# c-zhou/oatk

Hardware: AMD Instinct MI355X
Metric: HiFi Gbases/s through syncasm (syncmer+syncerr) at k=1001 s=31 (higher is better)
Workload: dtype u64

## Files before the change

### include/oatk_hip_ec.h

```cpp
#ifndef OATK_HIP_EC_H
#define OATK_HIP_EC_H

#include "oatk_hip.h"

#ifdef __cplusplus
extern "C" {
#endif

typedef struct {
    uint64_t n_vtx, n_arc;
    const uint64_t *idx_p;
    const uint64_t *idx_n;
    const uint64_t *arc_v;
    const uint64_t *arc_w;
    const uint64_t *arc_ls;
    const uint32_t *arc_cov;
    const uint8_t *arc_del;
} oatk_ec_graph_t;

int oatk_hip_ec(oatk_hip_ctx *ctx, const oatk_ec_graph_t *g, double max_edist, uint32_t err_mer_c, uint32_t max_err_c,
                uint32_t err_arc_c, double max_arc_f);

int oatk_hip_ec_stats(oatk_hip_ctx *ctx, uint64_t *stats12);

int oatk_hip_debug_ec_tiers(oatk_hip_ctx *ctx, int cap_t0, int cap_t1);

int oatk_hip_debug_wf_ed(oatk_hip_ctx *ctx, uint64_t n_jobs, const uint8_t *t_codes, const uint64_t *t_off, const uint8_t *q_codes, const uint64_t *q_off,
                         const int32_t *bw, const int32_t *step_ql, const uint64_t *step_off, int32_t *out3);
int oatk_hip_debug_wf_ed_wg(oatk_hip_ctx *ctx, int R, uint64_t n_jobs, const uint8_t *t_codes, const uint64_t *t_off, const uint8_t *q_codes, const uint64_t *q_off,
                            const int32_t *bw, const int32_t *step_ql, const uint64_t *step_off, int32_t *out3);
int oatk_hip_debug_tables(oatk_hip_ctx *ctx, uint64_t n_jobs, const uint8_t *t_codes, const uint64_t *t_off, const uint8_t *s_codes, const uint64_t *s_off, int32_t *out, const uint64_t *out_off);

enum {
    OATK_BUF_EC_N_SCM = 100, OATK_BUF_EC_SCM_OFF, OATK_BUF_EC_KMER, OATK_BUF_EC_MPOS, OATK_BUF_EC_SMER,
    OATK_BUF_EC_SCM_COV, OATK_BUF_EC_SCM_DEL, OATK_BUF_EC_SCM_OCC_OFF, OATK_BUF_EC_SCM_OCC, OATK_BUF_EC_ERR_DEL,
    OATK_BUF_EC_SCM_FWD,
    OATK_BUF_EC_VTX_SRC,
    OATK_BUF_EC_BLOCK_WORK, OATK_BUF_EC_BLOCK_OUT,
    OATK_BUF_EC_CSEQ_LEN,
    OATK_BUF_EC_CSEQ_OFF,
    OATK_BUF_EC_CSEQ,
    OATK_BUF_EC_BLOCK_QEND
};

int oatk_hip_ec_keep_seq(oatk_hip_ctx *ctx, int on);
int oatk_hip_ec_corrected_reads(oatk_hip_ctx *ctx, uint64_t *n_bases);

int oatk_hip_ec_mark(oatk_hip_ctx *ctx, uint32_t err_mer_c, uint32_t max_err_c, uint32_t err_arc_c, double max_arc_f);
int oatk_hip_ec_correct(oatk_hip_ctx *ctx, double max_edist);

int oatk_hip_ec_graph(oatk_hip_ctx *ctx);
int oatk_hip_ec_graph_light(oatk_hip_ctx *ctx, uint32_t err_mer_c);

int oatk_hip_ec_set_global(oatk_hip_ctx *ctx, uint64_t n_global, const uint32_t *d_l2g, const uint32_t *d_cov, const uint64_t *d_s);
int oatk_hip_ec_pairs(oatk_hip_ctx *ctx, const void **d_keys, const void **d_dist, uint64_t *n_pairs);
int oatk_hip_ec_graph_from_pairs(oatk_hip_ctx *ctx, const uint64_t *d_keys, const uint32_t *d_dist, uint64_t n_pairs);
int oatk_hip_ec_graph_from_segments(oatk_hip_ctx *ctx, const uint64_t *d_keys, const uint64_t *d_val, uint64_t n_seg);
int oatk_hip_ec_export_kmers(oatk_hip_ctx *ctx, const uint32_t *d_ids, uint64_t n, uint8_t *d_out, uint32_t stride, uint8_t *d_rev);
int oatk_hip_ec_import_kmers(oatk_hip_ctx *ctx, const uint32_t *d_ids, const uint8_t *d_rev, const uint8_t *d_kmers, uint64_t n, uint32_t stride);
int oatk_hip_ec_reserve_import(oatk_hip_ctx *ctx, uint64_t bytes);

enum {
    OATK_BUF_EG_IDX_P = 120, OATK_BUF_EG_IDX_N, OATK_BUF_EG_ARC_V, OATK_BUF_EG_ARC_W, OATK_BUF_EG_ARC_LS, OATK_BUF_EG_ARC_COV,
    OATK_BUF_EG_ARC_COMP
};

#ifdef __cplusplus
}
#endif
#endif
```

### oatk_amd/_lib.py

```python
import ctypes as C
import os

HERE = os.path.dirname(os.path.abspath(__file__))
LIB_PATH = os.environ.get("OATK_HIP_LIB") or os.path.join(HERE, "lib", "liboatk_hip.so")
HOST_LIB_PATH = os.path.join(HERE, "lib", "liboatk_host.so")

OK, E_NODEV, E_ARG, E_STATE, E_SMER, E_SPLIT, E_NOMEM = range(7)
READ_ALIGN = 64
BUF = {name: i for i, name in enumerate([
    "HOCO_L", "N_SCM", "N_NN", "N_LRL", "HO_RL", "HOCO_S", "NN_KEY", "LRL_KEY", "LRL_VAL",
    "SCM_OFF", "POS_MPOS", "POS_SMER", "POS_HASH", "POS_KID",
    "SCM_H", "SCM_S", "SCM_COV", "SCM_OCC_OFF", "SCM_OCC"])}
BUF.update({name: 100 + i for i, name in enumerate([
    "EC_N_SCM", "EC_SCM_OFF", "EC_KMER", "EC_MPOS", "EC_SMER", "EC_SCM_COV", "EC_SCM_DEL", "EC_SCM_OCC_OFF", "EC_SCM_OCC", "EC_ERR_DEL",
    "EC_SCM_FWD", "EC_VTX_SRC", "EC_BLOCK_WORK", "EC_BLOCK_OUT", "EC_CSEQ_LEN", "EC_CSEQ_OFF", "EC_CSEQ", "EC_BLOCK_QEND"])})
BUF.update({name: 160 + i for i, name in enumerate(["INGEST_SEQ", "INGEST_OFF", "INGEST_LEN", "INGEST_HDR"])})
FMT_AUTO, FMT_FASTA, FMT_FASTQ = 0, 1, 2
BUF.update({name: 140 + i for i, name in enumerate(["CONS_SEL", "CONS_SLOT", "CONS_RL", "CONS_MSEQ", "CONS_FIRST", "CONS_TOT"])})
BUF.update({name: 200 + i for i, name in enumerate(["RA_ALN_SID", "RA_ALN_OFF", "RA_ALN_S", "RA_FRG_UID", "RA_FRG_UBEG", "RA_FRG_UEND", "RA_FRG_SBEG", "RA_FRG_SEND", "RA_SKIPPED"])})
BUF.update({name: 150 + i for i, name in enumerate(["OVL_KEY", "OVL_OFF", "OVL_DIST", "OVL_CNT", "OVL_TAIL"])})
BUF.update({name: 120 + i for i, name in enumerate([
    "EG_IDX_P", "EG_IDX_N", "EG_ARC_V", "EG_ARC_W", "EG_ARC_LS", "EG_ARC_COV", "EG_ARC_COMP"])})
BUF.update({name: 180 + i for i, name in enumerate([
    "AG_SCM_DEL", "AG_VTX_SCM", "AG_VTX_COV", "AG_IDX_P", "AG_IDX_N", "AG_ARC_V", "AG_ARC_W", "AG_ARC_COV", "AG_ARC_COMP", "AG_ARC_LINK"])})
BUF.update({name: 220 + i for i, name in enumerate(["MG_H", "MG_S", "MG_COV", "MG_L2G", "MG_EC_COV", "MG_EC_DEL", "MG_LCOV"])})
BUF.update({name: 230 + i for i, name in enumerate(["MG_G_H", "MG_G_S", "MG_G_COV", "MG_G_DEL", "MG_G_OCC_OFF", "MG_G_OCC", "MG_POS_GKID"])})
TIMERS = ["hpc", "syncmer", "syncmer_n", "scan_post", "count_place", "count_sort", "count_group", "kmer_hash", "ec_graph", "ec_mark", "ec_solve", "ec_refresh"]

EXPORTS = [
    "oatk_hip_abi_version", "oatk_hip_device_count", "oatk_hip_create", "oatk_hip_destroy", "oatk_hip_last_error",
    "oatk_hip_stream", "oatk_hip_sync", "oatk_hip_max_k", "oatk_hip_scan", "oatk_hip_scan_host", "oatk_hip_count",
    "oatk_comm_unique_id", "oatk_comm_create", "oatk_comm_group_create", "oatk_comm_group_rank", "oatk_comm_group_destroy", "oatk_comm_destroy",
    "oatk_comm_rank", "oatk_comm_size", "oatk_comm_backend", "oatk_comm_traffic", "oatk_hip_merge_counts", "oatk_hip_multi_range", "oatk_hip_ec_sharded",
    "oatk_hip_gather_table", "oatk_hip_asm_graph_sharded", "oatk_hip_consensus_sharded", "oatk_hip_overlap_hist_sharded", "oatk_hip_stat_sharded",
    "oatk_hip_scan_begin", "oatk_hip_scan_reserve", "oatk_hip_scan_append", "oatk_hip_device", "oatk_hip_d2d", "oatk_hip_mem_pool",
    "oatk_hip_info", "oatk_hip_buffer", "oatk_hip_d2h", "oatk_hip_d2h_async", "oatk_hip_h2d_async", "oatk_hip_staging", "oatk_hip_ingest_text_buffer", "oatk_hip_set_timing", "oatk_hip_get_timing",
    "oatk_hip_debug_hash_mask", "oatk_hip_debug_force_general", "oatk_hip_debug_list_cap",
    "oatk_hip_ec_graph", "oatk_hip_ec_graph_light", "oatk_hip_ec", "oatk_hip_ec_stats", "oatk_hip_debug_ec_tiers", "oatk_hip_debug_wf_ed", "oatk_hip_debug_wf_ed_wg", "oatk_hip_ec_mark", "oatk_hip_ec_correct",
    "oatk_hip_ec_set_global", "oatk_hip_ec_pairs", "oatk_hip_ec_graph_from_pairs", "oatk_hip_ec_graph_from_segments", "oatk_hip_ec_export_kmers", "oatk_hip_ec_import_kmers",
    "oatk_hip_ec_reserve_import", "oatk_hip_consensus", "oatk_hip_consensus_ids", "oatk_hip_ingest", "oatk_hip_ingest_host", "oatk_hip_scan_ingested", "oatk_hip_stat", "oatk_hip_stat_keys", "oatk_hip_stat_from_keys",
    "oatk_hip_asm_graph", "oatk_hip_asm_pairs", "oatk_hip_asm_graph_from_pairs", "oatk_hip_overlap_hist", "oatk_hip_overlap_pairs", "oatk_hip_overlap_hist_from_pairs", "oatk_hip_read_alignment", "oatk_hip_debug_align_two_pass",
    "oatk_hip_ra_utg_coverage", "oatk_hip_ra_arc_coverage", "oatk_hip_debug_racov_cap", "oatk_hip_ra_utg_coverage_sharded", "oatk_hip_ra_arc_coverage_sharded",
    "oatk_hip_ra_triplet_scores", "oatk_hip_ra_triplet_scores_sharded",
    "oatk_hip_ec_keep_seq", "oatk_hip_ec_corrected_reads",
]

HOST_EXPORTS = ["oatk_multi_scg_ra_utg_coverage", "oatk_multi_scg_ra_arc_coverage", "oatk_scg_multiplex_plan", "oatk_multi_scg_multiplex_plan",
                "oatk_triplet_table_free", "oatk_multi_read_error_correction_fo"]


def load_host():
    H = C.CDLL(HOST_LIB_PATH)
    vp = C.c_void_p
    H.oatk_sr_db_new.restype = vp
    H.oatk_sr_db_new.argtypes = [C.c_int, C.c_int]
    H.oatk_multi_create.restype = vp
    H.oatk_multi_create.argtypes = [C.POINTER(C.c_int), C.c_int]
    H.oatk_multi_destroy.argtypes = [vp]
    H.oatk_multi_ctx.restype = vp
    H.oatk_multi_ctx.argtypes = [vp, C.c_int]
    H.oatk_multi_last_error.restype = C.c_char_p
    H.oatk_multi_last_error.argtypes = [vp]
    H.oatk_multi_range.argtypes = [vp, C.c_int, C.POINTER(C.c_uint64), C.POINTER(C.c_uint64)]
    H.oatk_multi_sr_read_files.argtypes = [vp, vp, C.POINTER(C.c_char_p), C.c_int]
    H.oatk_multi_collect_syncmer_from_reads.restype = vp
    H.oatk_multi_collect_syncmer_from_reads.argtypes = [vp, vp, C.POINTER(C.c_int)]
    H.oatk_multi_read_error_correction.argtypes = [vp, vp, vp, C.c_double, C.c_uint32, C.c_uint32, C.c_uint32, C.c_double, vp]
    H.oatk_multi_read_error_correction_fo.argtypes = [vp, vp, vp, C.c_double, C.c_uint32, C.c_uint32, C.c_uint32, C.c_double, vp, vp]
    H.oatk_multi_make_syncmer_asmg.restype = vp
    H.oatk_multi_make_syncmer_asmg.argtypes = [vp, vp, C.c_uint32, C.c_double, C.POINTER(C.c_int)]
    H.oatk_multi_scg_read_alignment.argtypes = [vp, vp, vp, vp, C.c_int, C.POINTER(C.c_uint64)]
    H.oatk_multi_scg_ra_utg_coverage.argtypes = [vp, vp, vp, vp, C.c_int]
    H.oatk_multi_scg_ra_arc_coverage.argtypes = [vp, vp, vp, vp, C.c_int]
    H.oatk_scg_multiplex_plan.argtypes = [vp, vp, vp, C.c_uint, C.c_uint32, C.c_double, C.c_double, vp, C.POINTER(C.c_int), C.POINTER(TripletTable)]
    H.oatk_multi_scg_multiplex_plan.argtypes = [vp, vp, vp, C.c_uint32, C.c_double, C.c_double, vp, C.POINTER(C.c_int), C.POINTER(TripletTable)]
    H.oatk_triplet_table_free.restype = None
    H.oatk_triplet_table_free.argtypes = [C.POINTER(TripletTable)]
    H.oatk_host_debug_window.argtypes = [C.c_uint64]
    return H


class TripletTable(C.Structure):
    _fields_ = [("n", C.c_uint64), ("m", C.c_uint64), ("l_in", C.POINTER(C.c_uint64)), ("l_out", C.POINTER(C.c_uint64)), ("val", C.POINTER(C.c_double))]


class EcGraph(C.Structure):
    _fields_ = [("n_vtx", C.c_uint64), ("n_arc", C.c_uint64), ("idx_p", C.c_void_p), ("idx_n", C.c_void_p), ("arc_v", C.c_void_p),
                ("arc_w", C.c_void_p), ("arc_ls", C.c_void_p), ("arc_cov", C.c_void_p), ("arc_del", C.c_void_p)]


class RaGraph(C.Structure):
    _fields_ = [("n_scm", C.c_uint64), ("n_utg", C.c_uint64), ("n_arc", C.c_uint64), ("su_off", C.c_void_p), ("su_uid", C.c_void_p), ("su_pos", C.c_void_p),
                ("utg_n", C.c_void_p), ("idx_p", C.c_void_p), ("idx_n", C.c_void_p), ("arc_w", C.c_void_p), ("arc_ln", C.c_void_p), ("arc_del", C.c_void_p)]


class RacovGraph(C.Structure):
    _fields_ = [("n_scm", C.c_uint64), ("n_utg", C.c_uint64), ("n_arc", C.c_uint64), ("su_off", C.c_void_p), ("su_uid", C.c_void_p), ("su_pos", C.c_void_p),
                ("scm_cov", C.c_void_p), ("utg_off", C.c_void_p), ("utg_a", C.c_void_p), ("idx_p", C.c_void_p), ("idx_n", C.c_void_p), ("arc_v", C.c_void_p),
                ("arc_w", C.c_void_p), ("arc_link", C.c_void_p), ("arc_comp", C.c_void_p), ("arc_del", C.c_void_p), ("vtx_del", C.c_void_p)]


class RacovAln(C.Structure):
    _fields_ = [("n_aln", C.c_uint64), ("n_frg", C.c_uint64), ("sid", C.c_void_p), ("off", C.c_void_p), ("s", C.c_void_p), ("uid", C.c_void_p),
                ("u_beg", C.c_void_p), ("u_end", C.c_void_p), ("s_beg", C.c_void_p), ("s_end", C.c_void_p)]


class RacovReads(C.Structure):
    _fields_ = [("n_reads", C.c_uint64), ("off", C.c_void_p), ("k_mer", C.c_void_p)]


class StatRaw(C.Structure):
    _fields_ = [("n_reads", C.c_uint64), ("n_syncmers", C.c_uint64), ("sum_dist", C.c_int64), ("n_dist", C.c_uint64),
                ("smer_unique", C.c_uint64), ("kmer_unique", C.c_uint64), ("smer_cnt", C.c_int64 * 1001), ("kmer_cnt", C.c_int64 * 1001),
                ("smer_no_singleton", C.c_int64), ("kmer_no_singleton", C.c_int64)]


class Info(C.Structure):
    _fields_ = [("n_reads", C.c_uint64), ("seq_bytes", C.c_uint64), ("sid0", C.c_uint64),
                ("k", C.c_int32), ("s", C.c_int32),
                ("n_occ", C.c_uint64), ("n_nn", C.c_uint64), ("n_lrl", C.c_uint64), ("n_scm", C.c_uint64),
                ("scan_retries", C.c_uint32), ("collisions", C.c_uint32)]


class OatkHipError(RuntimeError):
    pass


_lib = None


def load():
    global _lib
    if _lib is not None:
        return _lib
    if not os.path.exists(LIB_PATH):
        raise OatkHipError("%s is missing: build it with __graft_entry__.build()" % LIB_PATH)
    L = C.CDLL(LIB_PATH)
    vp = C.c_void_p
    L.oatk_hip_abi_version.restype = C.c_int
    L.oatk_hip_device_count.restype = C.c_int
    L.oatk_hip_create.restype = vp
    L.oatk_hip_create.argtypes = [C.c_int]
    L.oatk_hip_destroy.argtypes = [vp]
    L.oatk_hip_last_error.restype = C.c_char_p
    L.oatk_hip_last_error.argtypes = [vp]
    L.oatk_hip_stream.restype = vp
    L.oatk_hip_stream.argtypes = [vp]
    L.oatk_hip_sync.argtypes = [vp]
    L.oatk_hip_max_k.restype = C.c_int
    L.oatk_hip_scan.argtypes = [vp, vp, vp, vp, C.c_uint64, C.c_uint64, C.c_uint64, C.c_int, C.c_int]
    L.oatk_hip_scan_host.argtypes = [vp, vp, vp, vp, C.c_uint64, C.c_uint64, C.c_uint64, C.c_int, C.c_int]
    L.oatk_hip_count.argtypes = [vp]
    L.oatk_comm_unique_id.argtypes = [vp]
    L.oatk_comm_create.restype = vp
    L.oatk_comm_create.argtypes = [vp, C.c_int, C.c_int, C.c_int]
    L.oatk_comm_group_create.restype = vp
    L.oatk_comm_group_create.argtypes = [C.c_int]
    L.oatk_comm_group_rank.restype = vp
    L.oatk_comm_group_rank.argtypes = [vp, C.c_int]
    L.oatk_comm_group_destroy.argtypes = [vp]
    L.oatk_comm_destroy.argtypes = [vp]
    L.oatk_comm_rank.argtypes = [vp]
    L.oatk_comm_size.argtypes = [vp]
    L.oatk_comm_backend.restype = C.c_char_p
    L.oatk_comm_backend.argtypes = [vp]
    L.oatk_comm_traffic.restype = None
    L.oatk_comm_traffic.argtypes = [vp, C.POINTER(C.c_uint64), C.c_int]
    L.oatk_hip_merge_counts.argtypes = [vp, vp, C.POINTER(C.c_uint64)]
    L.oatk_hip_multi_range.argtypes = [vp, C.POINTER(C.c_uint64), C.POINTER(C.c_uint64), C.POINTER(C.c_uint64)]
    L.oatk_hip_ec_sharded.argtypes = [vp, vp, C.c_double, C.c_uint32, C.c_uint32, C.c_uint32, C.c_double, vp, C.POINTER(C.c_uint64)]
    L.oatk_hip_gather_table.argtypes = [vp, vp, C.c_int]
    L.oatk_hip_asm_graph_sharded.argtypes = [vp, vp, C.c_uint32, C.c_double, C.POINTER(C.c_uint64), C.POINTER(C.c_uint64)]
    L.oatk_hip_consensus_sharded.argtypes = [vp, vp, C.c_uint32]
    L.oatk_hip_overlap_hist_sharded.argtypes = [vp, vp, C.c_uint32, C.POINTER(C.c_uint64), C.POINTER(C.c_uint64)]
    L.oatk_hip_stat_sharded.argtypes = [vp, vp, C.POINTER(StatRaw)]
    L.oatk_hip_scan_begin.argtypes = [vp, C.c_uint64, C.c_int, C.c_int]
    L.oatk_hip_scan_reserve.argtypes = [vp, C.c_uint64, C.c_uint64, C.c_uint64]
    L.oatk_hip_scan_append.argtypes = [vp, vp]
    L.oatk_hip_device.argtypes = [vp]
    L.oatk_hip_mem_pool.argtypes = [vp, C.c_uint64]
    L.oatk_hip_d2d.argtypes = [vp, vp, vp, C.c_uint64]
    L.oatk_hip_info.argtypes = [vp, C.POINTER(Info)]
    L.oatk_hip_buffer.argtypes = [vp, C.c_int, C.POINTER(vp), C.POINTER(C.c_uint64)]
    L.oatk_hip_d2h.argtypes = [vp, vp, vp, C.c_uint64]
    L.oatk_hip_staging.restype = vp
    L.oatk_hip_staging.argtypes = [vp, C.c_uint64]
    L.oatk_hip_set_timing.argtypes = [vp, C.c_int]
    L.oatk_hip_get_timing.argtypes = [vp, C.POINTER(C.c_float), C.c_int]
    L.oatk_hip_debug_hash_mask.argtypes = [vp, C.c_uint64]
    L.oatk_hip_debug_force_general.argtypes = [vp, C.c_int]
    L.oatk_hip_debug_list_cap.argtypes = [vp, C.c_int]
    L.oatk_hip_ec_graph.argtypes = [vp]
    L.oatk_hip_ec_graph_light.argtypes = [vp, C.c_uint32]
    L.oatk_hip_ec.argtypes = [vp, C.POINTER(EcGraph), C.c_double, C.c_uint32, C.c_uint32, C.c_uint32, C.c_double]
    L.oatk_hip_ec_stats.argtypes = [vp, vp]
    L.oatk_hip_debug_ec_tiers.argtypes = [vp, C.c_int, C.c_int]
    L.oatk_hip_debug_wf_ed.argtypes = [vp, C.c_uint64, vp, vp, vp, vp, vp, vp, vp, vp]
    if hasattr(L, "oatk_hip_debug_wf_ed_wg"):
        L.oatk_hip_debug_wf_ed_wg.argtypes = [vp, C.c_int, C.c_uint64, vp, vp, vp, vp, vp, vp, vp, vp]
    if hasattr(L, "oatk_hip_debug_ed_ab"):
        L.oatk_hip_debug_ed_ab.argtypes = [vp, C.c_int, C.c_uint64, vp, vp, vp, vp, vp, vp, C.POINTER(C.c_float)]
    L.oatk_hip_ec_mark.argtypes = [vp, C.c_uint32, C.c_uint32, C.c_uint32, C.c_double]
    L.oatk_hip_ec_correct.argtypes = [vp, C.c_double]
    L.oatk_hip_ec_keep_seq.argtypes = [vp, C.c_int]
    L.oatk_hip_ec_corrected_reads.argtypes = [vp, C.POINTER(C.c_uint64)]
    L.oatk_hip_ec_set_global.argtypes = [vp, C.c_uint64, vp, vp, vp]
    L.oatk_hip_ec_pairs.argtypes = [vp, C.POINTER(vp), C.POINTER(vp), C.POINTER(C.c_uint64)]
    L.oatk_hip_ec_graph_from_pairs.argtypes = [vp, vp, vp, C.c_uint64]
    L.oatk_hip_ec_graph_from_segments.argtypes = [vp, vp, vp, C.c_uint64]
    L.oatk_hip_ec_export_kmers.argtypes = [vp, vp, C.c_uint64, vp, C.c_uint32, vp]
    L.oatk_hip_ec_import_kmers.argtypes = [vp, vp, vp, vp, C.c_uint64, C.c_uint32]
    L.oatk_hip_ec_reserve_import.argtypes = [vp, C.c_uint64]
    L.oatk_hip_consensus.argtypes = [vp, C.c_uint32]
    L.oatk_hip_consensus_ids.argtypes = [vp, vp, C.c_uint64]
    L.oatk_hip_ingest.argtypes = [vp, vp, C.c_uint64, C.c_int, C.c_int, C.POINTER(C.c_uint64), C.POINTER(C.c_uint64)]
    L.oatk_hip_ingest_host.argtypes = [vp, vp, C.c_uint64, C.c_int, C.c_int, C.POINTER(C.c_uint64), C.POINTER(C.c_uint64)]
    L.oatk_hip_scan_ingested.argtypes = [vp, C.c_uint64, C.c_int, C.c_int]
    L.oatk_hip_stat.argtypes = [vp, C.POINTER(StatRaw)]
    L.oatk_hip_stat_keys.argtypes = [vp, C.POINTER(vp), C.POINTER(vp), C.POINTER(C.c_uint64), vp]
    L.oatk_hip_stat_from_keys.argtypes = [vp, vp, vp, C.c_uint64, vp, C.POINTER(StatRaw)]
    L.oatk_hip_debug_align_two_pass.argtypes = [vp, C.c_int]
    L.oatk_hip_read_alignment.argtypes = [vp, C.POINTER(RaGraph), vp, C.POINTER(C.c_uint64), C.POINTER(C.c_uint64), vp]
    L.oatk_hip_ra_utg_coverage.argtypes = [vp, C.POINTER(RacovGraph), C.POINTER(RacovReads), C.POINTER(RacovAln), C.c_int, vp, C.POINTER(C.c_uint64)]
    L.oatk_hip_ra_arc_coverage.argtypes = [vp, C.POINTER(RacovGraph), C.POINTER(RacovAln), vp]
    L.oatk_hip_debug_racov_cap.argtypes = [vp, C.c_uint64]
    L.oatk_hip_ra_utg_coverage_sharded.argtypes = [vp, vp, C.POINTER(RacovGraph), C.POINTER(RacovReads), C.POINTER(RacovAln), C.c_int, vp, C.POINTER(C.c_uint64)]
    L.oatk_hip_ra_arc_coverage_sharded.argtypes = [vp, vp, C.POINTER(RacovGraph), C.POINTER(RacovAln), vp]
    u64p = C.POINTER(C.c_uint64)
    L.oatk_hip_ra_triplet_scores.argtypes = [vp, C.POINTER(RacovGraph), C.POINTER(RacovAln), vp, C.c_uint64, u64p, vp, vp, vp, vp]
    L.oatk_hip_ra_triplet_scores_sharded.argtypes = [vp, vp, C.POINTER(RacovGraph), C.POINTER(RacovAln), vp, C.c_uint64, u64p, vp, vp, vp, vp]
    L.oatk_hip_overlap_pairs.argtypes = [vp, C.POINTER(vp), C.POINTER(vp), C.POINTER(C.c_uint64)]
    L.oatk_hip_overlap_hist_from_pairs.argtypes = [vp, vp, vp, C.c_uint64, C.POINTER(C.c_uint64), C.POINTER(C.c_uint64)]
    L.oatk_hip_overlap_hist.argtypes = [vp, C.POINTER(C.c_uint64), C.POINTER(C.c_uint64)]
    L.oatk_hip_asm_graph.argtypes = [vp, C.c_uint32, C.c_double, C.POINTER(C.c_uint64), C.POINTER(C.c_uint64)]
    L.oatk_hip_asm_pairs.argtypes = [vp, C.POINTER(vp), C.POINTER(C.c_uint64)]
    L.oatk_hip_asm_graph_from_pairs.argtypes = [vp, vp, C.c_uint64, C.c_uint64, vp, vp, C.c_uint32, C.c_double, C.POINTER(C.c_uint64), C.POINTER(C.c_uint64)]
    _lib = L
    return L
```

### oatk_amd/csrc/api_ec.inc

```
#include "../../include/oatk_hip_ec.h"
#include "ec.hpp"
#include "ec_wave.hpp"
#include "ec_heavy.hpp"
#include "ec_fused.hpp"
#include "ecgraph.hpp"
#include "ec_seq.hpp"
#include <rocprim/device/device_run_length_encode.hpp>
#include <rocprim/device/device_select.hpp>

struct EcState {
    DevBuf idx_p, idx_n, arc_v, arc_w, arc_ls, arc_cov, arc_del, conv;
    DevBuf scm_del, err_del, vtx_hs_off, vtx_mpos;
    DevBuf copy_n, seg, keep_all, n_blocks, n_blocks64, blk_off, work, out, path_pool, cursor, todo, todo2, slabs, big_slabs, os_slabs;
    DevBuf hyb_slabs[16];
    hipStream_t aux[5] = {nullptr, nullptr, nullptr, nullptr, nullptr};
    hipEvent_t aux_ev[5] = {nullptr, nullptr, nullptr, nullptr, nullptr}, fork_ev = nullptr;
    DevBuf new_n, new_n64, new_off, new_k, new_m, new_s, stats;
    DevBuf live32, live64, live_off, larc, lidx_p, lidx_n;
    DevBuf cov, fwd, key_id, key_sorted, val_occ, occ, occ_off, cov64;
    uint64_t n_vtx = 0, new_tot = 0;
    uint64_t stats_h[12] = {0};
    uint64_t n_work = 0;
    bool done = false;
    DevBuf g_keys, g_keys2, g_ukeys, g_counts, g_nruns, g_nout, g_nout64, g_outoff, g_akey, g_aval, g_skey, g_sval, g_comp, g_flags, g_huge;
    DevBuf g_dist, g_dist2, g_cnt64, g_runoff, g_runls;
    DevBuf g_big, g_keep, g_other, g_lkeys, g_ldist, g_val2, g_wgt2, g_runcov, g_head, g_hpos, g_iota, g_segk, g_segv;
    uint32_t light_c = 0;
    uint64_t g_n_vtx = 0, g_n_arc = 0;
    bool graph_resident = false;
    bool global = false, marked = false;
    uint64_t n_global = 0, imp_used = 0;
    DevBuf g_l2g, g_kid, g_gcov, g_gs;
    bool keep_seq = false;
    bool seq_kept = false, cseq_done = false;
    bool seq_global = false;
    DevBuf slot_w, slot_w64, slot_off, slots, qend, sblk, clen, cbytes, cbytes64, coff, cseq;
    uint64_t cseq_bytes = 0;
};

static uint64_t ec_n_vtx(oatk_hip_ctx *ctx) { return ctx->ec && ctx->ec->global? ctx->ec->n_global : ctx->n_scm_total; }
static const uint64_t *ec_chains(oatk_hip_ctx *ctx) { return ctx->ec && ctx->ec->global? ctx->ec->g_kid.as<uint64_t>() : ctx->pos_kid.as<uint64_t>(); }

static void ec_state_free(oatk_hip_ctx *ctx)
{
    if (!ctx->ec) return;
    EcState *e = ctx->ec;
    DevBuf *all[] = {&e->idx_p, &e->idx_n, &e->arc_v, &e->arc_w, &e->arc_ls, &e->arc_cov, &e->arc_del, &e->conv, &e->scm_del, &e->err_del,
                     &e->vtx_hs_off, &e->vtx_mpos, &e->copy_n, &e->seg, &e->keep_all, &e->n_blocks, &e->n_blocks64, &e->blk_off, &e->work, &e->out, &e->path_pool, &e->cursor,
                     &e->todo, &e->todo2, &e->slabs, &e->big_slabs, &e->os_slabs, &e->hyb_slabs[0], &e->hyb_slabs[1], &e->hyb_slabs[2], &e->hyb_slabs[3], &e->hyb_slabs[4], &e->hyb_slabs[5], &e->hyb_slabs[6], &e->hyb_slabs[7], &e->hyb_slabs[8], &e->hyb_slabs[9], &e->hyb_slabs[10], &e->hyb_slabs[11], &e->hyb_slabs[12], &e->hyb_slabs[13], &e->hyb_slabs[14], &e->hyb_slabs[15], &e->new_n, &e->new_n64, &e->new_off, &e->new_k, &e->new_m, &e->new_s, &e->stats,
                     &e->live32, &e->live64, &e->live_off, &e->larc, &e->lidx_p, &e->lidx_n, &e->cov, &e->fwd, &e->key_id, &e->key_sorted, &e->val_occ, &e->occ, &e->occ_off, &e->cov64,
                     &e->g_keys, &e->g_keys2, &e->g_ukeys, &e->g_counts, &e->g_nruns, &e->g_nout, &e->g_nout64, &e->g_outoff, &e->g_akey,
                     &e->g_aval, &e->g_skey, &e->g_sval, &e->g_comp, &e->g_flags, &e->g_huge, &e->g_dist, &e->g_dist2, &e->g_cnt64, &e->g_runoff, &e->g_runls,
                     &e->g_big, &e->g_keep, &e->g_other, &e->g_lkeys, &e->g_ldist, &e->g_val2, &e->g_wgt2, &e->g_runcov, &e->g_head, &e->g_hpos, &e->g_iota, &e->g_segk, &e->g_segv,
                     &e->g_l2g, &e->g_kid, &e->g_gcov, &e->g_gs,
                     &e->slot_w, &e->slot_w64, &e->slot_off, &e->slots, &e->qend, &e->sblk, &e->clen, &e->cbytes, &e->cbytes64, &e->coff, &e->cseq};
    for (DevBuf *b : all) b->release();
    for (int i = 0; i < 5; ++i) { if (e->aux[i]) (void) hipStreamDestroy(e->aux[i]); if (e->aux_ev[i]) (void) hipEventDestroy(e->aux_ev[i]); }
    if (e->fork_ev) (void) hipEventDestroy(e->fork_ev);
    delete e;
    ctx->ec = nullptr;
}

static int ec_buffer(oatk_hip_ctx *ctx, int which, const void **d_ptr, uint64_t *bytes)
{
    EcState *e = ctx->ec;
    if (e && which >= OATK_BUF_EG_IDX_P && which <= OATK_BUF_EG_ARC_COMP) {
        if (!e->graph_resident) { ctx->err = "EC graph requested before oatk_hip_ec_graph"; return OATK_E_STATE; }
        const uint64_t gv = e->g_n_vtx, ga = e->g_n_arc;
        switch (which) {
            case OATK_BUF_EG_IDX_P: *d_ptr = e->idx_p.p, *bytes = 2 * gv * 8; break;
            case OATK_BUF_EG_IDX_N: *d_ptr = e->idx_n.p, *bytes = 2 * gv * 4; break;
            case OATK_BUF_EG_ARC_V: *d_ptr = e->arc_v.p, *bytes = ga * 8; break;
            case OATK_BUF_EG_ARC_W: *d_ptr = e->arc_w.p, *bytes = ga * 8; break;
            case OATK_BUF_EG_ARC_LS: *d_ptr = e->arc_ls.p, *bytes = ga * 4; break;
            case OATK_BUF_EG_ARC_COV: *d_ptr = e->arc_cov.p, *bytes = ga * 4; break;
            default: *d_ptr = e->g_comp.p, *bytes = ga; break;
        }
        return OATK_OK;
    }
    if (e && (which == OATK_BUF_EC_VTX_SRC || (which == OATK_BUF_EC_ERR_DEL && !e->done))) {
        if (!e->marked) { ctx->err = "vertex sources / marks requested before oatk_hip_ec_mark"; return OATK_E_STATE; }
        if (which == OATK_BUF_EC_VTX_SRC) *d_ptr = e->vtx_hs_off.p, *bytes = e->n_vtx * 8;
        else *d_ptr = e->err_del.p, *bytes = e->n_vtx;
        return OATK_OK;
    }
    if (!e || !e->done) { ctx->err = "unknown buffer id, or error-correction results requested before oatk_hip_ec"; return OATK_E_STATE; }
    if (which == OATK_BUF_EC_BLOCK_WORK) { *d_ptr = e->work.p, *bytes = e->n_work * sizeof(oatk::EcWork); return OATK_OK; }
    if (which == OATK_BUF_EC_BLOCK_OUT) { *d_ptr = e->out.p, *bytes = e->n_work * sizeof(oatk::EcBlockOut); return OATK_OK; }
    if (which == OATK_BUF_EC_BLOCK_QEND) {
        if (!e->seq_kept) { ctx->err = "EC_BLOCK_QEND: the resident correction was made without oatk_hip_ec_keep_seq"; return OATK_E_STATE; }
        *d_ptr = e->qend.p, *bytes = e->n_work * 4;
        return OATK_OK;
    }
    if (which >= OATK_BUF_EC_CSEQ_LEN && which <= OATK_BUF_EC_CSEQ) {
        if (!e->seq_kept || !e->cseq_done) { ctx->err = "corrected sequences requested before oatk_hip_ec_corrected_reads"; return OATK_E_STATE; }
        if (which == OATK_BUF_EC_CSEQ_LEN) *d_ptr = e->clen.p, *bytes = ctx->n_reads * 4;
        else if (which == OATK_BUF_EC_CSEQ_OFF) *d_ptr = e->coff.p, *bytes = (ctx->n_reads + 1) * 8;
        else *d_ptr = e->cseq.p, *bytes = e->cseq_bytes;
        return OATK_OK;
    }
    const uint64_t n = ctx->n_reads, ns = e->n_vtx, tot = e->new_tot;
    switch (which) {
        case OATK_BUF_EC_N_SCM: *d_ptr = e->new_n.p, *bytes = n * 4; break;
        case OATK_BUF_EC_SCM_OFF: *d_ptr = e->new_off.p, *bytes = (n + 1) * 8; break;
        case OATK_BUF_EC_KMER: *d_ptr = e->new_k.p, *bytes = tot * 8; break;
        case OATK_BUF_EC_MPOS: *d_ptr = e->new_m.p, *bytes = tot * 4; break;
        case OATK_BUF_EC_SMER: *d_ptr = e->new_s.p, *bytes = tot * 8; break;
        case OATK_BUF_EC_SCM_COV: *d_ptr = e->cov.p, *bytes = ns * 4; break;
        case OATK_BUF_EC_SCM_DEL: *d_ptr = e->scm_del.p, *bytes = ns; break;
        case OATK_BUF_EC_SCM_OCC_OFF: *d_ptr = e->occ_off.p, *bytes = (ns + 1) * 8; break;
        case OATK_BUF_EC_SCM_OCC: *d_ptr = e->occ.p, *bytes = tot * 8; break;
        case OATK_BUF_EC_ERR_DEL: *d_ptr = e->err_del.p, *bytes = ns; break;
        case OATK_BUF_EC_SCM_FWD: *d_ptr = e->fwd.p, *bytes = ns * 4; break;
        default: ctx->err = "unknown buffer id"; return OATK_E_ARG;
    }
    return OATK_OK;
}

__global__ void ec_narrow_kernel(const uint64_t *in, uint32_t *out, uint64_t n)
{
    uint64_t i = (uint64_t) blockIdx.x * blockDim.x + threadIdx.x;
    if (i < n) out[i] = (uint32_t) in[i];
}
__global__ void ec_widen_kernel(const uint32_t *in, uint64_t *out, uint64_t n)
{
    uint64_t i = (uint64_t) blockIdx.x * blockDim.x + threadIdx.x;
    if (i < n) out[i] = in[i];
    if (i == n) out[i] = 0;
}
#define EENSURE(buf, bytes, ...)                                                                   \
    do {                                                                                           \
        if (!e->buf.ensure((bytes), ctx->stream, ##__VA_ARGS__)) {                                 \
            ctx->err = "hipMalloc failed for ec." #buf;                                            \
            return OATK_E_NOMEM;                                                                   \
        }                                                                                          \
    } while (0)

static int ec_exclusive_scan_u32(oatk_hip_ctx *ctx, EcState *e, DevBuf &in32, DevBuf &tmp64, DevBuf &out64, uint64_t n, uint64_t *total)
{
    if (!tmp64.ensure((n + 1) * 8, ctx->stream) || !out64.ensure((n + 1) * 8, ctx->stream)) { ctx->err = "hipMalloc failed (ec scan)"; return OATK_E_NOMEM; }
    hipLaunchKernelGGL(ec_widen_kernel, dim3((unsigned) ((n + 1 + 255) / 256)), dim3(256), 0, ctx->stream, in32.as<uint32_t>(), tmp64.as<uint64_t>(), n);
    size_t tb = 0;
    CK(rocprim::exclusive_scan(nullptr, tb, tmp64.as<uint64_t>(), out64.as<uint64_t>(), (uint64_t) 0, n + 1, rocprim::plus<uint64_t>(), ctx->stream));
    if (!ctx->tmp.ensure(tb, ctx->stream)) { ctx->err = "hipMalloc failed (ec scan tmp)"; return OATK_E_NOMEM; }
    CK(rocprim::exclusive_scan(ctx->tmp.p, tb, tmp64.as<uint64_t>(), out64.as<uint64_t>(), (uint64_t) 0, n + 1, rocprim::plus<uint64_t>(), ctx->stream));
    CK(hipMemcpyAsync(total, out64.as<uint64_t>() + n, 8, hipMemcpyDeviceToHost, ctx->stream));
    CK(hipStreamSynchronize(ctx->stream));
    (void) e;
    return OATK_OK;
}

extern "C" int oatk_hip_debug_ec_tiers(oatk_hip_ctx *ctx, int cap_t0, int cap_t1)
{
    if (!ctx) return OATK_E_NODEV;
    if (cap_t0 < 0 || cap_t1 < 0 || (cap_t0 && cap_t1 && cap_t1 < cap_t0)) { ctx->err = "oatk_hip_debug_ec_tiers: 0 <= cap_t0 <= cap_t1"; return OATK_E_ARG; }
    ctx->ec_cap_t0 = cap_t0, ctx->ec_cap_t1 = cap_t1;
    return OATK_OK;
}

static int debug_ed_impl(oatk_hip_ctx *ctx, uint64_t n_jobs, const uint8_t *t_codes, const uint64_t *t_off, const uint8_t *q_codes, const uint64_t *q_off,
                         const int32_t *bw, const int32_t *step_ql, const uint64_t *step_off, int32_t *out3, bool myers, float *kernel_ms, int wg_R = 0)
{
    using namespace oatk;
    if (!ctx) return OATK_E_NODEV;
    if (n_jobs == 0) return OATK_OK;
    if (n_jobs >= 0x7FFFFFFFULL) { ctx->err = "oatk_hip_debug_wf_ed: too many jobs"; return OATK_E_ARG; }
    CK(hipSetDevice(ctx->device));
    std::vector<uint64_t> tw_off(n_jobs + 1, 0), qw_off(n_jobs + 1, 0), k_off(n_jobs + 1, 0);
    std::vector<int32_t> tl(n_jobs);
    for (uint64_t j = 0; j < n_jobs; ++j) {
        const uint64_t t = t_off[j + 1] - t_off[j], q = q_off[j + 1] - q_off[j];
        if (t == 0 || q == 0 || t > 0x3FFFFFFF || q > 0x3FFFFFFF) { ctx->err = "oatk_hip_debug_wf_ed: empty or oversized string (wf_ed asserts tl > 0 && ql > 0)"; return OATK_E_ARG; }
        for (uint64_t s = step_off[j]; s < step_off[j + 1]; ++s)
            if (step_ql[s] < 1 || (uint64_t) step_ql[s] > q || (s > step_off[j] && step_ql[s] < step_ql[s - 1])) { ctx->err = "oatk_hip_debug_wf_ed: query lengths must ascend within the query"; return OATK_E_ARG; }
        tl[j] = (int32_t) t;
        if (wg_R && (bw[j] >= 0? (uint64_t) 2 * (uint64_t) bw[j] + 3 : t + q + 3) > (wg_R == ECF_NW? (uint64_t) ECF_NW * ECF_OWN : (uint64_t) 64 * ECH_NW * (uint64_t) wg_R)) { ctx->err = "oatk_hip_debug_wf_ed_wg: a job's diagonals do not fit the registers of this variant"; return OATK_E_ARG; }
        tw_off[j + 1] = tw_off[j] + ecw_words((int32_t) t), qw_off[j + 1] = qw_off[j] + ecw_words((int32_t) q);
        k_off[j + 1] = k_off[j] + 2 * (t + q + 8);
    }
    auto pack = [](const uint8_t *codes, const uint64_t *off, const std::vector<uint64_t> &woff, uint64_t n) {
        std::vector<uint32_t> w(woff[n], 0u);
        for (uint64_t j = 0; j < n; ++j)
            for (uint64_t p = 0, len = off[j + 1] - off[j]; p < len; ++p)
                w[woff[j] + (p >> 4)] |= (uint32_t) (codes[off[j] + p] & 3u) << ((p & 15u) << 1);
        return w;
    };
    const std::vector<uint32_t> tw = pack(t_codes, t_off, tw_off, n_jobs), qw = pack(q_codes, q_off, qw_off, n_jobs);
    const uint64_t n_steps = step_off[n_jobs];
    DevBuf d_tw, d_qw, d_two, d_qwo, d_tl, d_bw, d_sq, d_so, d_k, d_ko, d_out, d_slab;
    DevBuf *all[] = {&d_tw, &d_qw, &d_two, &d_qwo, &d_tl, &d_bw, &d_sq, &d_so, &d_k, &d_ko, &d_out, &d_slab};
    hipEvent_t ev0 = nullptr, ev1 = nullptr;
    if (kernel_ms) { *kernel_ms = 0.f; (void) hipEventCreate(&ev0); (void) hipEventCreate(&ev1); }
    int32_t max_t = 0;
    for (uint64_t j = 0; j < n_jobs; ++j) if (tl[j] > max_t) max_t = tl[j];
    const uint64_t n_waves = (n_jobs + 63) / 64, slab_words = (uint64_t) 6 * 64 * (uint64_t) ((max_t + 63) / 64 + 1);
    std::vector<int32_t> ql_last(n_jobs);
    for (uint64_t j = 0; j < n_jobs; ++j) ql_last[j] = step_off[j + 1] > step_off[j]? step_ql[step_off[j + 1] - 1] : (int32_t) (q_off[j + 1] - q_off[j]);
    int rc = OATK_OK;
    hipError_t he = hipSuccess;
    auto up = [&](DevBuf &b, const void *src, size_t bytes) {
        if (rc) return;
        if (!b.ensure(bytes + 16, ctx->stream)) { rc = OATK_E_NOMEM; return; }
        if (bytes && (he = hipMemcpyAsync(b.p, src, bytes, hipMemcpyHostToDevice, ctx->stream)) != hipSuccess) rc = OATK_E_NODEV;
    };
    up(d_tw, tw.data(), tw.size() * 4); up(d_qw, qw.data(), qw.size() * 4);
    up(d_two, tw_off.data(), (n_jobs + 1) * 8); up(d_qwo, qw_off.data(), (n_jobs + 1) * 8); up(d_ko, k_off.data(), (n_jobs + 1) * 8);
    up(d_tl, tl.data(), n_jobs * 4); up(d_bw, bw, n_jobs * 4); up(d_sq, step_ql, n_steps * 4); up(d_so, step_off, (n_jobs + 1) * 8);
    if (!rc && (!d_k.ensure(k_off[n_jobs] * 4 + 16, ctx->stream) || !d_out.ensure(n_steps * 12 + 16, ctx->stream))) rc = OATK_E_NOMEM;
    if (!rc && myers) {
        if (!d_slab.ensure(n_waves * slab_words * 8 + 64, ctx->stream) || !d_out.ensure(n_jobs * 12 + 16, ctx->stream)) rc = OATK_E_NOMEM;
        up(d_sq, ql_last.data(), n_jobs * 4);
    }
    if (!rc) {
        if (ev0) (void) hipEventRecord(ev0, ctx->stream);
#ifdef OATK_EXPERIMENTS
        if (myers)
            hipLaunchKernelGGL(myers_ed_kernel, dim3((unsigned) n_waves), dim3(64), 0, ctx->stream, n_jobs, d_tw.as<uint32_t>(), d_two.as<uint64_t>(), d_tl.as<int32_t>(),
                               d_qw.as<uint32_t>(), d_qwo.as<uint64_t>(), d_sq.as<int32_t>(), d_bw.as<int32_t>(), d_slab.as<uint64_t>(), slab_words, d_out.as<int32_t>());
        else
#endif
        if (wg_R) {
            uint64_t cap_words = 0;
            for (uint64_t j = 0; j < n_jobs; ++j) { if (tw_off[j + 1] - tw_off[j] > cap_words) cap_words = tw_off[j + 1] - tw_off[j]; if (qw_off[j + 1] - qw_off[j] > cap_words) cap_words = qw_off[j + 1] - qw_off[j]; }
            const uint64_t lds = ((uint64_t) ech_misc_words(wg_R) + 2 * cap_words) * 4;
            if (lds > 64 * 1024 || (wg_R != 1 && wg_R != 2 && wg_R != 6 && wg_R != ECF_NW)) { ctx->err = "oatk_hip_debug_wf_ed_wg: strings too long for LDS, or no such variant (1, 2, 6, 16)"; rc = OATK_E_ARG; }
            else if (wg_R == ECF_NW) hipLaunchKernelGGL((ecf_wf_ed_kernel<ECF_NW>), dim3((unsigned) n_jobs), dim3(64 * ECF_NW), (unsigned) (((uint64_t) ecf_misc_words(ECF_NW) + 2 * cap_words) * 4), ctx->stream, d_tw.as<uint32_t>(), d_two.as<uint64_t>(), d_tl.as<int32_t>(),
                                                         d_qw.as<uint32_t>(), d_qwo.as<uint64_t>(), d_bw.as<int32_t>(), d_sq.as<int32_t>(), d_so.as<uint64_t>(), d_out.as<int32_t>(), (int32_t) cap_words);
            else if (wg_R == 1) hipLaunchKernelGGL((ech_wf_ed_kernel<ECH_NW, 1>), dim3((unsigned) n_jobs), dim3(64 * ECH_NW), (unsigned) lds, ctx->stream, d_tw.as<uint32_t>(), d_two.as<uint64_t>(), d_tl.as<int32_t>(),
                                                    d_qw.as<uint32_t>(), d_qwo.as<uint64_t>(), d_bw.as<int32_t>(), d_sq.as<int32_t>(), d_so.as<uint64_t>(), d_out.as<int32_t>(), (int32_t) cap_words);
            else if (wg_R == 2) hipLaunchKernelGGL((ech_wf_ed_kernel<ECH_NW, 2>), dim3((unsigned) n_jobs), dim3(64 * ECH_NW), (unsigned) lds, ctx->stream, d_tw.as<uint32_t>(), d_two.as<uint64_t>(), d_tl.as<int32_t>(),
                                                    d_qw.as<uint32_t>(), d_qwo.as<uint64_t>(), d_bw.as<int32_t>(), d_sq.as<int32_t>(), d_so.as<uint64_t>(), d_out.as<int32_t>(), (int32_t) cap_words);
            else hipLaunchKernelGGL((ech_wf_ed_kernel<ECH_NW, 6>), dim3((unsigned) n_jobs), dim3(64 * ECH_NW), (unsigned) lds, ctx->stream, d_tw.as<uint32_t>(), d_two.as<uint64_t>(), d_tl.as<int32_t>(),
                                    d_qw.as<uint32_t>(), d_qwo.as<uint64_t>(), d_bw.as<int32_t>(), d_sq.as<int32_t>(), d_so.as<uint64_t>(), d_out.as<int32_t>(), (int32_t) cap_words);
        } else
        hipLaunchKernelGGL(ecw_wf_ed_kernel, dim3((unsigned) n_jobs), dim3(64), 0, ctx->stream, d_tw.as<uint32_t>(), d_two.as<uint64_t>(), d_tl.as<int32_t>(),
                           d_qw.as<uint32_t>(), d_qwo.as<uint64_t>(), d_bw.as<int32_t>(), d_sq.as<int32_t>(), d_so.as<uint64_t>(), d_k.as<int32_t>(),
                           d_ko.as<uint64_t>(), d_out.as<int32_t>());
        if (ev1) (void) hipEventRecord(ev1, ctx->stream);
        const uint64_t n_out = myers? n_jobs : n_steps;
        if (n_out && (he = hipMemcpyAsync(out3, d_out.p, n_out * 12, hipMemcpyDeviceToHost, ctx->stream)) != hipSuccess) rc = OATK_E_NODEV;
        if ((he = hipStreamSynchronize(ctx->stream)) != hipSuccess) rc = OATK_E_NODEV;
        if (!rc && (he = hipGetLastError()) != hipSuccess) rc = OATK_E_NODEV;
    }
    (void) hipStreamSynchronize(ctx->stream);
    if (ev0 && ev1 && !rc) (void) hipEventElapsedTime(kernel_ms, ev0, ev1);
    if (ev0) (void) hipEventDestroy(ev0);
    if (ev1) (void) hipEventDestroy(ev1);
    for (DevBuf *b : all) b->release();
    if (rc == OATK_E_NODEV) ctx->err = std::string("oatk_hip_debug_wf_ed: ") + hipGetErrorString(he);
    if (rc == OATK_E_NOMEM) ctx->err = "oatk_hip_debug_wf_ed: hipMalloc failed";
    return rc;
}

extern "C" int oatk_hip_debug_wf_ed(oatk_hip_ctx *ctx, uint64_t n_jobs, const uint8_t *t_codes, const uint64_t *t_off, const uint8_t *q_codes, const uint64_t *q_off,
                                    const int32_t *bw, const int32_t *step_ql, const uint64_t *step_off, int32_t *out3)
{
    float ms = 0.f;
    const bool timed = getenv("OATK_DEBUG_ED_TIME") != nullptr;
    const int rc = debug_ed_impl(ctx, n_jobs, t_codes, t_off, q_codes, q_off, bw, step_ql, step_off, out3, false, timed? &ms : nullptr);
    if (timed) fprintf(stderr, "[wf_ed_wg] R 0: %llu jobs, kernel %.3f ms\n", (unsigned long long) n_jobs, ms);
    return rc;
}

extern "C" int oatk_hip_debug_tables(oatk_hip_ctx *ctx, uint64_t n_jobs, const uint8_t *t_codes, const uint64_t *t_off, const uint8_t *s_codes, const uint64_t *s_off, int32_t *out, const uint64_t *out_off)
{
    using namespace oatk;
    if (!ctx) return OATK_E_NODEV;
    if (n_jobs == 0) return OATK_OK;
    if (n_jobs >= 0x7FFFFFFFULL) { ctx->err = "oatk_hip_debug_tables: too many jobs"; return OATK_E_ARG; }
    CK(hipSetDevice(ctx->device));
    std::vector<uint64_t> tw_off(n_jobs + 1, 0), qw_off(n_jobs + 1, 0);
    std::vector<int32_t> tl(n_jobs), ql(n_jobs);
    uint64_t cap_words = 0;
    for (uint64_t j = 0; j < n_jobs; ++j) {
        const uint64_t t = t_off[j + 1] - t_off[j], q = s_off[j + 1] - s_off[j];
        if (t == 0 || q == 0 || t > 0x3FFFFFFF || q > 1024) { ctx->err = "oatk_hip_debug_tables: an empty string, or one of more than 1024 bases"; return OATK_E_ARG; }
        if (out_off[j + 1] - out_off[j] < 2 * (t + 1)) { ctx->err = "oatk_hip_debug_tables: a job's output holds 2 (tl + 1) numbers"; return OATK_E_ARG; }
        tl[j] = (int32_t) t, ql[j] = (int32_t) q;
        tw_off[j + 1] = tw_off[j] + ecw_words((int32_t) t), qw_off[j + 1] = qw_off[j] + ecw_words((int32_t) q);
        if (tw_off[j + 1] - tw_off[j] > cap_words) cap_words = tw_off[j + 1] - tw_off[j];
        if (qw_off[j + 1] - qw_off[j] > cap_words) cap_words = qw_off[j + 1] - qw_off[j];
    }
    if (2 * cap_words * 4 > 64 * 1024) { ctx->err = "oatk_hip_debug_tables: strings too long for LDS"; return OATK_E_ARG; }
    auto pack = [](const uint8_t *codes, const uint64_t *off, const std::vector<uint64_t> &woff, uint64_t n) {
        std::vector<uint32_t> w(woff[n], 0u);
        for (uint64_t j = 0; j < n; ++j)
            for (uint64_t p = 0, len = off[j + 1] - off[j]; p < len; ++p)
                w[woff[j] + (p >> 4)] |= (uint32_t) (codes[off[j] + p] & 3u) << ((p & 15u) << 1);
        return w;
    };
    const std::vector<uint32_t> tw = pack(t_codes, t_off, tw_off, n_jobs), qw = pack(s_codes, s_off, qw_off, n_jobs);
    DevBuf d_tw, d_qw, d_two, d_qwo, d_tl, d_ql, d_oo, d_out;
    DevBuf *all[] = {&d_tw, &d_qw, &d_two, &d_qwo, &d_tl, &d_ql, &d_oo, &d_out};
    int rc = OATK_OK;
    hipError_t he = hipSuccess;
    auto up = [&](DevBuf &b, const void *src, size_t bytes) {
        if (rc) return;
        if (!b.ensure(bytes + 16, ctx->stream)) { rc = OATK_E_NOMEM; return; }
        if (bytes && (he = hipMemcpyAsync(b.p, src, bytes, hipMemcpyHostToDevice, ctx->stream)) != hipSuccess) rc = OATK_E_NODEV;
    };
    up(d_tw, tw.data(), tw.size() * 4); up(d_qw, qw.data(), qw.size() * 4);
    up(d_two, tw_off.data(), (n_jobs + 1) * 8); up(d_qwo, qw_off.data(), (n_jobs + 1) * 8);
    up(d_tl, tl.data(), n_jobs * 4); up(d_ql, ql.data(), n_jobs * 4); up(d_oo, out_off, (n_jobs + 1) * 8);
    const uint64_t n_out = out_off[n_jobs];
    if (!rc && !d_out.ensure(n_out * 4 + 16, ctx->stream)) rc = OATK_E_NOMEM;
    if (!rc) {
        int seg_nw = 1, seg_cut = 0;
        { const char *ev = getenv("OATK_DEBUG_TABLES_SEG"); if (ev && sscanf(ev, "%d:%d", &seg_nw, &seg_cut) != 2) seg_nw = 1, seg_cut = 0; }
        if (n_out && (he = hipMemsetAsync(d_out.p, 0xFF, n_out * 4, ctx->stream)) != hipSuccess) rc = OATK_E_NODEV;
#define OATK_TABLES_LAUNCH(NW) hipLaunchKernelGGL((ecb_tables_kernel<NW>), dim3((unsigned) n_jobs), dim3(64 * NW), (unsigned) (2 * cap_words * 4), ctx->stream, d_tw.as<uint32_t>(), d_two.as<uint64_t>(), d_tl.as<int32_t>(), \
                           d_qw.as<uint32_t>(), d_qwo.as<uint64_t>(), d_ql.as<int32_t>(), d_out.as<int32_t>(), d_oo.as<uint64_t>(), (int32_t) cap_words, (int32_t) seg_cut)
        if (seg_nw == 2) OATK_TABLES_LAUNCH(2); else if (seg_nw == 4) OATK_TABLES_LAUNCH(4); else if (seg_nw == 8) OATK_TABLES_LAUNCH(8); else if (seg_nw == 16) OATK_TABLES_LAUNCH(16); else OATK_TABLES_LAUNCH(1);
#undef OATK_TABLES_LAUNCH
        if (n_out && (he = hipMemcpyAsync(out, d_out.p, n_out * 4, hipMemcpyDeviceToHost, ctx->stream)) != hipSuccess) rc = OATK_E_NODEV;
        if ((he = hipStreamSynchronize(ctx->stream)) != hipSuccess) rc = OATK_E_NODEV;
        if (!rc && (he = hipGetLastError()) != hipSuccess) rc = OATK_E_NODEV;
    }
    (void) hipStreamSynchronize(ctx->stream);
    for (DevBuf *b : all) b->release();
    if (rc == OATK_E_NODEV) ctx->err = std::string("oatk_hip_debug_tables: ") + hipGetErrorString(he);
    if (rc == OATK_E_NOMEM) ctx->err = "oatk_hip_debug_tables: hipMalloc failed";
    return rc;
}

extern "C" int oatk_hip_debug_wf_ed_wg(oatk_hip_ctx *ctx, int R, uint64_t n_jobs, const uint8_t *t_codes, const uint64_t *t_off, const uint8_t *q_codes, const uint64_t *q_off,
                                       const int32_t *bw, const int32_t *step_ql, const uint64_t *step_off, int32_t *out3)
{
    if (R != 1 && R != 2 && R != 6 && R != ECF_NW) { if (ctx) ctx->err = "oatk_hip_debug_wf_ed_wg: R must be 1, 2, 6 (a workgroup per wavefront) or 16 (several steps per barrier: sixteen waves, 896 diagonals)"; return OATK_E_ARG; }
    float ms = 0.f;
    const bool timed = getenv("OATK_DEBUG_ED_TIME") != nullptr;
    const int rc = debug_ed_impl(ctx, n_jobs, t_codes, t_off, q_codes, q_off, bw, step_ql, step_off, out3, false, timed? &ms : nullptr, R);
    if (timed) fprintf(stderr, "[wf_ed_wg] R %d: %llu jobs, kernel %.3f ms\n", R, (unsigned long long) n_jobs, ms);
    return rc;
}

#ifdef OATK_EXPERIMENTS
extern "C" int oatk_hip_debug_ed_ab(oatk_hip_ctx *ctx, int myers, uint64_t n_jobs, const uint8_t *t_codes, const uint64_t *t_off, const uint8_t *q_codes,
                                    const uint64_t *q_off, const int32_t *bw, int32_t *out3, float *kernel_ms)
{
    if (!ctx) return OATK_E_NODEV;
    std::vector<int32_t> ql(n_jobs);
    std::vector<uint64_t> so(n_jobs + 1);
    for (uint64_t j = 0; j < n_jobs; ++j) ql[j] = (int32_t) (q_off[j + 1] - q_off[j]), so[j] = j;
    so[n_jobs] = n_jobs;
    return debug_ed_impl(ctx, n_jobs, t_codes, t_off, q_codes, q_off, bw, ql.data(), so.data(), out3, myers != 0, kernel_ms);
}
#endif

extern "C" int oatk_hip_ec_stats(oatk_hip_ctx *ctx, uint64_t *stats12)
{
    if (!ctx) return OATK_E_NODEV;
    if (!ctx->ec || !ctx->ec->done) { ctx->err = "oatk_hip_ec has not run"; return OATK_E_STATE; }
    for (int i = 0; i < 12; ++i) stats12[i] = ctx->ec->stats_h[i];
    return OATK_OK;
}

extern "C" int oatk_hip_ec_set_global(oatk_hip_ctx *ctx, uint64_t n_global, const uint32_t *d_l2g, const uint32_t *d_cov, const uint64_t *d_s)
{
    using namespace oatk;
    if (!ctx) return OATK_E_NODEV;
    if (!ctx->counted) { ctx->err = "oatk_hip_ec_set_global needs a resident scan + count"; return OATK_E_STATE; }
    CK(hipSetDevice(ctx->device));
    if (!ctx->ec) ctx->ec = new EcState();
    EcState *e = ctx->ec;
    e->graph_resident = false, e->done = false, e->marked = false, e->imp_used = 0;
    if (n_global == 0) { e->global = false, e->n_global = 0; return OATK_OK; }
    if (n_global < ctx->n_scm_total || n_global >= 0x7FFFFFFFULL) { ctx->err = "oatk_hip_ec_set_global: bad global table size"; return OATK_E_ARG; }
    const uint64_t nl = ctx->n_scm_total, nocc = ctx->n_occ;
    EENSURE(g_l2g, (nl + 1) * 4); EENSURE(g_gcov, (n_global + 1) * 4); EENSURE(g_gs, (n_global + 1) * 8); EENSURE(g_kid, (nocc + 1) * 8);
    CK(hipMemcpyAsync(e->g_l2g.p, d_l2g, nl * 4, hipMemcpyDeviceToDevice, ctx->stream));
    CK(hipMemcpyAsync(e->g_gcov.p, d_cov, n_global * 4, hipMemcpyDeviceToDevice, ctx->stream));
    CK(hipMemcpyAsync(e->g_gs.p, d_s, n_global * 8, hipMemcpyDeviceToDevice, ctx->stream));
    if (nocc) hipLaunchKernelGGL(ec_remap_kernel, dim3((unsigned) ((nocc + 255) / 256)), dim3(256), 0, ctx->stream, nocc, ctx->pos_kid.as<uint64_t>(),
                                 e->g_l2g.as<uint32_t>(), e->g_kid.as<uint64_t>());
    CK(hipStreamSynchronize(ctx->stream));
    CK(hipGetLastError());
    e->global = true, e->n_global = n_global;
    return OATK_OK;
}

extern "C" int oatk_hip_ec_pairs(oatk_hip_ctx *ctx, const void **d_keys, const void **d_dist, uint64_t *n_pairs)
{
    using namespace oatk;
    if (!ctx) return OATK_E_NODEV;
    if (!ctx->counted) { ctx->err = "oatk_hip_ec_pairs needs a resident scan + count"; return OATK_E_STATE; }
    CK(hipSetDevice(ctx->device));
    if (!ctx->ec) ctx->ec = new EcState();
    EcState *e = ctx->ec;
    const uint64_t nr = ctx->n_reads, nocc = ctx->n_occ;
    EENSURE(g_keys, (nocc + 1) * 8); EENSURE(g_dist, (nocc + 1) * 4);
    if (nocc) hipLaunchKernelGGL(egr_pair_keys_kernel, dim3((unsigned) ((nr + 255) / 256)), dim3(256), 0, ctx->stream, nr, ctx->scm_off.as<uint64_t>(),
                                 ec_chains(ctx), ctx->pos_mpos.as<uint32_t>(), e->g_keys.as<uint64_t>(), e->g_dist.as<uint32_t>(), 0);
    CK(hipStreamSynchronize(ctx->stream));
    CK(hipGetLastError());
    *d_keys = e->g_keys.p, *d_dist = e->g_dist.p, *n_pairs = nocc;
    return OATK_OK;
}

static int ec_graph_build(oatk_hip_ctx *ctx, const uint64_t *d_keys, const uint32_t *d_dist, const uint64_t *d_val, uint64_t nocc, bool timer_running = false)
{
    using namespace oatk;
    if (!ctx) return OATK_E_NODEV;
    if (!ctx->counted) { ctx->err = "oatk_hip_ec_graph needs a resident scan + count"; return OATK_E_STATE; }
    CK(hipSetDevice(ctx->device));
    if (!ctx->ec) ctx->ec = new EcState();
    EcState *e = ctx->ec;
    e->graph_resident = false, e->marked = false, e->light_c = 0;
    const bool weighted = d_val != nullptr;
    if (nocc >= 0xFFFFFFFFULL) { ctx->err = "more than 2^32 adjacent pairs"; return OATK_E_ARG; }
    const uint64_t nv = ec_n_vtx(ctx);
    if (nv >= 0x7FFFFFFFULL) { ctx->err = "too many syncmers for 32-bit oriented vertex ids"; return OATK_E_ARG; }
    auto blocks = [](uint64_t n) { return dim3((unsigned) ((n + 255) / 256 > 0? (n + 255) / 256 : 1)); };
    EENSURE(g_flags, 64);
    if (!timer_running) t_begin(ctx, OATK_T_EC_GRAPH);
    CK(hipMemsetAsync(e->g_flags.p, 0, 64, ctx->stream));
    EENSURE(idx_p, (2 * nv + 1) * 8); EENSURE(idx_n, (2 * nv + 1) * 4);
    CK(hipMemsetAsync(e->idx_p.p, 0, (2 * nv + 1) * 8, ctx->stream));
    CK(hipMemsetAsync(e->idx_n.p, 0, (2 * nv + 1) * 4, ctx->stream));
    uint64_t na = 0;
    if (nocc) {
        EENSURE(g_keys2, (nocc + 1) * 8); EENSURE(g_ukeys, (nocc + 1) * 8); EENSURE(g_counts, (nocc + 1) * 4);
        EENSURE(g_nruns, 64); EENSURE(g_dist2, (nocc + 1) * 4);
        uint64_t *keys_in = const_cast<uint64_t *>(d_keys);
        uint32_t *dist_in = const_cast<uint32_t *>(d_dist);
        size_t tb = 0;
        if (weighted) {
            EENSURE(g_val2, (nocc + 1) * 8); EENSURE(g_wgt2, (nocc + 1) * 4);
            uint64_t *val_in = const_cast<uint64_t *>(d_val);
            CK(rocprim::radix_sort_pairs(nullptr, tb, keys_in, e->g_keys2.as<uint64_t>(), val_in, e->g_val2.as<uint64_t>(), nocc, 0, 64, ctx->stream));
            ENSURE(tmp, tb);
            CK(rocprim::radix_sort_pairs(ctx->tmp.p, tb, keys_in, e->g_keys2.as<uint64_t>(), val_in, e->g_val2.as<uint64_t>(), nocc, 0, 64, ctx->stream));
            hipLaunchKernelGGL(egr_seg_split_kernel, blocks(nocc), dim3(256), 0, ctx->stream, nocc, e->g_val2.as<uint64_t>(), e->g_dist2.as<uint32_t>(), e->g_wgt2.as<uint32_t>());
        } else {
            CK(rocprim::radix_sort_pairs(nullptr, tb, keys_in, e->g_keys2.as<uint64_t>(), dist_in, e->g_dist2.as<uint32_t>(), nocc, 0, 64, ctx->stream));
            ENSURE(tmp, tb);
            CK(rocprim::radix_sort_pairs(ctx->tmp.p, tb, keys_in, e->g_keys2.as<uint64_t>(), dist_in, e->g_dist2.as<uint32_t>(), nocc, 0, 64, ctx->stream));
        }
        tb = 0;
        CK(rocprim::run_length_encode(nullptr, tb, e->g_keys2.as<uint64_t>(), (unsigned int) nocc, e->g_ukeys.as<uint64_t>(), e->g_counts.as<uint32_t>(),
                                      e->g_nruns.as<uint32_t>(), ctx->stream));
        ENSURE(tmp, tb);
        CK(rocprim::run_length_encode(ctx->tmp.p, tb, e->g_keys2.as<uint64_t>(), (unsigned int) nocc, e->g_ukeys.as<uint64_t>(), e->g_counts.as<uint32_t>(),
                                      e->g_nruns.as<uint32_t>(), ctx->stream));
        uint32_t n_runs = 0;
        CK(hipMemcpyAsync(&n_runs, e->g_nruns.p, 4, hipMemcpyDeviceToHost, ctx->stream));
        CK(hipStreamSynchronize(ctx->stream));
        EENSURE(g_nout, ((uint64_t) n_runs + 1) * 4);
        hipLaunchKernelGGL(egr_expand_count_kernel, blocks(n_runs), dim3(256), 0, ctx->stream, (uint64_t) n_runs, e->g_ukeys.as<uint64_t>(), e->g_nout.as<uint32_t>());
        { int rc = ec_exclusive_scan_u32(ctx, e, e->g_nout, e->g_nout64, e->g_outoff, n_runs, &na); if (rc) return rc; }
        uint64_t chk = 0;
        EENSURE(g_runls, ((uint64_t) n_runs + 1) * 4); EENSURE(g_runcov, ((uint64_t) n_runs + 1) * 4);
        { int rc = ec_exclusive_scan_u32(ctx, e, e->g_counts, e->g_cnt64, e->g_runoff, n_runs, &chk); if (rc) return rc; }
        if (n_runs) {
            EENSURE(g_big, ((uint64_t) n_runs + 1) * 8);
            EENSURE(g_huge, EGR_HUGE_SCRATCH);
            const uint32_t *wg = weighted? e->g_wgt2.as<uint32_t>() : (const uint32_t *) nullptr;
            uint32_t *rc_ = weighted? e->g_runcov.as<uint32_t>() : (uint32_t *) nullptr;
            hipLaunchKernelGGL(egr_mode_kernel, dim3((n_runs + 63) / 64), dim3(64), 0, ctx->stream, (uint64_t) n_runs, e->g_ukeys.as<uint64_t>(),
                               e->g_counts.as<uint32_t>(), e->g_runoff.as<uint64_t>(), e->g_dist2.as<uint32_t>(), ctx->K, e->g_runls.as<uint32_t>(),
                               e->g_flags.as<uint32_t>(), e->g_big.as<uint32_t>(), e->g_big.as<uint32_t>() + n_runs + 1, wg, rc_);
            hipLaunchKernelGGL(egr_mode_big_kernel, dim3(n_runs < 8192u? n_runs : 8192u), dim3(64), 0, ctx->stream, e->g_counts.as<uint32_t>(), e->g_runoff.as<uint64_t>(),
                               e->g_dist2.as<uint32_t>(), ctx->K, e->g_runls.as<uint32_t>(), e->g_flags.as<uint32_t>(), e->g_big.as<uint32_t>(),
                               e->g_big.as<uint32_t>() + n_runs + 1, wg, rc_);
            hipLaunchKernelGGL(egr_mode_huge_kernel, dim3(1024), dim3(64), 0, ctx->stream, e->g_counts.as<uint32_t>(), e->g_runoff.as<uint64_t>(),
                               e->g_dist2.as<uint32_t>(), ctx->K, e->g_runls.as<uint32_t>(), e->g_flags.as<uint32_t>(), e->g_big.as<uint32_t>() + n_runs + 1,
                               e->g_huge.as<uint8_t>(), (uint64_t) EGR_HUGE_SCRATCH, wg, rc_);
        }
        EENSURE(g_akey, (na + 1) * 8); EENSURE(g_aval, (na + 1) * 8); EENSURE(g_skey, (na + 1) * 8); EENSURE(g_sval, (na + 1) * 8);
        if (na) {
            hipLaunchKernelGGL(egr_expand_kernel, blocks(n_runs), dim3(256), 0, ctx->stream, (uint64_t) n_runs, e->g_ukeys.as<uint64_t>(),
                               weighted? e->g_runcov.as<uint32_t>() : e->g_counts.as<uint32_t>(), e->g_runls.as<uint32_t>(), e->g_outoff.as<uint64_t>(), e->g_akey.as<uint64_t>(), e->g_aval.as<uint64_t>());
            tb = 0;
            CK(rocprim::radix_sort_pairs(nullptr, tb, e->g_akey.as<uint64_t>(), e->g_skey.as<uint64_t>(), e->g_aval.as<uint64_t>(), e->g_sval.as<uint64_t>(), na, 0, 64, ctx->stream));
            ENSURE(tmp, tb);
            CK(rocprim::radix_sort_pairs(ctx->tmp.p, tb, e->g_akey.as<uint64_t>(), e->g_skey.as<uint64_t>(), e->g_aval.as<uint64_t>(), e->g_sval.as<uint64_t>(), na, 0, 64, ctx->stream));
        }
    }
    EENSURE(arc_v, (na + 1) * 8); EENSURE(arc_w, (na + 1) * 8); EENSURE(arc_ls, (na + 1) * 4); EENSURE(arc_cov, (na + 1) * 4); EENSURE(arc_del, na + 8);
    EENSURE(g_comp, na + 8);
    EgrArcs a;
    a.n_arc = na, a.arc_v = e->arc_v.as<uint64_t>(), a.arc_w = e->arc_w.as<uint64_t>(), a.arc_ls = e->arc_ls.as<uint32_t>(), a.arc_cov = e->arc_cov.as<uint32_t>();
    a.arc_comp = e->g_comp.as<uint8_t>(), a.arc_del = e->arc_del.as<uint8_t>(), a.idx_p = e->idx_p.as<uint64_t>(), a.idx_n = e->idx_n.as<uint32_t>();
    a.flags = e->g_flags.as<uint32_t>();
    if (na) {
        hipLaunchKernelGGL(egr_unpack_kernel, blocks(na), dim3(256), 0, ctx->stream, a, (const uint64_t *) e->g_skey.p, (const uint64_t *) e->g_sval.p);
    }
    uint32_t fl[4] = {0, 0, 0, 0};
    CK(hipMemcpyAsync(fl, e->g_flags.p, sizeof(fl), hipMemcpyDeviceToHost, ctx->stream));
    t_end(ctx, OATK_T_EC_GRAPH);
    CK(hipStreamSynchronize(ctx->stream));
    CK(hipGetLastError());
    t_collect(ctx, OATK_T_EC_GRAPH, OATK_T_EC_GRAPH);
    if (fl[0]) { ctx->err = "EC graph has duplicate arcs (a syncmer adjacent to itself on both strands): the reference's order is unspecified"; return OATK_E_SPLIT; }
    if (fl[1]) { ctx->err = "EC graph: the arcs with more than 48 distinct syncmer distances need more than the 256 MB of working memory set aside for them"; return OATK_E_SPLIT; }
    if (debug_refuse(ctx, 1, "oatk_hip_ec_graph")) return OATK_E_SPLIT;
    e->g_n_vtx = nv, e->g_n_arc = na;
    e->graph_resident = true;
    return OATK_OK;
}

extern "C" int oatk_hip_ec_graph_from_pairs(oatk_hip_ctx *ctx, const uint64_t *d_keys, const uint32_t *d_dist, uint64_t nocc)
{
    return ec_graph_build(ctx, d_keys, d_dist, nullptr, nocc);
}

extern "C" int oatk_hip_ec_graph_from_segments(oatk_hip_ctx *ctx, const uint64_t *d_keys, const uint64_t *d_val, uint64_t n_seg)
{
    if (ctx && !d_val && n_seg) { ctx->err = "oatk_hip_ec_graph_from_segments: no segment values"; return OATK_E_ARG; }
    return ec_graph_build(ctx, d_keys, nullptr, d_val? d_val : (const uint64_t *) d_keys, n_seg);
}

extern "C" int oatk_hip_ec_graph(oatk_hip_ctx *ctx)
{
    const void *k = nullptr, *d = nullptr;
    uint64_t n = 0;
    int rc = oatk_hip_ec_pairs(ctx, &k, &d, &n);
    if (rc) return rc;
    return oatk_hip_ec_graph_from_pairs(ctx, (const uint64_t *) k, (const uint32_t *) d, n);
}

template <class T>
static int ec_select(oatk_hip_ctx *ctx, EcState *e, const T *in, const uint8_t *flag, uint64_t n, T *out, uint64_t *n_out)
{
    *n_out = 0;
    if (n == 0) return OATK_OK;
    EENSURE(g_nruns, 64);
    uint64_t *d_cnt = e->g_nruns.as<uint64_t>() + 2;
    size_t tb = 0;
    CK(rocprim::select(nullptr, tb, in, flag, out, d_cnt, n, ctx->stream));
    ENSURE(tmp, tb);
    CK(rocprim::select(ctx->tmp.p, tb, in, flag, out, d_cnt, n, ctx->stream));
    CK(hipMemcpyAsync(n_out, d_cnt, 8, hipMemcpyDeviceToHost, ctx->stream));
    CK(hipStreamSynchronize(ctx->stream));
    return OATK_OK;
}

static int ec_light_pairs(oatk_hip_ctx *ctx, uint32_t c, const uint64_t **d_keys, const uint32_t **d_dist, uint64_t *n_keep)
{
    using namespace oatk;
    if (!ctx->counted) { ctx->err = "the light EC graph needs a resident scan + count"; return OATK_E_STATE; }
    if (!ctx->ec) ctx->ec = new EcState();
    EcState *e = ctx->ec;
    const uint64_t nv = ec_n_vtx(ctx), nr = ctx->n_reads, n = ctx->n_occ;
    int rc;
    EENSURE(g_keys, (n + 1) * 8); EENSURE(g_dist, (n + 1) * 4);
    EENSURE(g_other, 2 * nv + 8); EENSURE(g_keep, n + 8); EENSURE(g_lkeys, (n + 1) * 8); EENSURE(g_ldist, (n + 1) * 4);
    t_begin(ctx, OATK_T_EC_GRAPH);
    CK(hipMemsetAsync(e->g_other.p, 0, 2 * nv + 8, ctx->stream));
    if (n) hipLaunchKernelGGL(egr_pair_light_wave_kernel, dim3((unsigned) ((nr + 3) / 4)), dim3(256), 0, ctx->stream, nr, ctx->scm_off.as<uint64_t>(), ec_chains(ctx),
                              ctx->pos_mpos.as<uint32_t>(), e->global? e->g_gcov.as<uint32_t>() : ctx->scm_cov.as<uint32_t>(), c, e->g_keys.as<uint64_t>(), e->g_dist.as<uint32_t>(),
                              e->g_keep.as<uint8_t>(), e->g_other.as<uint8_t>());
    uint64_t nk = 0;
    if (n) {
        if (n >= 0xFFFFFFFFULL) { ctx->err = "more than 2^32 adjacent pairs"; return OATK_E_ARG; }
        EENSURE(g_keys2, (n + 1) * 8); EENSURE(g_nruns, 64);
        uint32_t *pos = e->g_keys2.as<uint32_t>();
        uint64_t *d_cnt = e->g_nruns.as<uint64_t>() + 2;
        auto flags = rocprim::make_transform_iterator(e->g_keep.as<uint8_t>(), [] __device__(uint8_t f) -> uint32_t { return f; });
        size_t tb = 0;
        CK(rocprim::exclusive_scan(nullptr, tb, flags, pos, 0u, n, rocprim::plus<uint32_t>(), ctx->stream));
        ENSURE(tmp, tb);
        CK(rocprim::exclusive_scan(ctx->tmp.p, tb, flags, pos, 0u, n, rocprim::plus<uint32_t>(), ctx->stream));
        hipLaunchKernelGGL(egr_compact_pairs_kernel, dim3((unsigned) ((n + 255) / 256)), dim3(256), 0, ctx->stream, n, e->g_keep.as<uint8_t>(), pos, e->g_keys.as<uint64_t>(),
                           e->g_dist.as<uint32_t>(), e->g_lkeys.as<uint64_t>(), e->g_ldist.as<uint32_t>(), d_cnt);
        CK(hipMemcpyAsync(&nk, d_cnt, 8, hipMemcpyDeviceToHost, ctx->stream));
        CK(hipStreamSynchronize(ctx->stream));
    }
    (void) rc;
    CK(hipGetLastError());
    *d_keys = e->g_lkeys.as<uint64_t>(), *d_dist = e->g_ldist.as<uint32_t>(), *n_keep = nk;
    return OATK_OK;
}

extern "C" int oatk_hip_ec_graph_light(oatk_hip_ctx *ctx, uint32_t err_mer_c)
{
    if (!ctx) return OATK_E_NODEV;
    if (!ctx->counted) { ctx->err = "oatk_hip_ec_graph_light needs a resident scan + count"; return OATK_E_STATE; }
    CK(hipSetDevice(ctx->device));
    if (!ctx->ec) ctx->ec = new EcState();
    if (err_mer_c == 0) return oatk_hip_ec_graph(ctx);
    const uint64_t *k = nullptr;
    const uint32_t *d = nullptr;
    uint64_t n = 0;
    int rc = ec_light_pairs(ctx, err_mer_c, &k, &d, &n);
    if (rc) return rc;
    if ((rc = ec_graph_build(ctx, k, d, nullptr, n, true)) != OATK_OK) return rc;
    ctx->ec->light_c = err_mer_c;
    return OATK_OK;
}

#define EC_VIEWS()                                                                                                                       \
    const uint64_t nv = e->g_n_vtx, na = e->g_n_arc, nr = ctx->n_reads, nocc = ctx->n_occ;                                               \
    auto blocks = [](uint64_t n) { return dim3((unsigned) ((n + 255) / 256 > 0? (n + 255) / 256 : 1)); };                                 \
    EcGraph g;                                                                                                                           \
    g.n_vtx = nv, g.n_arc = na, g.idx_p = e->idx_p.as<uint64_t>(), g.idx_n = e->idx_n.as<uint32_t>();                                    \
    g.arc_v = e->arc_v.as<uint64_t>(), g.arc_w = e->arc_w.as<uint64_t>(), g.arc_ls = e->arc_ls.as<uint32_t>(), g.arc_cov = e->arc_cov.as<uint32_t>(); \
    g.arc_del = e->arc_del.as<uint8_t>(), g.scm_del = e->scm_del.as<uint8_t>();                                                          \
    g.scm_cov = e->global? e->g_gcov.as<uint32_t>() : ctx->scm_cov.as<uint32_t>(), g.scm_s = e->global? e->g_gs.as<uint64_t>() : ctx->scm_s.as<uint64_t>(); \
    g.vtx_hs_off = e->vtx_hs_off.as<uint64_t>(), g.vtx_mpos = e->vtx_mpos.as<uint32_t>();                                                \
    g.other = e->light_c? e->g_other.as<uint8_t>() : (const uint8_t *) nullptr;                                                          \
    EcReads rd;                                                                                                                          \
    rd.n_reads = nr, rd.sid0 = ctx->sid0, rd.K = ctx->K, rd.hoco_s = ctx->hoco_s.as<uint8_t>(), rd.off = ctx->d_off, rd.hoco_l = ctx->hoco_l.as<uint32_t>(); \
    rd.scm_off = ctx->scm_off.as<uint64_t>(), rd.k_mer = ec_chains(ctx), rd.m_pos = ctx->pos_mpos.as<uint32_t>();                        \
    (void) nocc; (void) blocks; (void) rd

static int ec_upload_graph(oatk_hip_ctx *ctx, const oatk_ec_graph_t *hg)
{
    EcState *e = ctx->ec;
    const uint64_t nv = hg->n_vtx, na = hg->n_arc;
    auto blocks = [](uint64_t n) { return dim3((unsigned) ((n + 255) / 256 > 0? (n + 255) / 256 : 1)); };
    e->graph_resident = false, e->light_c = 0;

    EENSURE(idx_p, (2 * nv + 1) * 8); EENSURE(idx_n, (2 * nv + 1) * 4); EENSURE(conv, (2 * nv + na + 2) * 8);
    EENSURE(arc_v, (na + 1) * 8); EENSURE(arc_w, (na + 1) * 8); EENSURE(arc_ls, (na + 1) * 4); EENSURE(arc_cov, (na + 1) * 4); EENSURE(arc_del, na + 8);
    CK(hipMemcpyAsync(e->idx_p.p, hg->idx_p, 2 * nv * 8, hipMemcpyHostToDevice, ctx->stream));
    CK(hipMemcpyAsync(e->conv.p, hg->idx_n, 2 * nv * 8, hipMemcpyHostToDevice, ctx->stream));
    hipLaunchKernelGGL(ec_narrow_kernel, blocks(2 * nv), dim3(256), 0, ctx->stream, e->conv.as<uint64_t>(), e->idx_n.as<uint32_t>(), 2 * nv);
    if (na) {
        CK(hipMemcpyAsync(e->arc_v.p, hg->arc_v, na * 8, hipMemcpyHostToDevice, ctx->stream));
        CK(hipMemcpyAsync(e->arc_w.p, hg->arc_w, na * 8, hipMemcpyHostToDevice, ctx->stream));
        CK(hipStreamSynchronize(ctx->stream));
        CK(hipMemcpyAsync(e->conv.p, hg->arc_ls, na * 8, hipMemcpyHostToDevice, ctx->stream));
        hipLaunchKernelGGL(ec_narrow_kernel, blocks(na), dim3(256), 0, ctx->stream, e->conv.as<uint64_t>(), e->arc_ls.as<uint32_t>(), na);
        CK(hipMemcpyAsync(e->arc_cov.p, hg->arc_cov, na * 4, hipMemcpyHostToDevice, ctx->stream));
        CK(hipMemcpyAsync(e->arc_del.p, hg->arc_del, na, hipMemcpyHostToDevice, ctx->stream));
    }
    CK(hipStreamSynchronize(ctx->stream));
    e->g_n_vtx = nv, e->g_n_arc = na;
    e->graph_resident = true;
    return OATK_OK;
}

extern "C" int oatk_hip_ec_mark(oatk_hip_ctx *ctx, uint32_t err_mer_c, uint32_t max_err_c, uint32_t err_arc_c, double max_arc_f)
{
    using namespace oatk;
    if (!ctx) return OATK_E_NODEV;
    if (!ctx->counted || !ctx->ec || !ctx->ec->graph_resident) { ctx->err = "oatk_hip_ec_mark needs a resident scan + count and an EC graph"; return OATK_E_STATE; }
    CK(hipSetDevice(ctx->device));
    EcState *e = ctx->ec;
    e->done = false, e->marked = false, e->imp_used = 0;
    if (e->g_n_vtx != ec_n_vtx(ctx)) { ctx->err = "EC graph must have one vertex per syncmer"; return OATK_E_ARG; }
    if (e->light_c && !(err_mer_c >= e->light_c && err_arc_c >= err_mer_c && max_err_c >= err_mer_c)) {
        ctx->err = "the resident EC graph is a light one: it serves err_arc_c >= err_mer_c >= the coverage it was built for, and max_err_c >= err_mer_c (oatk_hip_ec_graph_light)";
        return OATK_E_ARG;
    }
    e->n_vtx = e->g_n_vtx;
    EENSURE(scm_del, e->g_n_vtx + 8); EENSURE(err_del, e->g_n_vtx + 8); EENSURE(vtx_hs_off, (e->g_n_vtx + 1) * 8); EENSURE(vtx_mpos, (e->g_n_vtx + 1) * 4);
    EC_VIEWS();
    t_begin(ctx, OATK_T_EC_MARK);
    CK(hipMemsetAsync(e->scm_del.p, 0, nv + 8, ctx->stream));
    if (na) CK(hipMemsetAsync(e->arc_del.p, 0, na, ctx->stream));
    CK(hipMemsetAsync(e->vtx_hs_off.p, 0xFF, (nv + 1) * 8, ctx->stream));
    const uint64_t nl = ctx->n_scm_total;
    if (nl) hipLaunchKernelGGL(ec_vtx_src_kernel, blocks(nl), dim3(256), 0, ctx->stream, nl, ctx->scm_loc.as<uint64_t>(),
                               e->global? e->g_l2g.as<uint32_t>() : (const uint32_t *) nullptr, e->vtx_hs_off.as<uint64_t>(), e->vtx_mpos.as<uint32_t>());
    hipLaunchKernelGGL(ec_mark_kernel, blocks(nv), dim3(256), 0, ctx->stream, g, err_mer_c, max_err_c, err_arc_c, max_arc_f);
    if (na) hipLaunchKernelGGL(ec_arc_del_kernel, blocks(na), dim3(256), 0, ctx->stream, g);
    CK(hipMemcpyAsync(e->err_del.p, e->scm_del.p, nv, hipMemcpyDeviceToDevice, ctx->stream));
    CK(hipStreamSynchronize(ctx->stream));
    CK(hipGetLastError());
    e->marked = true;
    return OATK_OK;
}

extern "C" int oatk_hip_ec_export_kmers(oatk_hip_ctx *ctx, const uint32_t *d_ids, uint64_t n, uint8_t *d_out, uint32_t stride, uint8_t *d_rev)
{
    using namespace oatk;
    if (!ctx) return OATK_E_NODEV;
    if (!ctx->ec || !ctx->ec->marked) { ctx->err = "oatk_hip_ec_export_kmers needs oatk_hip_ec_mark"; return OATK_E_STATE; }
    if (stride % 16 || stride < (uint32_t) ((ctx->K + 3) / 4 + 8)) { ctx->err = "k-mer stride must be a multiple of 16 and hold the k-mer + 8 bytes"; return OATK_E_ARG; }
    CK(hipSetDevice(ctx->device));
    EcState *e = ctx->ec;
    if (n) hipLaunchKernelGGL(ecw_export_kmer_kernel, dim3((unsigned) n), dim3(64), 0, ctx->stream, n, d_ids, e->vtx_hs_off.as<uint64_t>(), e->vtx_mpos.as<uint32_t>(),
                              ctx->hoco_s.as<uint8_t>(), ctx->K, stride, d_out, d_rev);
    CK(hipStreamSynchronize(ctx->stream));
    CK(hipGetLastError());
    return OATK_OK;
}

extern "C" int oatk_hip_ec_import_kmers(oatk_hip_ctx *ctx, const uint32_t *d_ids, const uint8_t *d_rev, const uint8_t *d_kmers, uint64_t n, uint32_t stride)
{
    using namespace oatk;
    if (!ctx) return OATK_E_NODEV;
    if (!ctx->ec || !ctx->ec->marked) { ctx->err = "oatk_hip_ec_import_kmers needs oatk_hip_ec_mark"; return OATK_E_STATE; }
    if (stride % 16 || stride < (uint32_t) ((ctx->K + 3) / 4 + 8)) { ctx->err = "k-mer stride must be a multiple of 16 and hold the k-mer + 8 bytes"; return OATK_E_ARG; }
    CK(hipSetDevice(ctx->device));
    EcState *e = ctx->ec;
    if (n && !ctx->hoco_s.p) { ctx->err = "oatk_hip_ec_import_kmers: this batch has no hoco strings to put k-mers behind"; return OATK_E_STATE; }
    const uint64_t base = ((ctx->seq_bytes / 4 + 128) + 15) & ~15ULL;
    if (e->imp_used + n * stride > ctx->import_reserve) { ctx->err = "imported k-mers exceed the reserve behind the hoco strings (oatk_hip_ec_reserve_import before the scan)"; return OATK_E_NOMEM; }
    if (n) {
        CK(hipMemcpyAsync(ctx->hoco_s.as<uint8_t>() + base + e->imp_used, d_kmers, n * stride, hipMemcpyDeviceToDevice, ctx->stream));
        hipLaunchKernelGGL(ecw_import_kmer_kernel, dim3((unsigned) ((n + 255) / 256)), dim3(256), 0, ctx->stream, n, d_ids, d_rev, base + e->imp_used, stride,
                           e->vtx_hs_off.as<uint64_t>(), e->vtx_mpos.as<uint32_t>());
        e->imp_used += n * stride;
    }
    CK(hipStreamSynchronize(ctx->stream));
    CK(hipGetLastError());
    return OATK_OK;
}

extern "C" int oatk_hip_ec_reserve_import(oatk_hip_ctx *ctx, uint64_t bytes)
{
    if (!ctx) return OATK_E_NODEV;
    ctx->import_reserve = bytes < (1u << 20)? (1u << 20) : (bytes + 15) & ~15ULL;
    return OATK_OK;
}

struct EcKnobs {
    int heavy = -1;
    bool stages = false;
    bool serial_tiers = false;
    int32_t step_budget = 1000;
    int32_t min_nw = 0;
    int32_t heavy_cap2 = 0;
    int32_t heavy_fl = 0;
    int32_t waves = 32;
    bool assemble_walk = false;
};
static EcKnobs ec_knobs_read()
{
    EcKnobs k;
    auto num = [](const char *n, int32_t lo, int32_t dflt) { const char *e = getenv(n); return e && atoi(e) >= lo? (int32_t) atoi(e) : dflt; };
    { const char *e = getenv("OATK_DEBUG_EC_HEAVY"); k.heavy = e && (e[0] == '0' || e[0] == '1') && !e[1]? e[0] - '0' : -1; }
    k.stages = getenv("OATK_DEBUG_EC_STAGES") != nullptr;
    { const char *e = getenv("OATK_DEBUG_EC_SERIAL_TIERS"); k.serial_tiers = e && e[0] == '1'; }
    k.step_budget = num("OATK_DEBUG_EC_STEP_BUDGET", 1, 1000);
    k.min_nw = num("OATK_DEBUG_EC_FUSED_MIN_NW", 2, 0);
    k.heavy_cap2 = num("OATK_DEBUG_EC_HEAVY_CAP2", 1, 0), k.heavy_fl = num("OATK_DEBUG_EC_HEAVY_FL", 64, 0) & ~7;
    k.waves = num("OATK_DEBUG_EC_WAVES", 1, 32);
    { const char *e = getenv("OATK_DEBUG_EC_ASSEMBLE_WALK"); k.assemble_walk = e && e[0] == '1'; }
    return k;
}

namespace oatk {

static const int32_t EC_CAP_T0 = 3072;
static const int32_t EC_CAP_T1 = 16384;
static const int32_t EC_ARC_BUDGET = 512;

struct EcTier { int32_t cap_t, cap_c, cap_w, cap_path, cap_f; uint64_t bytes, slab; bool usable, hybrid; int wpb; };

static int32_t ec_cap_c(int32_t cap_t, int K) { return cap_t + cap_t / 8 + 2 * K + 64; }

static int32_t ec_band_cap(int32_t bwmax, double max_edist)
{
    int64_t ct = max_edist > 0? (int64_t) floor((double) bwmax / max_edist) : 0x3FFFFFFF;
    while (ct > 0 && (int32_t) ceil((double) ct * max_edist) > bwmax) --ct;
    return (int32_t) (ct > 60000? 60000 : ct);
}

static uint64_t ec_wg_per_cu(uint64_t bytes)
{
    const uint64_t n = 160 * 1024 / (bytes + 256);
    return n > 16? 16 : (n? n : 1);
}

static EcTier ec_lds_tier(int32_t cap_t, int32_t cap_path, int32_t cap_f, bool hybrid, double max_edist, int K)
{
    EcTier t;
    const int32_t bw = (int32_t) (cap_t * max_edist) + 1;
    t.cap_t = cap_t, t.cap_w = 2 * (bw > EC_MIN_ERR_BASE? bw : EC_MIN_ERR_BASE) + 12, t.cap_c = ec_cap_c(cap_t, K);
    t.hybrid = hybrid;
    if (hybrid) {
        t.cap_path = t.cap_c, t.cap_f = 1 << 20;
        t.bytes = (uint64_t) ecw_lds_words_hybrid(t.cap_t, t.cap_c, t.cap_w) * 4;
        t.slab = ecw_slab_bytes_hybrid(t.cap_path, t.cap_f);
    } else {
        t.cap_path = cap_path, t.cap_f = cap_f;
        t.bytes = (uint64_t) ecw_scratch_words(t.cap_t, t.cap_c, t.cap_w, t.cap_path, t.cap_f, false) * 4;
        t.slab = 0;
    }
    t.usable = t.bytes <= 64 * 1024;
    t.wpb = ECW_WPB * t.bytes <= 64 * 1024? ECW_WPB : 1;
    return t;
}

static uint64_t ec_tier_waves(const EcTier &t, int32_t per_cu_max, int n_cu)
{
    uint64_t per_cu = ec_wg_per_cu((uint64_t) t.wpb * t.bytes) * (uint64_t) t.wpb;
    if (per_cu > (uint64_t) per_cu_max) per_cu = (uint64_t) per_cu_max / (uint64_t) t.wpb * (uint64_t) t.wpb;
    return (uint64_t) n_cu * (per_cu? per_cu : (uint64_t) t.wpb);
}

static uint64_t ec_os_words(int32_t cap_c) { return ((uint64_t) ecw_words(cap_c) + 15) & ~15ULL; }

static void ec_set_caps(EcwArgs &a, const EcTier &t) { a.cap_t = t.cap_t, a.cap_c = t.cap_c, a.cap_w = t.cap_w, a.cap_path = t.cap_path, a.cap_f = t.cap_f; }

template <int MODE, int WPB> static void ec_wave_launch(uint64_t waves, uint64_t lds, hipStream_t st, const EcwArgs &a)
{
    if (a.seq_qend) hipLaunchKernelGGL((ec_wave_kernel<MODE, WPB, true>), dim3((unsigned) ((waves + WPB - 1) / WPB)), dim3(64 * WPB), (unsigned) (WPB * lds), st, a);
    else hipLaunchKernelGGL((ec_wave_kernel<MODE, WPB>), dim3((unsigned) ((waves + WPB - 1) / WPB)), dim3(64 * WPB), (unsigned) (WPB * lds), st, a);
}
static void ec_launch_lds_tier(const EcTier &t, uint64_t waves, hipStream_t st, const EcwArgs &a)
{
    if (t.wpb > 1) {
        if (t.hybrid) ec_wave_launch<2, ECW_WPB>(waves, t.bytes, st, a);
        else ec_wave_launch<0, ECW_WPB>(waves, t.bytes, st, a);
    } else {
        if (t.hybrid) ec_wave_launch<2, 1>(waves, t.bytes, st, a);
        else ec_wave_launch<0, 1>(waves, t.bytes, st, a);
    }
}
template <int NW, int R> static void ec_heavy_launch(uint64_t wgs, uint64_t lds, hipStream_t st, const EcwArgs &a)
{
    if (a.seq_qend) hipLaunchKernelGGL((ec_heavy_kernel<NW, R, true>), dim3((unsigned) wgs), dim3(64 * NW), (unsigned) lds, st, a);
    else hipLaunchKernelGGL((ec_heavy_kernel<NW, R>), dim3((unsigned) wgs), dim3(64 * NW), (unsigned) lds, st, a);
}
template <int NW> static void ec_fused_launch(uint64_t wgs, uint64_t lds, hipStream_t st, const EcwArgs &a)
{
    if (a.seq_qend) hipLaunchKernelGGL((ec_fused_kernel<NW, true>), dim3((unsigned) wgs), dim3(64 * NW), (unsigned) lds, st, a);
    else hipLaunchKernelGGL((ec_fused_kernel<NW>), dim3((unsigned) wgs), dim3(64 * NW), (unsigned) lds, st, a);
}

static int ec_slab_buf(oatk_hip_ctx *ctx, EcState *e, int &k, uint64_t bytes, hipStream_t st, const char *who, const char *what, void **p)
{
    if (k >= 16) { ctx->err = std::string("EC solver: more launches of ") + who + " than slab buffers (internal)"; return OATK_E_STATE; }
    DevBuf &b = e->hyb_slabs[k++];
    if (!b.ensure(bytes, st)) { ctx->err = std::string("hipMalloc failed for ") + who + "'s " + what; return OATK_E_NOMEM; }
    *p = b.p;
    return OATK_OK;
}

static int ec_fork_side_streams(oatk_hip_ctx *ctx, EcState *e)
{
    if (!e->aux[0]) {
        int pr_least = 0, pr_greatest = 0;
        CK(hipDeviceGetStreamPriorityRange(&pr_least, &pr_greatest));
        for (int i = 0; i < 5; ++i) { CK(hipStreamCreateWithPriority(&e->aux[i], hipStreamNonBlocking, i < 4? pr_greatest : pr_least)); CK(hipEventCreateWithFlags(&e->aux_ev[i], hipEventDisableTiming)); }
        CK(hipEventCreateWithFlags(&e->fork_ev, hipEventDisableTiming));
    }
    CK(hipEventRecord(e->fork_ev, ctx->stream));
    return OATK_OK;
}

static int ec_route(oatk_hip_ctx *ctx, EcState *e, uint64_t n_work, const EcRoute &rt, unsigned long long *routed, size_t bytes)
{
    hipLaunchKernelGGL(ec_route_kernel, dim3((unsigned) ((n_work + 256 * ECW_ROUTE_ITEMS - 1) / (256 * ECW_ROUTE_ITEMS))), dim3(256), 0, ctx->stream, e->work.as<EcWork>(), n_work, rt);
    CK(hipMemcpyAsync(routed, rt.cnt[0], bytes, hipMemcpyDeviceToHost, ctx->stream));
    CK(hipStreamSynchronize(ctx->stream));
    return OATK_OK;
}

static int ec_sort_longest_first(oatk_hip_ctx *ctx, EcState *e, uint32_t *list, uint64_t n)
{
    uint32_t *k_in = e->todo2.as<uint32_t>(), *k_out = k_in + (n + 1), *v_out = k_out + (n + 1);
    hipLaunchKernelGGL(ec_route_keys_kernel, dim3((unsigned) ((n + 255) / 256)), dim3(256), 0, ctx->stream, e->work.as<EcWork>(), list, n, k_in);
    size_t tb = 0;
    CK(rocprim::radix_sort_pairs(nullptr, tb, k_in, k_out, list, v_out, n, 0, 32, ctx->stream));
    ENSURE(tmp, tb);
    CK(rocprim::radix_sort_pairs(ctx->tmp.p, tb, k_in, k_out, list, v_out, n, 0, 32, ctx->stream));
    CK(hipMemcpyAsync(list, v_out, n * 4, hipMemcpyDeviceToDevice, ctx->stream));
    return OATK_OK;
}

static int ec_launch_slab_tier(oatk_hip_ctx *ctx, EcState *e, const EcwArgs &base, uint32_t &max_hl, const uint32_t *todo, uint64_t n_todo,
                               unsigned long long *queue, hipStream_t st)
{
    if (max_hl == 0) {
        std::vector<uint32_t> hl(ctx->n_reads);
        CK(hipMemcpy(hl.data(), ctx->hoco_l.p, ctx->n_reads * 4, hipMemcpyDeviceToHost));
        for (uint64_t i = 0; i < ctx->n_reads; ++i) if (hl[i] > max_hl) max_hl = hl[i];
    }
    EcwArgs a = base;
    a.cap_t = (int32_t) max_hl + 64, a.cap_c = ec_cap_c(a.cap_t, ctx->K);
    a.cap_w = 2 * ((int32_t) (max_hl * base.max_edist) + 16) + 16, a.cap_path = ec_cap_c((int32_t) max_hl, ctx->K), a.cap_f = 1 << 22;
    a.todo = todo, a.n_todo = n_todo, a.next = queue, a.skip_l = 0x7FFFFFFF, a.batch = 1;
    a.todo_out = e->todo2.as<uint32_t>(), a.todo_cnt = base.pool_cursor + 63;
    a.slab_bytes = ((uint64_t) ecw_scratch_words(a.cap_t, a.cap_c, a.cap_w, a.cap_path, a.cap_f) * 4 + 63) & ~63ULL;
    uint64_t waves = todo? n_todo : base.n_work;
    if (waves > 1024) waves = 1024;
    if (!waves) return OATK_OK;
    EENSURE(big_slabs, waves * a.slab_bytes);
    a.slabs = e->big_slabs.as<uint8_t>();
    ec_wave_launch<1, 1>(waves, 0, st, a);
    return OATK_OK;
}

static int ec_second_stage(oatk_hip_ctx *ctx, EcState *e, const EcKnobs &kn, const EcwArgs &base, uint32_t *todo, uint64_t nh, uint32_t *todo_out,
                           int &qslot, int &hyb_k, unsigned long long &left)
{
    unsigned long long *cur = base.pool_cursor;
    struct timespec ts0, ts1;
    if (kn.stages) clock_gettime(CLOCK_MONOTONIC, &ts0);
    if (nh > 1 && nh <= (4u << 20)) {
        if (3 * (nh + 1) > base.n_work + 1) EENSURE(todo2, 3 * (nh + 1) * 4);
        int rc = ec_sort_longest_first(ctx, e, todo, nh); if (rc) return rc;
    }
    const int NCLS = 5;
// ... 512 lines not shown
```

### oatk_amd/csrc/api_multi.inc

```
#include "../../include/oatk_hip_multi.h"
#include <dlfcn.h>
#include <pthread.h>
#include <time.h>
#include <unistd.h>
#include <rccl/rccl.h>
#include <rocprim/device/device_select.hpp>

namespace {

struct RcclApi {
    void *lib = nullptr;
    ncclResult_t (*GetUniqueId)(ncclUniqueId *) = nullptr;
    ncclResult_t (*CommInitRank)(ncclComm_t *, int, ncclUniqueId, int) = nullptr;
    ncclResult_t (*CommDestroy)(ncclComm_t) = nullptr;
    ncclResult_t (*CommAbort)(ncclComm_t) = nullptr;
    ncclResult_t (*AllGather)(const void *, void *, size_t, ncclDataType_t, ncclComm_t, hipStream_t) = nullptr;
    ncclResult_t (*AllReduce)(const void *, void *, size_t, ncclDataType_t, ncclRedOp_t, ncclComm_t, hipStream_t) = nullptr;
    ncclResult_t (*Broadcast)(const void *, void *, size_t, ncclDataType_t, int, ncclComm_t, hipStream_t) = nullptr;
    ncclResult_t (*Send)(const void *, size_t, ncclDataType_t, int, ncclComm_t, hipStream_t) = nullptr;
    ncclResult_t (*Recv)(void *, size_t, ncclDataType_t, int, ncclComm_t, hipStream_t) = nullptr;
    ncclResult_t (*GroupStart)() = nullptr;
    ncclResult_t (*GroupEnd)() = nullptr;
    const char *(*GetErrorString)(ncclResult_t) = nullptr;
    ncclResult_t (*CommGetAsyncError)(ncclComm_t, ncclResult_t *) = nullptr;
// ... 586 lines not shown
    const int n = c->n, me = c->rank;
    int rc;
    MENSURE(bad, 64); MENSURE(plan_d, 130 * 8);
    CK(hipMemsetAsync(m->bad.p, 0, 64, ctx->stream));

    uint64_t key[65] = {0};
    for (int r = 0; r < n; ++r) key[r] = (uint64_t) ((((unsigned __int128) (uint64_t) r << 64) + (uint64_t) (n - 1)) / (uint64_t) n);
    CK(hipMemcpyAsync(m->plan_d.as<uint64_t>() + 65, key, sizeof(key), hipMemcpyHostToDevice, ctx->stream));
    hipLaunchKernelGGL(mg_bounds_kernel, dim3(1), dim3(128), 0, ctx->stream, ctx->scm_h.as<uint64_t>(), nl, n, m->plan_d.as<uint64_t>());
    CK(hipMemcpyAsync(m->send_off, m->plan_d.p, (size_t) (n + 1) * 8, hipMemcpyDeviceToHost, ctx->stream));
    CK(hipStreamSynchronize(ctx->stream));
    uint64_t largest = 0;
    if ((rc = comm_plan(ctx, c, m->send_off, m->recv_off, &largest)) != OATK_OK) return rc;
    const uint64_t nr = m->recv_off[n];
    if (largest >= 0x7FFFFFFFULL) {
        c->agreed = true;
        ctx->err = "an owner's part of the merged table is too large for 32-bit indices";
        return OATK_E_ARG;
    }
    MENSURE(recv_h, (nr + 1) * 8); MENSURE(recv_s, (nr + 1) * 8); MENSURE(recv_cov, (nr + 1) * 4);
    {
        const void *out3[3] = {ctx->scm_h.p, ctx->scm_s.p, ctx->scm_cov.p};
        void *in3[3] = {m->recv_h.p, m->recv_s.p, m->recv_cov.p};
        const uint32_t w3[3] = {8, 8, 4};
        if ((rc = comm_exchange_multi(ctx, c, 3, out3, m->send_off, in3, m->recv_off, w3)) != OATK_OK) return rc;
    }

    uint64_t n_own = 0;
    MENSURE(srt_h, (nr + 1) * 8); MENSURE(srt_i, (nr + 1) * 4); MENSURE(iota, (nr + 1) * 4); MENSURE(flag, (nr + 1) * 4); MENSURE(grp, (nr + 1) * 4); MENSURE(grp_of, (nr + 1) * 4);
    MENSURE(own_h, (nr + 1) * 8); MENSURE(own_s, (nr + 1) * 8); MENSURE(own_cov, (nr + 1) * 4); MENSURE(reply, (nr + 1) * 8);
    MENSURE(need_j, (nr + 1) * 4); MENSURE(pos_of_j, (nr + 2) * 4); MENSURE(rep, (nr + 1) * 4); MENSURE(clhead, (nr + 1) * 4); MENSURE(req_j, (nr + 1) * 4); MENSURE(req_k, (nr + 1) * 4);
    MENSURE(need8, nr + 8);
    uint64_t n_req = 0, req_off[65] = {0}, asked_off[65] = {0};
    const int nw = (ctx->K + 31) / 32;
    CK(hipMemsetAsync(m->need_j.p, 0, (nr + 1) * 4, ctx->stream));
    if (nr) {
        hipLaunchKernelGGL(mg_iota_kernel, blocks(nr), dim3(256), 0, ctx->stream, m->iota.as<uint32_t>(), nr);
        size_t tb = 0;
        CK(rocprim::radix_sort_pairs(nullptr, tb, m->recv_h.as<uint64_t>(), m->srt_h.as<uint64_t>(), m->iota.as<uint32_t>(), m->srt_i.as<uint32_t>(), nr, 0, 64, ctx->stream));
        ENSURE(tmp, tb);
        CK(rocprim::radix_sort_pairs(ctx->tmp.p, tb, m->recv_h.as<uint64_t>(), m->srt_h.as<uint64_t>(), m->iota.as<uint32_t>(), m->srt_i.as<uint32_t>(), nr, 0, 64, ctx->stream));
        hipLaunchKernelGGL(mg_heads_kernel, blocks(nr), dim3(256), 0, ctx->stream, m->srt_h.as<uint64_t>(), m->srt_i.as<uint32_t>(), nr, m->flag.as<uint32_t>(), m->need_j.as<uint32_t>());
        tb = 0;
        CK(rocprim::exclusive_scan(nullptr, tb, m->need_j.as<uint32_t>(), m->pos_of_j.as<uint32_t>(), 0u, nr + 1, rocprim::plus<uint32_t>(), ctx->stream));
        ENSURE(tmp, tb);
        CK(rocprim::exclusive_scan(ctx->tmp.p, tb, m->need_j.as<uint32_t>(), m->pos_of_j.as<uint32_t>(), 0u, nr + 1, rocprim::plus<uint32_t>(), ctx->stream));
        uint32_t nq = 0;
        CK(hipMemcpyAsync(&nq, m->pos_of_j.as<uint32_t>() + nr, 4, hipMemcpyDeviceToHost, ctx->stream));
        CK(hipStreamSynchronize(ctx->stream));
        n_req = nq;
        if (n_req) {
            hipLaunchKernelGGL(mg_narrow8_kernel, blocks(nr), dim3(256), 0, ctx->stream, m->need_j.as<uint32_t>(), nr, m->need8.as<uint8_t>());
            uint64_t chk = 0;
            if ((rc = mg_select_u32(ctx, m, m->iota.as<uint32_t>(), m->need8.as<uint8_t>(), nr, m->req_j, &chk)) != OATK_OK) return rc;
        }
    }
    CK(hipMemcpyAsync(m->plan_d.as<uint64_t>(), m->recv_off, 65 * 8, hipMemcpyHostToDevice, ctx->stream));
    if (n_req) {
        hipLaunchKernelGGL(mg_req_bounds_kernel, dim3(1), dim3(128), 0, ctx->stream, m->req_j.as<uint32_t>(), n_req, m->plan_d.as<uint64_t>(), n, m->plan_d.as<uint64_t>() + 65);
        hipLaunchKernelGGL(mg_req_kernel, blocks(n_req), dim3(256), 0, ctx->stream, m->req_j.as<uint32_t>(), n_req, m->plan_d.as<uint64_t>(), n, m->req_k.as<uint32_t>());
        CK(hipMemcpyAsync(req_off, m->plan_d.as<uint64_t>() + 65, (size_t) (n + 1) * 8, hipMemcpyDeviceToHost, ctx->stream));
        CK(hipStreamSynchronize(ctx->stream));
    }
    if ((rc = comm_plan(ctx, c, req_off, asked_off)) != OATK_OK) return rc;
    const uint64_t n_asked = asked_off[n];
    MENSURE(asked, (n_asked + 1) * 4); MENSURE(lid, (n_asked + 1) * 4); MENSURE(seq_out, (n_asked + 1) * (size_t) nw * 8); MENSURE(seq_in, (n_req + 1) * (size_t) nw * 8);
    if ((rc = comm_exchange(ctx, c, m->req_k.p, req_off, m->asked.p, asked_off, 4)) != OATK_OK) return rc;
    if (n_asked) {
        CK(hipMemcpyAsync(m->plan_d.as<uint64_t>(), m->send_off, 65 * 8, hipMemcpyHostToDevice, ctx->stream));
        CK(hipMemcpyAsync(m->plan_d.as<uint64_t>() + 65, asked_off, 65 * 8, hipMemcpyHostToDevice, ctx->stream));
        hipLaunchKernelGGL(mg_asked_ids_kernel, blocks(n_asked), dim3(256), 0, ctx->stream, m->asked.as<uint32_t>(), n_asked, m->plan_d.as<uint64_t>(), m->plan_d.as<uint64_t>() + 65, n,
                           m->lid.as<uint32_t>());
        hipLaunchKernelGGL(mg_export_kmers_kernel, dim3((unsigned) n_asked), dim3(64), 0, ctx->stream, m->lid.as<uint32_t>(), n_asked, ctx->scm_occ_off.as<uint64_t>(),
                           ctx->scm_occ.as<uint64_t>(), ctx->sid0, ctx->d_off, ctx->scm_off.as<uint64_t>(), ctx->pos_mpos.as<uint32_t>(), ctx->hoco_s.as<uint8_t>(), ctx->K, nw,
                           m->seq_out.as<uint64_t>());
    }
    if ((rc = comm_exchange(ctx, c, m->seq_out.p, asked_off, m->seq_in.p, req_off, (uint32_t) nw * 8u)) != OATK_OK) return rc;
    if (nr) {
        hipLaunchKernelGGL(mg_cluster_kernel, blocks(nr), dim3(256), 0, ctx->stream, m->flag.as<uint32_t>(), m->srt_i.as<uint32_t>(), nr, m->need_j.as<uint32_t>(), m->pos_of_j.as<uint32_t>(),
                           m->seq_in.as<uint64_t>(), nw, m->recv_s.as<uint64_t>(), m->rep.as<uint32_t>(), m->clhead.as<uint32_t>(), m->bad.as<uint32_t>() + 1);
        size_t tb = 0;
        CK(rocprim::inclusive_scan(nullptr, tb, m->clhead.as<uint32_t>(), m->grp.as<uint32_t>(), nr, rocprim::plus<uint32_t>(), ctx->stream));
        ENSURE(tmp, tb);
        CK(rocprim::inclusive_scan(ctx->tmp.p, tb, m->clhead.as<uint32_t>(), m->grp.as<uint32_t>(), nr, rocprim::plus<uint32_t>(), ctx->stream));
        CK(hipMemsetAsync(m->own_cov.p, 0, (nr + 1) * 4, ctx->stream));
        hipLaunchKernelGGL(mg_groups_kernel, blocks(nr), dim3(256), 0, ctx->stream, m->srt_h.as<uint64_t>(), m->srt_i.as<uint32_t>(), m->grp.as<uint32_t>(), m->rep.as<uint32_t>(),
                           m->recv_s.as<uint64_t>(), m->recv_cov.as<uint32_t>(), nr, m->own_h.as<uint64_t>(), m->own_s.as<uint64_t>(), m->own_cov.as<uint32_t>(), m->grp_of.as<uint32_t>());
        hipLaunchKernelGGL(mg_reply_kernel, blocks(nr), dim3(256), 0, ctx->stream, m->grp_of.as<uint32_t>(), m->own_cov.as<uint32_t>(), nr, m->reply.as<uint64_t>());
        uint32_t last = 0;
        CK(hipMemcpyAsync(&last, m->grp.as<uint32_t>() + (nr - 1), 4, hipMemcpyDeviceToHost, ctx->stream));
        CK(hipStreamSynchronize(ctx->stream));
        n_own = last;
    }
    uint32_t bad[2] = {0, 0};
    CK(hipMemcpyAsync(bad, m->bad.p, 8, hipMemcpyDeviceToHost, ctx->stream));
    CK(hipStreamSynchronize(ctx->stream));
    uint64_t mine2[2] = {(uint64_t) (bad[1]? 1 : 0), n_own}, all2[128], worst = 0, ng = 0;
    if ((rc = comm_allgather_vec(ctx, c, mine2, 2, all2)) != OATK_OK) return rc;
    for (int r = 0; r < n; ++r) { worst = all2[2 * r] > worst? all2[2 * r] : worst; m->first_id[r] = ng; ng += all2[2 * r + 1]; }
    m->first_id[n] = ng;
    if (worst == 1) { c->agreed = true; ctx->err = "identical k-mers with different s-mers across shards (syncmer.c:1370: fatal in the reference)"; return OATK_E_SMER; }
    if (ng >= 0x7FFFFFFFULL) { c->agreed = true; ctx->err = "merged syncmer table too large for 32-bit ids"; return OATK_E_ARG; }

    MENSURE(back, (nl + 1) * 8); MENSURE(l2g, (nl + 1) * 4); MENSURE(lcov, (nl + 1) * 4);
    if ((rc = comm_exchange(ctx, c, m->reply.p, m->recv_off, m->back.p, m->send_off, 8)) != OATK_OK) return rc;
    CK(hipMemcpyAsync(m->plan_d.p, m->send_off, 65 * 8, hipMemcpyHostToDevice, ctx->stream));
    CK(hipMemcpyAsync(m->plan_d.as<uint64_t>() + 65, m->first_id, 65 * 8, hipMemcpyHostToDevice, ctx->stream));
    if (nl) hipLaunchKernelGGL(mg_l2g_kernel, blocks(nl), dim3(256), 0, ctx->stream, m->back.as<uint64_t>(), nl, m->plan_d.as<uint64_t>(), n, m->l2g.as<uint32_t>(), m->lcov.as<uint32_t>());
    CK(hipStreamSynchronize(ctx->stream));
    CK(hipGetLastError());
    (void) me;
    m->n_global = ng, m->n_owned = n_own, m->merged = true;
    if (n_global) *n_global = ng;
    return OATK_OK;
}

extern "C" int oatk_hip_merge_counts(oatk_hip_ctx *ctx, oatk_comm *c, uint64_t *n_global)
{
    if (!ctx) return OATK_E_NODEV;
    if (!c) { ctx->err = "oatk_hip_merge_counts: no communicator"; return OATK_E_ARG; }
    return comm_finish(c, merge_counts_impl(ctx, c, n_global));
}

extern "C" int oatk_hip_multi_range(oatk_hip_ctx *ctx, uint64_t *first_id, uint64_t *n_owned, uint64_t *n_global)
{
    if (!ctx) return OATK_E_NODEV;
    if (!ctx->multi || !ctx->multi->merged) { ctx->err = "oatk_hip_multi_range before oatk_hip_merge_counts"; return OATK_E_STATE; }
    if (first_id) *first_id = ctx->multi->first_id[ctx->multi->rank];
    if (n_owned) *n_owned = ctx->multi->n_owned;
    if (n_global) *n_global = ctx->multi->n_global;
    return OATK_OK;
}


__global__ void mg_need_flag_kernel(const uint8_t *err_del, const uint64_t *src, uint64_t n, uint8_t *flag, int nothing)
{
    const uint64_t i = (uint64_t) blockIdx.x * blockDim.x + threadIdx.x;
    if (i < n) flag[i] = !nothing && err_del[i] == 0 && src[i] == EC_NO_SRC;
}
__global__ void mg_owner_kernel(const uint32_t *ids, uint64_t n, const uint64_t *src, uint32_t rank, uint32_t nobody, uint32_t *owner)
{
    const uint64_t i = (uint64_t) blockIdx.x * blockDim.x + threadIdx.x;
    if (i < n) owner[i] = src[ids[i]] != EC_NO_SRC? rank : nobody;
}
__global__ void mg_eq_flag_kernel(const uint32_t *v, uint64_t n, uint32_t what, uint8_t *flag, uint32_t *any_left, uint32_t nobody)
{
    const uint64_t i = (uint64_t) blockIdx.x * blockDim.x + threadIdx.x;
    if (i >= n) return;
    flag[i] = v[i] == what;
    if (v[i] == nobody) *any_left = 1u;
}
__global__ void mg_need_cand_kernel(const uint32_t *cand, uint64_t n, const uint8_t *err_del, const uint64_t *src, uint8_t *flag, int nothing)
{
    const uint64_t i = (uint64_t) blockIdx.x * blockDim.x + threadIdx.x;
    if (i < n) flag[i] = !nothing && err_del[cand[i]] == 0 && src[cand[i]] == EC_NO_SRC;
}
__global__ void mg_lack_kernel(const uint32_t *ids, uint64_t n, const uint64_t *src, uint8_t *flag, int nothing)
{
    const uint64_t i = (uint64_t) blockIdx.x * blockDim.x + threadIdx.x;
    if (i < n) flag[i] = !nothing && src[ids[i]] == EC_NO_SRC;
}
__global__ void mg_rows_kernel(const uint8_t *in, const uint32_t *rows, uint64_t n, uint32_t stride, uint8_t *out)
{
    const uint64_t i = blockIdx.x;
    if (i >= n) return;
    const uint4 *a = (const uint4 *) (in + (uint64_t) rows[i] * stride);
    uint4 *b = (uint4 *) (out + i * stride);
    for (uint32_t t = threadIdx.x; t < stride / 16; t += blockDim.x) b[t] = a[t];
}
template <class T>
__global__ void mg_scatter_kernel(const uint32_t *ids, const T *val, uint64_t n, T *dense)
{
    const uint64_t i = (uint64_t) blockIdx.x * blockDim.x + threadIdx.x;
    if (i < n) dense[ids[i]] = val[i];
}
__global__ void mg_cand_flag_kernel(const uint32_t *cov, uint64_t n, uint32_t c, uint8_t *flag)
{
    const uint64_t i = (uint64_t) blockIdx.x * blockDim.x + threadIdx.x;
    if (i < n) flag[i] = cov[i] >= c;
}
__global__ void mg_cand_emit_kernel(const uint32_t *idx, uint64_t n, uint32_t first, const uint32_t *own_cov, const uint64_t *own_s, uint32_t *ids, uint32_t *cov, uint64_t *s)
{
    const uint64_t i = (uint64_t) blockIdx.x * blockDim.x + threadIdx.x;
    if (i < n) ids[i] = first + idx[i], cov[i] = own_cov[idx[i]], s[i] = own_s[idx[i]];
}
__global__ void mg_other_pack_kernel(const uint32_t *cand, uint64_t n2, const uint8_t *other, uint8_t *packed)
{
    const uint64_t j = (uint64_t) blockIdx.x * blockDim.x + threadIdx.x;
    if (j < n2) packed[j] = other[(uint64_t) cand[j >> 1] << 1 | (j & 1ULL)];
}
__global__ void mg_other_unpack_kernel(const uint32_t *cand, uint64_t n2, const uint8_t *packed, uint8_t *other)
{
    const uint64_t j = (uint64_t) blockIdx.x * blockDim.x + threadIdx.x;
    if (j < n2) other[(uint64_t) cand[j >> 1] << 1 | (j & 1ULL)] = packed[j] != 0;
}
__global__ void mg_pack_cand_kernel(const uint32_t *cand, uint64_t nc, const uint32_t *cov, const uint32_t *fwd, uint32_t *pc)
{
    const uint64_t i = (uint64_t) blockIdx.x * blockDim.x + threadIdx.x;
    if (i < nc) pc[i] = cov[cand[i]], pc[nc + i] = fwd[cand[i]];
}
__global__ void mg_local_contrib_kernel(const uint32_t *l2g, uint64_t nl, const uint32_t *gcov, uint32_t c, const uint32_t *cov, const uint32_t *fwd, uint32_t *lc, uint32_t *lf)
{
    const uint64_t j = (uint64_t) blockIdx.x * blockDim.x + threadIdx.x;
    if (j >= nl) return;
    const uint32_t g = l2g[j];
    const bool cand = gcov[g] >= c;
    lc[j] = cand? 0u : cov[g], lf[j] = cand? 0u : fwd[g];
}
__global__ void mg_owner_add_kernel(const uint32_t *grp_of, uint64_t n, const uint32_t *rc, const uint32_t *rf, uint32_t *ec_cov, uint32_t *ec_fwd)
{
    const uint64_t j = (uint64_t) blockIdx.x * blockDim.x + threadIdx.x;
    if (j >= n) return;
    if (rc[j]) atomicAdd(&ec_cov[grp_of[j]], rc[j]);
    if (rf[j]) atomicAdd(&ec_fwd[grp_of[j]], rf[j]);
}
__global__ void mg_owner_cand_kernel(const uint32_t *cand, uint64_t nc, const uint32_t *pc, uint32_t first, uint32_t n_owned, uint32_t *ec_cov, uint32_t *ec_fwd)
{
    const uint64_t i = (uint64_t) blockIdx.x * blockDim.x + threadIdx.x;
    if (i >= nc) return;
    const uint32_t g = cand[i];
    if (g >= first && g - first < n_owned) ec_cov[g - first] = pc[i], ec_fwd[g - first] = pc[nc + i];
}
__global__ void mg_del_kernel(const uint32_t *fwd, uint64_t n, uint8_t *del)
{
    const uint64_t i = (uint64_t) blockIdx.x * blockDim.x + threadIdx.x;
    if (i < n) del[i] = fwd[i] == 0;
}

static int mg_select_u32(oatk_hip_ctx *ctx, MultiState *m, const uint32_t *in, const uint8_t *flag, uint64_t n, DevBuf &out, uint64_t *n_out)
{
    *n_out = 0;
    if (!out.ensure((n + 1) * 4, ctx->stream)) { ctx->err = "hipMalloc failed (select)"; return OATK_E_NOMEM; }
    if (n == 0) return OATK_OK;
    MENSURE(num, (64 * 65 + 64) * 8);
    uint64_t *d_cnt = m->num.as<uint64_t>() + 64 * 65 + 8;
    size_t tb = 0;
    CK(rocprim::select(nullptr, tb, in, flag, out.as<uint32_t>(), d_cnt, n, ctx->stream));
    ENSURE(tmp, tb);
    CK(rocprim::select(ctx->tmp.p, tb, in, flag, out.as<uint32_t>(), d_cnt, n, ctx->stream));
    CK(hipMemcpyAsync(n_out, d_cnt, 8, hipMemcpyDeviceToHost, ctx->stream));
    CK(hipStreamSynchronize(ctx->stream));
    return OATK_OK;
}

static int ec_sharded_impl(oatk_hip_ctx *ctx, oatk_comm *c, double max_edist, uint32_t err_mer_c, uint32_t max_err_c, uint32_t err_arc_c,
                           double max_arc_f, uint64_t *stats12, uint64_t *n_imported)
{
    using namespace oatk;
    int rc;
    if ((rc = comm_check(ctx, c, "oatk_hip_ec_sharded")) != OATK_OK) return rc;
    if (!ctx->counted) { ctx->err = "oatk_hip_ec_sharded needs a resident scan + count"; return OATK_E_STATE; }
    CK(hipSetDevice(ctx->device));
    if (!ctx->multi || !ctx->multi->merged) { if ((rc = merge_counts_impl(ctx, c, nullptr)) != OATK_OK) return rc; }
    MultiState *m = ctx->multi;
    m->ec_done = false, m->table_root = -1;
    auto blocks = [](uint64_t n) { return dim3((unsigned) ((n + 255) / 256 > 0? (n + 255) / 256 : 1)); };
    const uint64_t ng = m->n_global, nl = ctx->n_scm_total, no = m->n_owned;
    const uint32_t first_me = (uint32_t) m->first_id[c->rank];
    const int nothing = ctx->n_occ == 0;
    if (n_imported) *n_imported = 0;
    const bool light = err_mer_c > 0 && err_arc_c >= err_mer_c && max_err_c >= err_mer_c && !getenv("OATK_DEBUG_FULL_GRAPH");

    MENSURE(gcov, (ng + 1) * 4); MENSURE(S, (ng + 1) * 8); MENSURE(flag, (no > ng? no : ng) + 8); MENSURE(iota, ((no > ng? no : ng) + 1) * 4);
    CK(hipMemsetAsync(m->gcov.p, 0, (ng + 1) * 4, ctx->stream));
    CK(hipMemsetAsync(m->S.p, 0, (ng + 1) * 8, ctx->stream));
    uint64_t nc = 0;
    if (light) {
        uint64_t nc_me = 0, chk = 0;
        hipLaunchKernelGGL(mg_iota_kernel, blocks(no), dim3(256), 0, ctx->stream, m->iota.as<uint32_t>(), no);
        hipLaunchKernelGGL(mg_cand_flag_kernel, blocks(no), dim3(256), 0, ctx->stream, m->own_cov.as<uint32_t>(), no, err_mer_c, m->flag.as<uint8_t>());
        if ((rc = mg_select_u32(ctx, m, m->iota.as<uint32_t>(), m->flag.as<uint8_t>(), no, m->opack, &nc_me)) != OATK_OK) return rc;
        MENSURE(cand_mine, (nc_me + 1) * 4); MENSURE(ccov_mine, (nc_me + 1) * 4); MENSURE(cs_mine, (nc_me + 1) * 8);
        if (nc_me) hipLaunchKernelGGL(mg_cand_emit_kernel, blocks(nc_me), dim3(256), 0, ctx->stream, m->opack.as<uint32_t>(), nc_me, first_me, m->own_cov.as<uint32_t>(),
                                      m->own_s.as<uint64_t>(), m->cand_mine.as<uint32_t>(), m->ccov_mine.as<uint32_t>(), m->cs_mine.as<uint64_t>());
        {
            const void *src3[3] = {m->cand_mine.p, m->ccov_mine.p, m->cs_mine.p};
            DevBuf *dst3[3] = {&m->cand, &m->cand_cov, &m->cand_s};
            const uint32_t w3[3] = {4, 4, 8};
            if ((rc = comm_gather_items_multi(ctx, c, 3, src3, w3, dst3, nc_me, &nc)) != OATK_OK) return rc;
            (void) chk;
        }
        if (nc) {
            hipLaunchKernelGGL(mg_scatter_kernel<uint32_t>, blocks(nc), dim3(256), 0, ctx->stream, m->cand.as<uint32_t>(), m->cand_cov.as<uint32_t>(), nc, m->gcov.as<uint32_t>());
            hipLaunchKernelGGL(mg_scatter_kernel<uint64_t>, blocks(nc), dim3(256), 0, ctx->stream, m->cand.as<uint32_t>(), m->cand_s.as<uint64_t>(), nc, m->S.as<uint64_t>());
        }
    } else {
        uint64_t cnt[64], bytes[64];
        if ((rc = comm_allgather_u64(ctx, c, no, cnt)) != OATK_OK) return rc;
        for (int r = 0; r < c->n; ++r) bytes[r] = cnt[r] * 4;
        if ((rc = comm_allgatherv(ctx, c, m->own_cov.p, bytes, m->gcov.p)) != OATK_OK) return rc;
        for (int r = 0; r < c->n; ++r) bytes[r] = cnt[r] * 8;
        if ((rc = comm_allgatherv(ctx, c, m->own_s.p, bytes, m->S.p)) != OATK_OK) return rc;
    }
    m->n_cand = nc;
    if (nl) {
        hipLaunchKernelGGL(mg_scatter_kernel<uint32_t>, blocks(nl), dim3(256), 0, ctx->stream, m->l2g.as<uint32_t>(), m->lcov.as<uint32_t>(), nl, m->gcov.as<uint32_t>());
        hipLaunchKernelGGL(mg_scatter_kernel<uint64_t>, blocks(nl), dim3(256), 0, ctx->stream, m->l2g.as<uint32_t>(), ctx->scm_s.as<uint64_t>(), nl, m->S.as<uint64_t>());
    }

    if ((rc = oatk_hip_ec_set_global(ctx, ng, m->l2g.as<uint32_t>(), m->gcov.as<uint32_t>(), m->S.as<uint64_t>())) != OATK_OK) return rc;
    uint64_t np_all = 0;
    if (light) {
        EcState *e = ctx->ec;
        const uint64_t *lk = nullptr;
        const uint32_t *ld = nullptr;
        uint64_t nk = 0, n_seg = 0;
        if ((rc = ec_light_pairs(ctx, err_mer_c, &lk, &ld, &nk)) != OATK_OK) return rc;
        EENSURE(g_keys2, (nk + 1) * 8); EENSURE(g_dist2, (nk + 1) * 4); EENSURE(g_head, nk + 8); EENSURE(g_hpos, (nk + 1) * 4); EENSURE(g_iota, (nk + 1) * 4);
        if (nk) {
            size_t tb = 0;
            CK(rocprim::radix_sort_pairs(nullptr, tb, const_cast<uint64_t *>(lk), e->g_keys2.as<uint64_t>(), const_cast<uint32_t *>(ld), e->g_dist2.as<uint32_t>(), nk, 0, 64, ctx->stream));
            ENSURE(tmp, tb);
            CK(rocprim::radix_sort_pairs(ctx->tmp.p, tb, const_cast<uint64_t *>(lk), e->g_keys2.as<uint64_t>(), const_cast<uint32_t *>(ld), e->g_dist2.as<uint32_t>(), nk, 0, 64, ctx->stream));
            hipLaunchKernelGGL(egr_seg_head_kernel, blocks(nk), dim3(256), 0, ctx->stream, nk, e->g_keys2.as<uint64_t>(), e->g_dist2.as<uint32_t>(), e->g_head.as<uint8_t>());
            hipLaunchKernelGGL(mg_iota_kernel, blocks(nk), dim3(256), 0, ctx->stream, e->g_iota.as<uint32_t>(), nk);
            if ((rc = ec_select(ctx, e, e->g_iota.as<uint32_t>(), e->g_head.as<uint8_t>(), nk, e->g_hpos.as<uint32_t>(), &n_seg)) != OATK_OK) return rc;
        }
        EENSURE(g_segk, (n_seg + 1) * 8); EENSURE(g_segv, (n_seg + 1) * 8);
        if (n_seg) hipLaunchKernelGGL(egr_seg_emit_kernel, blocks(n_seg), dim3(256), 0, ctx->stream, n_seg, nk, e->g_hpos.as<uint32_t>(), e->g_keys2.as<uint64_t>(),
                                      e->g_dist2.as<uint32_t>(), e->g_segk.as<uint64_t>(), e->g_segv.as<uint64_t>());
        {
            const void *src2[2] = {e->g_segk.p, e->g_segv.p};
            DevBuf *dst2[2] = {&m->keys_all, &m->dist_all};
            const uint32_t w2[2] = {8, 8};
            if ((rc = comm_gather_items_multi(ctx, c, 2, src2, w2, dst2, n_seg, &np_all)) != OATK_OK) return rc;
        }
        rc = ec_graph_build(ctx, m->keys_all.as<uint64_t>(), nullptr, m->dist_all.as<uint64_t>(), np_all, true);
    } else {
        const void *d_keys = nullptr, *d_dist = nullptr;
        uint64_t np = 0;
        if ((rc = oatk_hip_ec_pairs(ctx, &d_keys, &d_dist, &np)) != OATK_OK) return rc;
        {
            const void *src2[2] = {d_keys, d_dist};
            DevBuf *dst2[2] = {&m->keys_all, &m->dist_all};
            const uint32_t w2[2] = {8, 4};
            if ((rc = comm_gather_items_multi(ctx, c, 2, src2, w2, dst2, np, &np_all)) != OATK_OK) return rc;
        }
        rc = oatk_hip_ec_graph_from_pairs(ctx, m->keys_all.as<uint64_t>(), m->dist_all.as<uint32_t>(), np_all);
    }
    int rc_graph = rc;
    if (light) {
        EcState *e = ctx->ec;
        if (nc) {
            const uint64_t words = (2 * nc + 3) / 4;
            MENSURE(opack, words * 4 + 16);
            CK(hipMemsetAsync(m->opack.p, 0, words * 4, ctx->stream));
            if (!rc_graph) hipLaunchKernelGGL(mg_other_pack_kernel, blocks(2 * nc), dim3(256), 0, ctx->stream, m->cand.as<uint32_t>(), 2 * nc, e->g_other.as<uint8_t>(), m->opack.as<uint8_t>());
            if ((rc = comm_allreduce(ctx, c, m->opack.p, words, false, false)) != OATK_OK) return rc;
            if (!rc_graph) hipLaunchKernelGGL(mg_other_unpack_kernel, blocks(2 * nc), dim3(256), 0, ctx->stream, m->cand.as<uint32_t>(), 2 * nc, m->opack.as<uint8_t>(), e->g_other.as<uint8_t>());
        }
        if (!rc_graph) e->light_c = err_mer_c;
    }
    if (!rc_graph) rc_graph = oatk_hip_ec_mark(ctx, err_mer_c, max_err_c, err_arc_c, max_arc_f);
    EcState *e = ctx->ec;

    uint64_t n_need = 0, n_need_all = 0, nu = 0;
    if (rc_graph) {
        MENSURE(need, 64);
    } else if (light) {
        MENSURE(flag, (nc > ng? nc : ng) + 8);
        if (nc) hipLaunchKernelGGL(mg_need_cand_kernel, blocks(nc), dim3(256), 0, ctx->stream, m->cand.as<uint32_t>(), nc, (const uint8_t *) e->err_del.p,
                                   e->vtx_hs_off.as<uint64_t>(), m->flag.as<uint8_t>(), nothing);
        if ((rc = mg_select_u32(ctx, m, m->cand.as<uint32_t>(), m->flag.as<uint8_t>(), nc, m->need, &n_need)) != OATK_OK) return rc;
    } else {
        MENSURE(flag, ng + 8); MENSURE(iota, (ng + 1) * 4);
        hipLaunchKernelGGL(mg_iota_kernel, blocks(ng), dim3(256), 0, ctx->stream, m->iota.as<uint32_t>(), ng);
        hipLaunchKernelGGL(mg_need_flag_kernel, blocks(ng), dim3(256), 0, ctx->stream, (const uint8_t *) e->err_del.p, e->vtx_hs_off.as<uint64_t>(), ng, m->flag.as<uint8_t>(), nothing);
        if ((rc = mg_select_u32(ctx, m, m->iota.as<uint32_t>(), m->flag.as<uint8_t>(), ng, m->need, &n_need)) != OATK_OK) return rc;
    }
    {
        const void *src1[1] = {m->need.p};
        DevBuf *dst1[1] = {&m->need_all};
        const uint32_t w1[1] = {4};
        uint64_t verdict[64];
        if ((rc = comm_gather_items_multi(ctx, c, 1, src1, w1, dst1, n_need, &n_need_all, (uint64_t) (uint32_t) rc_graph, verdict)) != OATK_OK) return rc;
        for (int r = 0; r < c->n; ++r)
            if (verdict[r]) {
                c->agreed = true;
                if (!rc_graph) ctx->err = "EC graph: refused on rank " + std::to_string(r);
                return rc_graph? rc_graph : (int) (int32_t) (uint32_t) verdict[r];
            }
    }
    if (n_need_all) {
        MENSURE(need_srt, (n_need_all + 1) * 4); MENSURE(uni, (n_need_all + 1) * 4); MENSURE(num, (64 * 65 + 64) * 8);
        size_t tb = 0;
        CK(rocprim::radix_sort_keys(nullptr, tb, m->need_all.as<uint32_t>(), m->need_srt.as<uint32_t>(), n_need_all, 0, 32, ctx->stream));
        ENSURE(tmp, tb);
        CK(rocprim::radix_sort_keys(ctx->tmp.p, tb, m->need_all.as<uint32_t>(), m->need_srt.as<uint32_t>(), n_need_all, 0, 32, ctx->stream));
        uint64_t *d_cnt = m->num.as<uint64_t>() + 64 * 65 + 9;
        tb = 0;
        CK(rocprim::unique(nullptr, tb, m->need_srt.as<uint32_t>(), m->uni.as<uint32_t>(), d_cnt, n_need_all, rocprim::equal_to<uint32_t>(), ctx->stream));
        ENSURE(tmp, tb);
        CK(rocprim::unique(ctx->tmp.p, tb, m->need_srt.as<uint32_t>(), m->uni.as<uint32_t>(), d_cnt, n_need_all, rocprim::equal_to<uint32_t>(), ctx->stream));
        CK(hipMemcpyAsync(&nu, d_cnt, 8, hipMemcpyDeviceToHost, ctx->stream));
        CK(hipStreamSynchronize(ctx->stream));
    }
    if (nu) {
        const uint32_t nobody = (uint32_t) c->n;
        MENSURE(owner, (nu + 1) * 4); MENSURE(bad, 64);
        hipLaunchKernelGGL(mg_owner_kernel, blocks(nu), dim3(256), 0, ctx->stream, m->uni.as<uint32_t>(), nu, e->vtx_hs_off.as<uint64_t>(), (uint32_t) c->rank, nobody, m->owner.as<uint32_t>());
        if ((rc = comm_allreduce(ctx, c, m->owner.p, nu, false, true)) != OATK_OK) return rc;
        CK(hipMemsetAsync(m->bad.p, 0, 64, ctx->stream));
        MENSURE(flag, (nu > ng? nu : ng) + 8);
        hipLaunchKernelGGL(mg_eq_flag_kernel, blocks(nu), dim3(256), 0, ctx->stream, m->owner.as<uint32_t>(), nu, (uint32_t) c->rank, m->flag.as<uint8_t>(), m->bad.as<uint32_t>(), nobody);
        uint32_t orphan = 0;
        CK(hipMemcpyAsync(&orphan, m->bad.p, 4, hipMemcpyDeviceToHost, ctx->stream));
        uint64_t n_mine = 0;
        if ((rc = mg_select_u32(ctx, m, m->uni.as<uint32_t>(), m->flag.as<uint8_t>(), nu, m->mine, &n_mine)) != OATK_OK) return rc;
        if (orphan) { c->agreed = true; ctx->err = "sharded error correction: a live syncmer occurs on no shard"; return OATK_E_STATE; }
        const uint32_t stride = (uint32_t) (((ctx->K + 3) / 4 + 8 + 15) / 16 * 16);
        MENSURE(kout, (n_mine + 1) * (size_t) stride); MENSURE(krev, n_mine + 8);
        if ((rc = oatk_hip_ec_export_kmers(ctx, m->mine.as<uint32_t>(), n_mine, m->kout.as<uint8_t>(), stride, m->krev.as<uint8_t>())) != OATK_OK) return rc;
        uint64_t n_all = 0;
        {
            const void *src3[3] = {m->mine.p, m->krev.p, m->kout.p};
            DevBuf *dst3[3] = {&m->ids_all, &m->rev_all, &m->km_all};
            const uint32_t w3[3] = {4, 1, stride};
            if ((rc = comm_gather_items_multi(ctx, c, 3, src3, w3, dst3, n_mine, &n_all)) != OATK_OK) return rc;
        }
        MENSURE(flag, (n_all > ng? n_all : ng) + 8); MENSURE(iota, ((n_all > ng? n_all : ng) + 1) * 4);
        hipLaunchKernelGGL(mg_iota_kernel, blocks(n_all), dim3(256), 0, ctx->stream, m->iota.as<uint32_t>(), n_all);
        hipLaunchKernelGGL(mg_lack_kernel, blocks(n_all), dim3(256), 0, ctx->stream, m->ids_all.as<uint32_t>(), n_all, e->vtx_hs_off.as<uint64_t>(), m->flag.as<uint8_t>(), nothing);
        uint64_t n_imp = 0;
        if ((rc = mg_select_u32(ctx, m, m->iota.as<uint32_t>(), m->flag.as<uint8_t>(), n_all, m->lack, &n_imp)) != OATK_OK) return rc;
        if (n_imp) {
            MENSURE(ids_i, (n_imp + 1) * 4); MENSURE(rev_i, n_imp + 16); MENSURE(km_i, (n_imp + 1) * (size_t) stride);
            hipLaunchKernelGGL(mg_rows_kernel, dim3((unsigned) n_imp), dim3(64), 0, ctx->stream, m->km_all.as<uint8_t>(), m->lack.as<uint32_t>(), n_imp, stride, m->km_i.as<uint8_t>());
            uint64_t chk = 0;
            if ((rc = mg_select_u32(ctx, m, m->ids_all.as<uint32_t>(), m->flag.as<uint8_t>(), n_all, m->ids_i, &chk)) != OATK_OK) return rc;
            {
                uint64_t *d_cnt = m->num.as<uint64_t>() + 64 * 65 + 10;
                size_t tb = 0;
                CK(rocprim::select(nullptr, tb, m->rev_all.as<uint8_t>(), m->flag.as<uint8_t>(), m->rev_i.as<uint8_t>(), d_cnt, n_all, ctx->stream));
                ENSURE(tmp, tb);
                CK(rocprim::select(ctx->tmp.p, tb, m->rev_all.as<uint8_t>(), m->flag.as<uint8_t>(), m->rev_i.as<uint8_t>(), d_cnt, n_all, ctx->stream));
            }
            if ((rc = oatk_hip_ec_import_kmers(ctx, m->ids_i.as<uint32_t>(), m->rev_i.as<uint8_t>(), m->km_i.as<uint8_t>(), n_imp, stride)) != OATK_OK) return rc;
        }
        if (n_imported) *n_imported = n_imp;
    }

    rc = oatk_hip_ec_correct(ctx, max_edist);
    if ((rc = comm_agree(ctx, c, rc, "correction")) != OATK_OK) return rc;
    MENSURE(ec_cov, (no + 1) * 4); MENSURE(ec_fwd, (no + 1) * 4); MENSURE(ec_del, no + 8); MENSURE(st64, 16 * 8);
    CK(hipMemcpyAsync(m->st64.p, e->stats_h, 12 * 8, hipMemcpyHostToDevice, ctx->stream));
    if (light) {
        CK(hipMemsetAsync(m->ec_cov.p, 0, (no + 1) * 4, ctx->stream));
        CK(hipMemsetAsync(m->ec_fwd.p, 0, (no + 1) * 4, ctx->stream));
        MENSURE(pc, (2 * nc + 2) * 4); MENSURE(loc_c, (nl + 1) * 4); MENSURE(loc_f, (nl + 1) * 4);
        const uint64_t nr = m->recv_off[c->n];
        MENSURE(rcv_c, (nr + 1) * 4); MENSURE(rcv_f, (nr + 1) * 4);
        if (nc) hipLaunchKernelGGL(mg_pack_cand_kernel, blocks(nc), dim3(256), 0, ctx->stream, m->cand.as<uint32_t>(), nc, e->cov.as<uint32_t>(), e->fwd.as<uint32_t>(), m->pc.as<uint32_t>());
        if ((rc = comm_allreduce(ctx, c, m->pc.p, 2 * nc, false, false)) != OATK_OK) return rc;
        if (nl) hipLaunchKernelGGL(mg_local_contrib_kernel, blocks(nl), dim3(256), 0, ctx->stream, m->l2g.as<uint32_t>(), nl, m->gcov.as<uint32_t>(), err_mer_c, e->cov.as<uint32_t>(),
                                   e->fwd.as<uint32_t>(), m->loc_c.as<uint32_t>(), m->loc_f.as<uint32_t>());
        {
            const void *out2[2] = {m->loc_c.p, m->loc_f.p};
            void *in2[2] = {m->rcv_c.p, m->rcv_f.p};
            const uint32_t w2[2] = {4, 4};
            if ((rc = comm_exchange_multi(ctx, c, 2, out2, m->send_off, in2, m->recv_off, w2)) != OATK_OK) return rc;
        }
        if (nr) hipLaunchKernelGGL(mg_owner_add_kernel, blocks(nr), dim3(256), 0, ctx->stream, m->grp_of.as<uint32_t>(), nr, m->rcv_c.as<uint32_t>(), m->rcv_f.as<uint32_t>(),
                                   m->ec_cov.as<uint32_t>(), m->ec_fwd.as<uint32_t>());
        if (nc) hipLaunchKernelGGL(mg_owner_cand_kernel, blocks(nc), dim3(256), 0, ctx->stream, m->cand.as<uint32_t>(), nc, m->pc.as<uint32_t>(), first_me, (uint32_t) no,
                                   m->ec_cov.as<uint32_t>(), m->ec_fwd.as<uint32_t>());
    } else {
        MENSURE(loc_c, (ng + 1) * 4); MENSURE(loc_f, (ng + 1) * 4);
        CK(hipMemcpyAsync(m->loc_c.p, e->cov.p, ng * 4, hipMemcpyDeviceToDevice, ctx->stream));
        CK(hipMemcpyAsync(m->loc_f.p, e->fwd.p, ng * 4, hipMemcpyDeviceToDevice, ctx->stream));
        if ((rc = comm_allreduce(ctx, c, m->loc_c.p, ng, false, false)) != OATK_OK) return rc;
        if ((rc = comm_allreduce(ctx, c, m->loc_f.p, ng, false, false)) != OATK_OK) return rc;
        CK(hipMemcpyAsync(m->ec_cov.p, m->loc_c.as<uint32_t>() + first_me, no * 4, hipMemcpyDeviceToDevice, ctx->stream));
        CK(hipMemcpyAsync(m->ec_fwd.p, m->loc_f.as<uint32_t>() + first_me, no * 4, hipMemcpyDeviceToDevice, ctx->stream));
    }
    if ((rc = comm_allreduce(ctx, c, m->st64.p, 12, true, false)) != OATK_OK) return rc;
    hipLaunchKernelGGL(mg_del_kernel, blocks(no), dim3(256), 0, ctx->stream, m->ec_fwd.as<uint32_t>(), no, m->ec_del.as<uint8_t>());
    uint64_t st[12];
    CK(hipMemcpyAsync(st, m->st64.p, sizeof(st), hipMemcpyDeviceToHost, ctx->stream));
    CK(hipStreamSynchronize(ctx->stream));
    CK(hipGetLastError());
    if (stats12) memcpy(stats12, st, sizeof(st));
    m->ec_done = true;
    return OATK_OK;
}

extern "C" int oatk_hip_ec_sharded(oatk_hip_ctx *ctx, oatk_comm *c, double max_edist, uint32_t err_mer_c, uint32_t max_err_c, uint32_t err_arc_c,
                                   double max_arc_f, uint64_t *stats12, uint64_t *n_imported)
{
    if (!ctx) return OATK_E_NODEV;
    if (!c) { ctx->err = "oatk_hip_ec_sharded: no communicator"; return OATK_E_ARG; }
    return comm_finish(c, ec_sharded_impl(ctx, c, max_edist, err_mer_c, max_err_c, err_arc_c, max_arc_f, stats12, n_imported));
}
```

### oatk_amd/csrc/ecgraph.hpp

```cpp
#pragma once
#include "common.hpp"

namespace oatk {

#define EGR_INVALID 0xFFFFFFFFFFFFFFFFULL

__global__ void egr_pair_keys_kernel(uint64_t n_reads, const uint64_t *scm_off, const uint64_t *k_mer, const uint32_t *m_pos, uint64_t *keys, uint32_t *dist,
                                     int skip_corrected = 0)
{
    uint64_t r = (uint64_t) blockIdx.x * blockDim.x + threadIdx.x;
    if (r >= n_reads) return;
    const uint64_t o = scm_off[r], n = scm_off[r + 1] - o;
    if (n == 0) return;
    keys[o] = EGR_INVALID, dist[o] = 0;
    uint64_t v0 = (k_mer[o] >> 1) << 1 | (m_pos[o] & 1u);
    uint32_t p0 = m_pos[o] >> 1;
    for (uint64_t j = 1; j < n; ++j) {
        const uint64_t v1 = (k_mer[o + j] >> 1) << 1 | (m_pos[o + j] & 1u);
        const uint32_t p1 = m_pos[o + j] >> 1;
        keys[o + j] = skip_corrected && ((k_mer[o + j - 1] | k_mer[o + j]) & 1ULL)? EGR_INVALID : (v0 <= v1? v0 << 32 | v1 : (v1 ^ 1ULL) << 32 | (v0 ^ 1ULL));
        dist[o + j] = p1 - p0;
        v0 = v1, p0 = p1;
    }
}

__global__ __launch_bounds__(256) void egr_pair_light_wave_kernel(uint64_t n_reads, const uint64_t *scm_off, const uint64_t *k_mer, const uint32_t *m_pos, const uint32_t *cov,
                                                                  uint32_t c, uint64_t *keys, uint32_t *dist, uint8_t *keep, uint8_t *other)
{
    const uint64_t r = (uint64_t) blockIdx.x * 4 + (threadIdx.x >> 6);
    const int lane = threadIdx.x & 63;
    if (r >= n_reads) return;
    const uint64_t o = scm_off[r];
    const int64_t n = (int64_t) (scm_off[r + 1] - o);
    auto emit = [&](uint64_t at, uint64_t v0, uint32_t p0, uint64_t v1, uint32_t p1) {
        const bool c0 = cov[v0 >> 1] >= c, c1 = cov[v1 >> 1] >= c;
        const uint64_t a = v0 <= v1? v0 : v1 ^ 1ULL, b = v0 <= v1? v1 : v0 ^ 1ULL;
        keys[at] = a << 32 | b, dist[at] = p1 - p0, keep[at] = c0 && c1;
        const bool ca = v0 <= v1? c0 : c1, cb = v0 <= v1? c1 : c0;
        if (ca && !cb) other[a] = 1;
        if (cb && !ca) other[b ^ 1ULL] = 1;
    };
    if (n > 64) {
        if (lane == 0) {
            keys[o] = EGR_INVALID, dist[o] = 0, keep[o] = 0;
            uint64_t v0 = (k_mer[o] >> 1) << 1 | (m_pos[o] & 1u);
            uint32_t p0 = m_pos[o] >> 1;
            for (int64_t j = 1; j < n; ++j) {
                const uint64_t v1 = (k_mer[o + j] >> 1) << 1 | (m_pos[o + j] & 1u);
                const uint32_t p1 = m_pos[o + j] >> 1;
                emit(o + j, v0, p0, v1, p1);
                v0 = v1, p0 = p1;
            }
        }
        return;
    }
    const bool in = lane < n;
    const uint64_t km = in? k_mer[o + lane] : 0;
    const uint32_t mp = in? m_pos[o + lane] : 0;
    const uint64_t v1 = (km >> 1) << 1 | (mp & 1u);
    const uint32_t p1 = mp >> 1;
    const uint64_t v0 = (uint64_t) wave_prev((uint32_t) (v1 >> 32)) << 32 | wave_prev((uint32_t) v1);
    const uint32_t p0 = wave_prev(p1);
    if (in && lane == 0) keys[o] = EGR_INVALID, dist[o] = 0, keep[o] = 0;
    if (in && lane > 0) emit(o + lane, v0, p0, v1, p1);
}

__global__ void egr_seg_head_kernel(uint64_t n, const uint64_t *skeys, const uint32_t *sdist, uint8_t *head)
{
    const uint64_t i = (uint64_t) blockIdx.x * blockDim.x + threadIdx.x;
    if (i < n) head[i] = i == 0 || skeys[i] != skeys[i - 1] || sdist[i] != sdist[i - 1];
}
__global__ void egr_seg_emit_kernel(uint64_t n_seg, uint64_t n, const uint32_t *head_pos, const uint64_t *skeys, const uint32_t *sdist, uint64_t *okey, uint64_t *oval)
{
    const uint64_t i = (uint64_t) blockIdx.x * blockDim.x + threadIdx.x;
    if (i >= n_seg) return;
    const uint64_t p = head_pos[i], q = i + 1 < n_seg? head_pos[i + 1] : n;
    okey[i] = skeys[p], oval[i] = (uint64_t) sdist[p] | (q - p) << 32;
}
__global__ void egr_seg_split_kernel(uint64_t n, const uint64_t *val, uint32_t *dist, uint32_t *wgt)
{
    const uint64_t i = (uint64_t) blockIdx.x * blockDim.x + threadIdx.x;
    if (i < n) dist[i] = (uint32_t) val[i], wgt[i] = (uint32_t) (val[i] >> 32);
}

__global__ void egr_expand_count_kernel(uint64_t n_keys, const uint64_t *ukeys, uint32_t *n_out)
{
    uint64_t i = (uint64_t) blockIdx.x * blockDim.x + threadIdx.x;
    if (i >= n_keys) return;
    const uint64_t k = ukeys[i];
    if (k == EGR_INVALID) { n_out[i] = 0; return; }
    const uint64_t v0 = k >> 32, v1 = k & 0xFFFFFFFFULL;
    n_out[i] = (v1 ^ 1ULL) != v0? 2u : 1u;
}

__global__ void egr_expand_kernel(uint64_t n_keys, const uint64_t *ukeys, const uint32_t *counts, const uint32_t *run_ls, const uint64_t *out_off,
                                  uint64_t *akey, uint64_t *aval)
{
    uint64_t i = (uint64_t) blockIdx.x * blockDim.x + threadIdx.x;
    if (i >= n_keys) return;
    const uint64_t k = ukeys[i];
    if (k == EGR_INVALID) return;
    const uint64_t v0 = k >> 32, v1 = k & 0xFFFFFFFFULL, o = out_off[i];
    const uint64_t ls = (v1 ^ 1ULL) == v0? 0ULL : (uint64_t) run_ls[i];
    const uint64_t c = ls << 44 | (uint64_t) counts[i] << 1;
    akey[o] = k, aval[o] = c;
    if ((v1 ^ 1ULL) != v0) akey[o + 1] = (v1 ^ 1ULL) << 32 | (v0 ^ 1ULL), aval[o + 1] = c | 1ULL;
}

struct EgrArcs {
    uint64_t n_arc;
    uint64_t *arc_v, *arc_w;
    uint32_t *arc_ls, *arc_cov;
    uint8_t *arc_comp, *arc_del;
    uint64_t *idx_p;
    uint32_t *idx_n;
    uint32_t *flags;
};

__global__ void egr_unpack_kernel(EgrArcs a, const uint64_t *skey, const uint64_t *sval)
{
    uint64_t i = (uint64_t) blockIdx.x * blockDim.x + threadIdx.x;
    if (i >= a.n_arc) return;
    const uint64_t k = skey[i], v = k >> 32, w = k & 0xFFFFFFFFULL;
    a.arc_v[i] = v, a.arc_w[i] = w;
    a.arc_cov[i] = (uint32_t) (sval[i] >> 1);
    uint8_t comp = (uint8_t) (sval[i] & 1ULL);
    if ((w ^ 1ULL) == v) comp ^= 1;
    a.arc_comp[i] = comp, a.arc_del[i] = 0, a.arc_ls[i] = (uint32_t) (sval[i] >> 44);
    if (i && skey[i - 1] == k) a.flags[0] = 1u;
    if (i == 0 || (skey[i - 1] >> 32) != v) a.idx_p[v] = i;
    atomicAdd(&a.idx_n[v], 1u);
}

struct MiniKh {
    uint32_t bits, count;
    uint64_t used;
    int32_t keys[64], vals[64];
    bool overflow;

    __device__ static uint32_t h2b(uint32_t hash, uint32_t bits) { return (hash * 2654435769U) >> (32 - bits); }
    __device__ void init() { bits = 0, count = 0, used = 0, overflow = false; }
    __device__ uint32_t nb() const { return bits? 1U << bits : 0U; }
    __device__ void resize(uint32_t want)
    {
        uint32_t j = 0, x = want;
        while ((x >>= 1) != 0) ++j;
        if (want & (want - 1)) ++j;
        const uint32_t nbits = j > 2? j : 2;
        if (nbits > 6) { overflow = true; return; }
        const uint32_t n_old = nb(), n_new = 1U << nbits;
        uint64_t nused = 0;
        for (j = 0; j != n_old; ++j) {
            if (!((used >> j) & 1ULL)) continue;
            int32_t key = keys[j], val = vals[j];
            used &= ~(1ULL << j);
            for (;;) {
                uint32_t i = h2b((uint32_t) key, nbits);
                while ((nused >> i) & 1ULL) i = (i + 1) & (n_new - 1);
                nused |= 1ULL << i;
                if (i < n_old && ((used >> i) & 1ULL)) {
                    const int32_t tk = keys[i], tv = vals[i];
                    keys[i] = key, vals[i] = val, key = tk, val = tv;
                    used &= ~(1ULL << i);
                } else {
                    keys[i] = key, vals[i] = val;
                    break;
                }
            }
        }
        used = nused, bits = nbits;
    }
    __device__ void add1(int32_t key)
    {
        uint32_t n = nb();
        if (count >= (n >> 1) + (n >> 2)) { resize(n + 1U); if (overflow) return; n = nb(); }
        uint32_t i = h2b((uint32_t) key, bits);
        const uint32_t last = i;
        while (((used >> i) & 1ULL) && keys[i] != key) { i = (i + 1U) & (n - 1); if (i == last) break; }
        if (!((used >> i) & 1ULL)) keys[i] = key, vals[i] = 1, used |= 1ULL << i, ++count;
        else ++vals[i];
    }
    __device__ void addw(int32_t key, uint32_t w)
    {
        add1(key);
        if (w < 2 || overflow) return;
        add1(key);
        if (w < 3 || overflow) return;
        const uint32_t n = nb();
        uint32_t i = h2b((uint32_t) key, bits);
        while (keys[i] != key || !((used >> i) & 1ULL)) i = (i + 1U) & (n - 1);
        vals[i] += (int32_t) (w - 2);
    }
    __device__ int32_t mode() const
    {
        int32_t movl = 0, mcnt = 0;
        for (uint32_t k = 0; k < nb(); ++k) if (((used >> k) & 1ULL) && vals[k] > mcnt) mcnt = vals[k], movl = keys[k];
        return movl;
    }
};

struct WaveKh {
    int32_t *keys, *vals;
    uint64_t used;
    uint32_t bits, count;
    bool overflow;

    __device__ void init(int32_t *k, int32_t *v) { keys = k, vals = v, used = 0, bits = 0, count = 0, overflow = false; }
    __device__ uint32_t nb() const { return bits? 1U << bits : 0U; }
    __device__ bool due() const { const uint32_t n = nb(); return count >= (n >> 1) + (n >> 2); }
    __device__ void resize(uint32_t want)
    {
        uint32_t j = 0, x = want;
        while ((x >>= 1) != 0) ++j;
        if (want & (want - 1)) ++j;
        const uint32_t nbits = j > 2? j : 2;
        if (nbits > 6) { overflow = true; return; }
        const uint32_t n_old = nb(), n_new = 1U << nbits;
        uint64_t nused = 0;
        for (j = 0; j != n_old; ++j) {
            if (!((used >> j) & 1ULL)) continue;
            int32_t key = keys[j], val = vals[j];
            used &= ~(1ULL << j);
            for (;;) {
                uint32_t i = MiniKh::h2b((uint32_t) key, nbits);
                while ((nused >> i) & 1ULL) i = (i + 1) & (n_new - 1);
                nused |= 1ULL << i;
                if (i < n_old && ((used >> i) & 1ULL)) {
                    const int32_t tk = keys[i], tv = vals[i];
                    keys[i] = key, vals[i] = val, key = tk, val = tv;
                    used &= ~(1ULL << i);
                } else {
                    keys[i] = key, vals[i] = val;
                    break;
                }
            }
        }
        used = nused, bits = nbits;
    }
    __device__ bool add(int32_t key, int32_t cnt)
    {
        for (int pass = 0; pass < 2; ++pass) {
            uint32_t n = nb(), i = 0;
            bool found = false;
            if (n) {
                i = MiniKh::h2b((uint32_t) key, bits);
                const uint32_t last = i;
                while (((used >> i) & 1ULL) && keys[i] != key) { i = (i + 1U) & (n - 1); if (i == last) break; }
                found = (used >> i) & 1ULL;
            }
            if (due()) {
                resize(n + 1U);
                if (overflow) return false;
                continue;
            }
            if (found) { vals[i] += cnt; return false; }
            keys[i] = key, vals[i] = cnt, used |= 1ULL << i, ++count;
            return true;
        }
        return false;
    }
    __device__ int32_t mode() const
    {
        int32_t movl = 0, mcnt = 0;
        for (uint32_t k = 0; k < nb(); ++k) if (((used >> k) & 1ULL) && vals[k] > mcnt) mcnt = vals[k], movl = keys[k];
        return movl;
    }
};

#define EGR_SMALL_RUN 48
#define EGR_HUGE_SCRATCH (256ull << 20)

__device__ __forceinline__ uint32_t egr_to_ls(int64_t l, int K)
{
    if (l < K) l = l < 0? K : K - l;
    else l = 0;
    return (uint32_t) l;
}

__global__ __launch_bounds__(64) void egr_mode_kernel(uint64_t n_runs, const uint64_t *ukeys, const uint32_t *counts, const uint64_t *run_off,
                                                      const uint32_t *sdist, int K, uint32_t *run_ls, uint32_t *flags, uint32_t *big_list, uint32_t *huge_list,
                                                      const uint32_t *swgt = nullptr, uint32_t *run_cov = nullptr)
{
    const int lane = threadIdx.x;
    const uint64_t i = (uint64_t) blockIdx.x * 64 + lane;
    const bool valid = i < n_runs && ukeys[i] != EGR_INVALID;
    const uint32_t c = valid? counts[i] : 0u;
    const uint64_t o = valid? run_off[i] : 0;
    if (valid && c <= EGR_SMALL_RUN) {
        MiniKh h;
        h.init();
        if (swgt) {
            uint32_t tot = 0;
            for (uint32_t t = 0; t < c; ++t) h.addw((int32_t) sdist[o + t], swgt[o + t]), tot += swgt[o + t];
            run_cov[i] = tot;
        } else {
            for (uint32_t t = 0; t < c; ++t) h.add1((int32_t) sdist[o + t]);
        }
        if (h.overflow) huge_list[atomicAdd(&flags[5], 1u)] = (uint32_t) i;
        else run_ls[i] = egr_to_ls(h.mode(), K);
    }
    const bool is_big = valid && c > EGR_SMALL_RUN;
    const uint64_t big = __ballot(is_big);
    if (big) {
        uint32_t base = 0;
        if (lane == __builtin_ctzll(big)) base = atomicAdd(&flags[4], (uint32_t) __builtin_popcountll(big));
        base = wave_read(base, __builtin_ctzll(big));
        if (is_big) big_list[base + (uint32_t) __builtin_popcountll(big & ((1ULL << lane) - 1ULL))] = (uint32_t) i;
    }
}

__global__ __launch_bounds__(64) void egr_mode_big_kernel(const uint32_t *counts, const uint64_t *run_off, const uint32_t *sdist, int K, uint32_t *run_ls,
                                                          uint32_t *flags, const uint32_t *big_list, uint32_t *huge_list, const uint32_t *swgt = nullptr,
                                                          uint32_t *run_cov = nullptr)
{
    __shared__ int32_t tk[64], tv[64];
    const int lane = threadIdx.x;
    const uint32_t n_big = flags[4];
    for (uint32_t b = blockIdx.x; b < n_big; b += gridDim.x) {
        const uint32_t i = big_list[b];
        const uint32_t cc = counts[i];
        const uint64_t oo = run_off[i];
        WaveKh h;
        h.init(tk, tv);
        bool tail_new = false;
        uint32_t tot = 0;
        for (uint32_t t0 = 0; t0 < cc && !h.overflow; t0 += 64) {
            const bool in = t0 + lane < cc;
            const int32_t d = in? (int32_t) sdist[oo + t0 + lane] : 0;
            const uint32_t w = in? (swgt? swgt[oo + t0 + lane] : 1u) : 0u;
            uint64_t rest = __ballot(in);
            while (rest && !h.overflow) {
                const int f = __builtin_ctzll(rest);
                const int32_t x = (int32_t) wave_read((uint32_t) d, f);
                const uint64_t eq = __ballot(in && d == x) & rest;
                rest &= ~eq;
                uint32_t calls = (uint32_t) __builtin_popcountll(eq);
                const uint32_t wf = wave_read(w, f);
                if (swgt) {
                    calls = 0;
                    for (uint64_t q = eq; q; q &= q - 1) calls += wave_read(w, __builtin_ctzll(q));
                }
                tot += calls;
                const bool fresh = h.add(x, (int32_t) calls);
                tail_new = fresh && eq == (1ULL << f) && t0 + f == cc - 1 && wf == 1u;
            }
        }
        if (!h.overflow && h.due() && !tail_new) h.resize(h.nb() + 1U);
        if (lane == 0) {
            if (swgt && !h.overflow) run_cov[i] = tot;
            if (h.overflow) huge_list[atomicAdd(&flags[5], 1u)] = i;
            else run_ls[i] = egr_to_ls(h.mode(), K);
        }
        __syncthreads();
    }
}

struct BigKh {
    int32_t *keys, *vals;
    uint8_t *used, *nused;
    uint32_t cap, bits, count;
    bool overflow;

    __device__ uint32_t nb() const { return bits? 1U << bits : 0U; }
    __device__ void resize(uint32_t want)
    {
        uint32_t j = 0, x = want;
        while ((x >>= 1) != 0) ++j;
// ... 102 lines not shown
```

### oatk_amd/device.py

```python
import os
import ctypes as C

import numpy as np

from . import _lib

_DTYPES = {
    "HOCO_L": np.uint32, "N_SCM": np.uint32, "N_NN": np.uint32, "N_LRL": np.uint32, "HO_RL": np.uint8, "HOCO_S": np.uint8,
    "NN_KEY": np.uint64, "LRL_KEY": np.uint64, "LRL_VAL": np.uint32, "SCM_OFF": np.uint64, "POS_MPOS": np.uint32,
    "POS_SMER": np.uint64, "POS_HASH": np.uint64, "POS_KID": np.uint64, "SCM_H": np.uint64, "SCM_S": np.uint64,
    "SCM_COV": np.uint32, "SCM_OCC_OFF": np.uint64, "SCM_OCC": np.uint64,
    "EC_N_SCM": np.uint32, "EC_SCM_OFF": np.uint64, "EC_KMER": np.uint64, "EC_MPOS": np.uint32, "EC_SMER": np.uint64,
    "EC_SCM_COV": np.uint32, "EC_SCM_DEL": np.uint8, "EC_SCM_OCC_OFF": np.uint64, "EC_SCM_OCC": np.uint64, "EC_ERR_DEL": np.uint8,
    "EC_SCM_FWD": np.uint32, "EC_VTX_SRC": np.uint64, "EC_BLOCK_WORK": np.uint32, "EC_BLOCK_OUT": np.uint32,
    "EC_CSEQ_LEN": np.uint32, "EC_CSEQ_OFF": np.uint64, "EC_CSEQ": np.uint8, "EC_BLOCK_QEND": np.uint32,
    "INGEST_SEQ": np.uint8, "INGEST_OFF": np.uint64, "INGEST_LEN": np.uint32, "INGEST_HDR": np.uint64,
    "CONS_SEL": np.uint32, "CONS_SLOT": np.uint32, "CONS_RL": np.uint32, "CONS_MSEQ": np.uint32, "CONS_FIRST": np.uint64, "CONS_TOT": np.uint64,
    "EG_IDX_P": np.uint64, "EG_IDX_N": np.uint32, "EG_ARC_V": np.uint64, "EG_ARC_W": np.uint64, "EG_ARC_LS": np.uint32,
    "EG_ARC_COV": np.uint32, "EG_ARC_COMP": np.uint8,
    "RA_ALN_SID": np.uint32, "RA_ALN_OFF": np.uint64, "RA_ALN_S": np.float64, "RA_FRG_UID": np.uint64, "RA_FRG_UBEG": np.uint32,
    "RA_FRG_UEND": np.uint32, "RA_FRG_SBEG": np.uint32, "RA_FRG_SEND": np.uint32, "RA_SKIPPED": np.uint32,
    "OVL_KEY": np.uint64, "OVL_OFF": np.uint64, "OVL_DIST": np.int32, "OVL_CNT": np.uint32, "OVL_TAIL": np.uint8,
    "MG_G_H": np.uint64, "MG_G_S": np.uint64, "MG_G_COV": np.uint32, "MG_G_DEL": np.uint8, "MG_G_OCC_OFF": np.uint64, "MG_G_OCC": np.uint64, "MG_POS_GKID": np.uint64,
    "MG_H": np.uint64, "MG_S": np.uint64, "MG_COV": np.uint32, "MG_L2G": np.uint32, "MG_EC_COV": np.uint32, "MG_EC_DEL": np.uint8, "MG_LCOV": np.uint32,
    "AG_SCM_DEL": np.uint8, "AG_VTX_SCM": np.uint32, "AG_VTX_COV": np.uint32, "AG_IDX_P": np.uint64, "AG_IDX_N": np.uint32,
    "AG_ARC_V": np.uint64, "AG_ARC_W": np.uint64, "AG_ARC_COV": np.uint32, "AG_ARC_COMP": np.uint8, "AG_ARC_LINK": np.uint64,
}


def pack_reads(reads):
    n = len(reads)
    lens = np.fromiter((len(r) for r in reads), dtype=np.uint32, count=n)
    padded = (lens.astype(np.uint64) + (_lib.READ_ALIGN - 1)) // _lib.READ_ALIGN * _lib.READ_ALIGN
    off = np.zeros(n, dtype=np.uint64)
    if n > 1:
        off[1:] = np.cumsum(padded[:-1], dtype=np.uint64)
    total = int(padded.sum()) if n else 0
    seq = np.zeros(max(total, _lib.READ_ALIGN), dtype=np.uint8)
    for i, r in enumerate(reads):
        if len(r):
            seq[int(off[i]):int(off[i]) + len(r)] = np.frombuffer(r, dtype=np.uint8)
    return seq, off, lens


class HipSyncasm:

    def __init__(self, device=0):
        self.L = _lib.load()
        self.h = self.L.oatk_hip_create(device)
        if not self.h:
            raise _lib.OatkHipError("oatk_hip_create(%d) failed: no usable MI355X (gfx950) device" % device)
        self.device = device
        if os.environ.get("OATK_TEST_POOL"):
            self.mem_pool(int(os.environ["OATK_TEST_POOL"]))

    def mem_pool(self, warm_bytes=0):
        self._check(self.L.oatk_hip_mem_pool(self.h, warm_bytes), "oatk_hip_mem_pool")

    def close(self):
        if self.h:
            self.L.oatk_hip_destroy(self.h)
            self.h = None

    def __del__(self):
        try:
            self.close()
        except Exception:
            pass

    def _check(self, rc, what):
        if rc != _lib.OK:
            msg = self.L.oatk_hip_last_error(self.h)
            raise _lib.OatkHipError("%s failed (code %d): %s" % (what, rc, msg.decode() if msg else ""))

    def scan_host(self, seq, off, lens, k, s, sid0=0):
        seq = np.ascontiguousarray(seq, dtype=np.uint8)
        off = np.ascontiguousarray(off, dtype=np.uint64)
        lens = np.ascontiguousarray(lens, dtype=np.uint32)
        n = len(off)
        self._keep = (seq, off, lens)
        rc = self.L.oatk_hip_scan_host(self.h, seq.ctypes.data, off.ctypes.data if n else None, lens.ctypes.data if n else None,
                                       n, seq.size if n else 0, sid0, k, s)
        self._check(rc, "oatk_hip_scan_host")

    def scan_device(self, d_seq, d_off, d_len, n_reads, seq_bytes, k, s, sid0=0):
        rc = self.L.oatk_hip_scan(self.h, d_seq, d_off, d_len, n_reads, seq_bytes, sid0, k, s)
        self._check(rc, "oatk_hip_scan")

    def scan_begin(self, k, s, sid0=0):
        self._check(self.L.oatk_hip_scan_begin(self.h, sid0, k, s), "oatk_hip_scan_begin")

    def scan_reserve(self, seq_bytes, n_reads, n_occ):
        self._check(self.L.oatk_hip_scan_reserve(self.h, seq_bytes, n_reads, n_occ), "oatk_hip_scan_reserve")

    def scan_append(self, piece):
        self._check(self.L.oatk_hip_scan_append(self.h, piece.h), "oatk_hip_scan_append")

    def count(self):
        self._check(self.L.oatk_hip_count(self.h), "oatk_hip_count")

    def merge_counts(self, comm):
        n = C.c_uint64()
        self._check(self.L.oatk_hip_merge_counts(self.h, comm, C.byref(n)), "oatk_hip_merge_counts")
        return int(n.value)

    def multi_range(self):
        a, b, g = C.c_uint64(), C.c_uint64(), C.c_uint64()
        self._check(self.L.oatk_hip_multi_range(self.h, C.byref(a), C.byref(b), C.byref(g)), "oatk_hip_multi_range")
        return int(a.value), int(b.value), int(g.value)

    def ec_sharded(self, comm, max_edist, c, a, keep_seq=False):
        self.ec_keep_seq(keep_seq)
        st = np.zeros(12, np.uint64)
        ni = C.c_uint64()
        self._check(self.L.oatk_hip_ec_sharded(self.h, comm, max_edist, c, 10 * c, c, a, st.ctypes.data, C.byref(ni)), "oatk_hip_ec_sharded")
        return st, int(ni.value)

    def gather_table(self, comm, root=0):
        self._check(self.L.oatk_hip_gather_table(self.h, comm, root), "oatk_hip_gather_table")

    def asm_graph_sharded(self, comm, min_k_cov, min_a_cov_f):
        nv, na = C.c_uint64(), C.c_uint64()
        self._check(self.L.oatk_hip_asm_graph_sharded(self.h, comm, int(min_k_cov), float(min_a_cov_f), C.byref(nv), C.byref(na)), "oatk_hip_asm_graph_sharded")
        return int(nv.value), int(na.value)

    def consensus_sharded(self, comm, min_cov=1):
        self._check(self.L.oatk_hip_consensus_sharded(self.h, comm, int(min_cov)), "oatk_hip_consensus_sharded")

    def overlap_hist_sharded(self, comm, min_cov=0):
        np_, ne = C.c_uint64(), C.c_uint64()
        self._check(self.L.oatk_hip_overlap_hist_sharded(self.h, comm, int(min_cov), C.byref(np_), C.byref(ne)), "oatk_hip_overlap_hist_sharded")
        return int(np_.value), int(ne.value)

    def stat_sharded(self, comm):
        r = _lib.StatRaw()
        self._check(self.L.oatk_hip_stat_sharded(self.h, comm, C.byref(r)), "oatk_hip_stat_sharded")
        return self._stat_dict(r)

    def ra_utg_coverage_sharded(self, comm, graph, aln=None, chains=None, verbose=0):
        g, keep_g = self._racov_graph(graph)
        a, keep_a = self._racov_aln(aln)
        r = None
        if chains is not None:
            keep_r = [np.ascontiguousarray(chains[0], dtype=np.uint64), np.ascontiguousarray(chains[1], dtype=np.uint64)]
            r = _lib.RacovReads(len(keep_r[0]) - 1, keep_r[0].ctypes.data, keep_r[1].ctypes.data)
        out = np.zeros(max(g.n_utg, 1), np.float64)
        it = C.c_uint64(0)
        self._check(self.L.oatk_hip_ra_utg_coverage_sharded(self.h, comm, C.byref(g), None if r is None else C.byref(r), None if a is None else C.byref(a),
                                                            verbose, out.ctypes.data, C.byref(it)), "oatk_hip_ra_utg_coverage_sharded")
        return out[:g.n_utg], int(it.value)

    def ra_arc_coverage_sharded(self, comm, graph, aln=None):
        g, keep_g = self._racov_graph(graph)
        a, keep_a = self._racov_aln(aln)
        out = np.zeros(max(g.n_arc, 1), np.float64)
        self._check(self.L.oatk_hip_ra_arc_coverage_sharded(self.h, comm, C.byref(g), None if a is None else C.byref(a), out.ctypes.data),
                    "oatk_hip_ra_arc_coverage_sharded")
        return out[:g.n_arc]

    def ec_graph(self, light_c=0):
        if light_c:
            self._check(self.L.oatk_hip_ec_graph_light(self.h, int(light_c)), "oatk_hip_ec_graph_light")
        else:
            self._check(self.L.oatk_hip_ec_graph(self.h), "oatk_hip_ec_graph")

    def ec(self, max_edist, c, a, graph=None, keep_seq=False):
        self.ec_keep_seq(keep_seq)
        if graph is None:
            rc = self.L.oatk_hip_ec(self.h, None, max_edist, c, 10 * c, c, a)
        else:
            keep = {k: np.ascontiguousarray(graph[k], dtype=dt) for k, dt in
                    (("idx_p", np.uint64), ("idx_n", np.uint64), ("arc_v", np.uint64), ("arc_w", np.uint64), ("arc_ls", np.uint64),
                     ("arc_cov", np.uint32), ("arc_del", np.uint8))}
            g = _lib.EcGraph(int(graph["n_vtx"]), int(graph["n_arc"]), *[keep[k].ctypes.data for k in
                             ("idx_p", "idx_n", "arc_v", "arc_w", "arc_ls", "arc_cov", "arc_del")])
            rc = self.L.oatk_hip_ec(self.h, C.byref(g), max_edist, c, 10 * c, c, a)
        self._check(rc, "oatk_hip_ec")
        st = np.zeros(12, np.uint64)
        self._check(self.L.oatk_hip_ec_stats(self.h, st.ctypes.data), "oatk_hip_ec_stats")
        return st

    def wf_ed(self, jobs, wg=0):
        code = np.full(256, 255, np.uint8)
        for i, ch in enumerate(b"ACGT"):
            code[ch] = code[ch + 32] = i
        t_off, q_off, s_off = np.zeros(len(jobs) + 1, np.uint64), np.zeros(len(jobs) + 1, np.uint64), np.zeros(len(jobs) + 1, np.uint64)
        for j, (t, q, _, steps) in enumerate(jobs):
            t_off[j + 1], q_off[j + 1], s_off[j + 1] = t_off[j] + len(t), q_off[j] + len(q), s_off[j] + len(steps)
        tc = code[np.frombuffer(b"".join(j[0] for j in jobs), np.uint8)] if jobs else np.zeros(0, np.uint8)
        qc = code[np.frombuffer(b"".join(j[1] for j in jobs), np.uint8)] if jobs else np.zeros(0, np.uint8)
        if (tc == 255).any() or (qc == 255).any():
            raise ValueError("wf_ed: the device alphabet is the 2-bit one of sr_t.hoco_s (ACGT)")
        bw = np.array([j[2] for j in jobs], np.int32)
        ql = np.array([x for j in jobs for x in j[3]], np.int32)
        out = np.zeros((len(ql), 3), np.int32)
        tc, qc = np.ascontiguousarray(tc), np.ascontiguousarray(qc)
        if wg:
            self._check(self.L.oatk_hip_debug_wf_ed_wg(self.h, wg, len(jobs), tc.ctypes.data, t_off.ctypes.data, qc.ctypes.data, q_off.ctypes.data, bw.ctypes.data,
                                                       ql.ctypes.data, s_off.ctypes.data, out.ctypes.data), "oatk_hip_debug_wf_ed_wg")
        else:
            self._check(self.L.oatk_hip_debug_wf_ed(self.h, len(jobs), tc.ctypes.data, t_off.ctypes.data, qc.ctypes.data, q_off.ctypes.data, bw.ctypes.data,
                                                    ql.ctypes.data, s_off.ctypes.data, out.ctypes.data), "oatk_hip_debug_wf_ed")
        return [[tuple(int(v) for v in out[s]) for s in range(int(s_off[j]), int(s_off[j + 1]))] for j in range(len(jobs))]

    def tables(self, jobs):
        code = np.full(256, 255, np.uint8)
        for i, ch in enumerate(b"ACGT"):
            code[ch] = code[ch + 32] = i
        t_off, s_off, o_off = np.zeros(len(jobs) + 1, np.uint64), np.zeros(len(jobs) + 1, np.uint64), np.zeros(len(jobs) + 1, np.uint64)
        for j, (t, q) in enumerate(jobs):
            t_off[j + 1], s_off[j + 1], o_off[j + 1] = t_off[j] + len(t), s_off[j] + len(q), o_off[j] + 2 * (len(t) + 1)
        tc = np.ascontiguousarray(code[np.frombuffer(b"".join(j[0] for j in jobs), np.uint8)])
        sc = np.ascontiguousarray(code[np.frombuffer(b"".join(j[1] for j in jobs), np.uint8)])
        out = np.zeros(int(o_off[-1]), np.int32)
        self.L.oatk_hip_debug_tables.argtypes = [C.c_void_p] + [C.c_uint64] + [C.c_void_p] * 6
        self._check(self.L.oatk_hip_debug_tables(self.h, len(jobs), tc.ctypes.data, t_off.ctypes.data, sc.ctypes.data, s_off.ctypes.data, out.ctypes.data, o_off.ctypes.data), "oatk_hip_debug_tables")
        res = []
        for j, (t, _) in enumerate(jobs):
            a = int(o_off[j])
            res.append((out[a:a + len(t) + 1].copy(), out[a + len(t) + 1:a + 2 * (len(t) + 1)].copy()))
        return res

    def ed_ab(self, pairs, myers):
        code = np.full(256, 255, np.uint8)
        for i, ch in enumerate(b"ACGT"):
            code[ch] = code[ch + 32] = i
        n = len(pairs)
        t_off, q_off = np.zeros(n + 1, np.uint64), np.zeros(n + 1, np.uint64)
        t_off[1:] = np.cumsum([len(p[0]) for p in pairs])
        q_off[1:] = np.cumsum([len(p[1]) for p in pairs])
        tc = np.ascontiguousarray(code[np.frombuffer(b"".join(p[0] for p in pairs), np.uint8)])
        qc = np.ascontiguousarray(code[np.frombuffer(b"".join(p[1] for p in pairs), np.uint8)])
        if (tc == 255).any() or (qc == 255).any():
            raise ValueError("ed_ab: the device alphabet is ACGT")
        bw = np.array([p[2] for p in pairs], np.int32)
        out = np.zeros((n, 3), np.int32)
        ms = C.c_float()
        self._check(self.L.oatk_hip_debug_ed_ab(self.h, 1 if myers else 0, n, tc.ctypes.data, t_off.ctypes.data, qc.ctypes.data, q_off.ctypes.data, bw.ctypes.data,
                                                out.ctypes.data, C.byref(ms)), "oatk_hip_debug_ed_ab")
        return [tuple(int(v) for v in r) for r in out], float(ms.value)

    def ec_stats(self):
        st = np.zeros(12, np.uint64)
        self._check(self.L.oatk_hip_ec_stats(self.h, st.ctypes.data), "oatk_hip_ec_stats")
        return st

    def ec_keep_seq(self, on):
        self._check(self.L.oatk_hip_ec_keep_seq(self.h, 1 if on else 0), "oatk_hip_ec_keep_seq")

    def corrected_reads(self):
        n = C.c_uint64(0)
        self._check(self.L.oatk_hip_ec_corrected_reads(self.h, C.byref(n)), "oatk_hip_ec_corrected_reads")
        ln, off, packed = self.fetch("EC_CSEQ_LEN"), self.fetch("EC_CSEQ_OFF"), self.fetch("EC_CSEQ")
        assert int(ln.sum(dtype=np.uint64)) == n.value
        codes = np.stack([(packed >> s) & 3 for s in (6, 4, 2, 0)], axis=1).reshape(-1)
        text = np.frombuffer(b"ACGT", np.uint8)[codes]
        return [text[4 * int(o):4 * int(o) + int(l)].tobytes() for o, l in zip(off[:-1], ln)]

    def ec_mark(self, c, a):
        self._check(self.L.oatk_hip_ec_mark(self.h, c, 10 * c, c, a), "oatk_hip_ec_mark")

    def ec_correct(self, max_edist):
        self._check(self.L.oatk_hip_ec_correct(self.h, max_edist), "oatk_hip_ec_correct")
        return self.ec_stats()

    def ec_set_global(self, n_global, d_l2g, d_cov, d_s):
        self._check(self.L.oatk_hip_ec_set_global(self.h, n_global, d_l2g, d_cov, d_s), "oatk_hip_ec_set_global")

    def ec_pairs(self):
        k, d, n = C.c_void_p(), C.c_void_p(), C.c_uint64()
        self._check(self.L.oatk_hip_ec_pairs(self.h, C.byref(k), C.byref(d), C.byref(n)), "oatk_hip_ec_pairs")
        return k.value, d.value, int(n.value)

    def ec_graph_from_pairs(self, d_keys, d_dist, n):
        self._check(self.L.oatk_hip_ec_graph_from_pairs(self.h, d_keys, d_dist, n), "oatk_hip_ec_graph_from_pairs")

    def ec_export_kmers(self, d_ids, n, d_out, stride, d_rev):
        self._check(self.L.oatk_hip_ec_export_kmers(self.h, d_ids, n, d_out, stride, d_rev), "oatk_hip_ec_export_kmers")

    def ec_import_kmers(self, d_ids, d_rev, d_kmers, n, stride):
        self._check(self.L.oatk_hip_ec_import_kmers(self.h, d_ids, d_rev, d_kmers, n, stride), "oatk_hip_ec_import_kmers")

    def ingest_host(self, text, fmt=0, final=True):
        t = np.frombuffer(text, dtype=np.uint8) if isinstance(text, (bytes, bytearray, memoryview)) else np.ascontiguousarray(text, dtype=np.uint8)
        self._keep_text = t
        n, used = C.c_uint64(), C.c_uint64()
        self._check(self.L.oatk_hip_ingest_host(self.h, t.ctypes.data if t.size else None, t.size, fmt, 1 if final else 0, C.byref(n), C.byref(used)),
                    "oatk_hip_ingest_host")
        return int(n.value), int(used.value)

    def ingest_device(self, d_text, n_bytes, fmt=0, final=True):
        n, used = C.c_uint64(), C.c_uint64()
        self._check(self.L.oatk_hip_ingest(self.h, d_text, n_bytes, fmt, 1 if final else 0, C.byref(n), C.byref(used)), "oatk_hip_ingest")
        return int(n.value), int(used.value)

    def scan_ingested(self, k, s, sid0=0):
        self._check(self.L.oatk_hip_scan_ingested(self.h, sid0, k, s), "oatk_hip_scan_ingested")

    @staticmethod
    def _stat_dict(r):
        return {"n_reads": r.n_reads, "n_syncmers": r.n_syncmers, "sum_dist": r.sum_dist, "n_dist": r.n_dist, "smer_unique": r.smer_unique,
                "kmer_unique": r.kmer_unique, "smer_cnt": np.array(r.smer_cnt, np.int64), "kmer_cnt": np.array(r.kmer_cnt, np.int64),
                "smer_no_singleton": r.smer_no_singleton, "kmer_no_singleton": r.kmer_no_singleton}

    def stat_raw(self):
        r = _lib.StatRaw()
        self._check(self.L.oatk_hip_stat(self.h, C.byref(r)), "oatk_hip_stat")
        return self._stat_dict(r)

    def stat_keys(self):
        s, k, n = C.c_void_p(), C.c_void_p(), C.c_uint64()
        add4 = np.zeros(4, np.int64)
        self._check(self.L.oatk_hip_stat_keys(self.h, C.byref(s), C.byref(k), C.byref(n), add4.ctypes.data), "oatk_hip_stat_keys")
        return s.value, k.value, int(n.value), add4

    def stat_from_keys(self, d_smer, d_kkey, n, add4):
        r = _lib.StatRaw()
        a = np.ascontiguousarray(add4, dtype=np.int64)
        self._check(self.L.oatk_hip_stat_from_keys(self.h, d_smer, d_kkey, n, a.ctypes.data, C.byref(r)), "oatk_hip_stat_from_keys")
        return self._stat_dict(r)

    def consensus(self, min_cov=1):
# ... 198 lines not shown
```

Before: 378.3.

## Rank-compress light EC graph pair keys and use flat ballot-based compaction

The light EC graph pair generation moves from a per-read wave kernel to a flat per-occurrence kernel. It compacts kept pairs with wave ballots, a per-block count scan and a scatter kernel. Candidate vertices (coverage at or above the threshold) are rank-compressed so pair keys fit in fewer bits, often 32-bit. This shrinks the radix sort's key width and bit range and the run-length-encode cost, and unpacked keys are restored after the encode. It adds an extra scan and rank-table pass plus host syncs, and keeps the old path behind a debug environment variable.

```diff
diff --git a/include/oatk_hip_ec.h b/include/oatk_hip_ec.h
--- a/include/oatk_hip_ec.h
+++ b/include/oatk_hip_ec.h
@@ -62,7 +62,8 @@
 
 enum {
     OATK_BUF_EG_IDX_P = 120, OATK_BUF_EG_IDX_N, OATK_BUF_EG_ARC_V, OATK_BUF_EG_ARC_W, OATK_BUF_EG_ARC_LS, OATK_BUF_EG_ARC_COV,
-    OATK_BUF_EG_ARC_COMP
+    OATK_BUF_EG_ARC_COMP,
+    OATK_BUF_EG_OTHER
 };
 
 #ifdef __cplusplus
diff --git a/oatk_amd/_lib.py b/oatk_amd/_lib.py
--- a/oatk_amd/_lib.py
+++ b/oatk_amd/_lib.py
@@ -20,7 +20,7 @@
 BUF.update({name: 200 + i for i, name in enumerate(["RA_ALN_SID", "RA_ALN_OFF", "RA_ALN_S", "RA_FRG_UID", "RA_FRG_UBEG", "RA_FRG_UEND", "RA_FRG_SBEG", "RA_FRG_SEND", "RA_SKIPPED"])})
 BUF.update({name: 150 + i for i, name in enumerate(["OVL_KEY", "OVL_OFF", "OVL_DIST", "OVL_CNT", "OVL_TAIL"])})
 BUF.update({name: 120 + i for i, name in enumerate([
-    "EG_IDX_P", "EG_IDX_N", "EG_ARC_V", "EG_ARC_W", "EG_ARC_LS", "EG_ARC_COV", "EG_ARC_COMP"])})
+    "EG_IDX_P", "EG_IDX_N", "EG_ARC_V", "EG_ARC_W", "EG_ARC_LS", "EG_ARC_COV", "EG_ARC_COMP", "EG_OTHER"])})
 BUF.update({name: 180 + i for i, name in enumerate([
     "AG_SCM_DEL", "AG_VTX_SCM", "AG_VTX_COV", "AG_IDX_P", "AG_IDX_N", "AG_ARC_V", "AG_ARC_W", "AG_ARC_COV", "AG_ARC_COMP", "AG_ARC_LINK"])})
 BUF.update({name: 220 + i for i, name in enumerate(["MG_H", "MG_S", "MG_COV", "MG_L2G", "MG_EC_COV", "MG_EC_DEL", "MG_LCOV"])})
diff --git a/oatk_amd/csrc/api_ec.inc b/oatk_amd/csrc/api_ec.inc
--- a/oatk_amd/csrc/api_ec.inc
+++ b/oatk_amd/csrc/api_ec.inc
@@ -7,6 +7,7 @@
 #include "ec_seq.hpp"
 #include <rocprim/device/device_run_length_encode.hpp>
 #include <rocprim/device/device_select.hpp>
+#include <rocprim/iterator/counting_iterator.hpp>
 
 struct EcState {
     DevBuf idx_p, idx_n, arc_v, arc_w, arc_ls, arc_cov, arc_del, conv;
@@ -25,6 +26,7 @@
     DevBuf g_keys, g_keys2, g_ukeys, g_counts, g_nruns, g_nout, g_nout64, g_outoff, g_akey, g_aval, g_skey, g_sval, g_comp, g_flags, g_huge;
     DevBuf g_dist, g_dist2, g_cnt64, g_runoff, g_runls;
     DevBuf g_big, g_keep, g_other, g_lkeys, g_ldist, g_val2, g_wgt2, g_runcov, g_head, g_hpos, g_iota, g_segk, g_segv;
+    DevBuf g_first, g_kmask, g_bcnt, g_boff, g_rank, g_cand, g_pkeys;
     uint32_t light_c = 0;
     uint64_t g_n_vtx = 0, g_n_arc = 0;
     bool graph_resident = false;
@@ -52,6 +54,7 @@
                      &e->g_keys, &e->g_keys2, &e->g_ukeys, &e->g_counts, &e->g_nruns, &e->g_nout, &e->g_nout64, &e->g_outoff, &e->g_akey,
                      &e->g_aval, &e->g_skey, &e->g_sval, &e->g_comp, &e->g_flags, &e->g_huge, &e->g_dist, &e->g_dist2, &e->g_cnt64, &e->g_runoff, &e->g_runls,
                      &e->g_big, &e->g_keep, &e->g_other, &e->g_lkeys, &e->g_ldist, &e->g_val2, &e->g_wgt2, &e->g_runcov, &e->g_head, &e->g_hpos, &e->g_iota, &e->g_segk, &e->g_segv,
+                     &e->g_first, &e->g_kmask, &e->g_bcnt, &e->g_boff, &e->g_rank, &e->g_cand, &e->g_pkeys,
                      &e->g_l2g, &e->g_kid, &e->g_gcov, &e->g_gs,
                      &e->slot_w, &e->slot_w64, &e->slot_off, &e->slots, &e->qend, &e->sblk, &e->clen, &e->cbytes, &e->cbytes64, &e->coff, &e->cseq};
     for (DevBuf *b : all) b->release();
@@ -64,10 +67,12 @@
 static int ec_buffer(oatk_hip_ctx *ctx, int which, const void **d_ptr, uint64_t *bytes)
 {
     EcState *e = ctx->ec;
-    if (e && which >= OATK_BUF_EG_IDX_P && which <= OATK_BUF_EG_ARC_COMP) {
+    if (e && which >= OATK_BUF_EG_IDX_P && which <= OATK_BUF_EG_OTHER) {
         if (!e->graph_resident) { ctx->err = "EC graph requested before oatk_hip_ec_graph"; return OATK_E_STATE; }
+        if (which == OATK_BUF_EG_OTHER && !e->light_c) { ctx->err = "EG_OTHER: the resident EC graph is not a light one"; return OATK_E_STATE; }
         const uint64_t gv = e->g_n_vtx, ga = e->g_n_arc;
         switch (which) {
+            case OATK_BUF_EG_OTHER: *d_ptr = e->g_other.p, *bytes = 2 * gv; break;
             case OATK_BUF_EG_IDX_P: *d_ptr = e->idx_p.p, *bytes = 2 * gv * 8; break;
             case OATK_BUF_EG_IDX_N: *d_ptr = e->idx_n.p, *bytes = 2 * gv * 4; break;
             case OATK_BUF_EG_ARC_V: *d_ptr = e->arc_v.p, *bytes = ga * 8; break;
@@ -397,7 +402,13 @@
     return OATK_OK;
 }
 
-static int ec_graph_build(oatk_hip_ctx *ctx, const uint64_t *d_keys, const uint32_t *d_dist, const uint64_t *d_val, uint64_t nocc, bool timer_running = false)
+struct EgrKeyForm {
+    uint32_t kb = 0;
+    bool key32 = false;
+    bool all_bits = false;
+};
+static int ec_graph_build(oatk_hip_ctx *ctx, const void *d_keys, const uint32_t *d_dist, const uint64_t *d_val, uint64_t nocc, bool timer_running = false,
+                          EgrKeyForm form = EgrKeyForm())
 {
     using namespace oatk;
     if (!ctx) return OATK_E_NODEV;
@@ -421,30 +432,53 @@
     if (nocc) {
         EENSURE(g_keys2, (nocc + 1) * 8); EENSURE(g_ukeys, (nocc + 1) * 8); EENSURE(g_counts, (nocc + 1) * 4);
         EENSURE(g_nruns, 64); EENSURE(g_dist2, (nocc + 1) * 4);
-        uint64_t *keys_in = const_cast<uint64_t *>(d_keys);
+        uint64_t *keys_in = (uint64_t *) const_cast<void *>(d_keys);
         uint32_t *dist_in = const_cast<uint32_t *>(d_dist);
         size_t tb = 0;
-        if (weighted) {
+        unsigned id_bits = 1;
+        while (id_bits < 32 && (2 * nv - 1) >> id_bits) ++id_bits;
+        const unsigned end_bit = form.kb? 2 * form.kb : form.all_bits? 64u : 32u + id_bits;
+        if (form.kb && form.key32) {
+            uint32_t *k32 = (uint32_t *) keys_in;
+            EENSURE(g_pkeys, (nocc + 1) * 4);
+            CK(rocprim::radix_sort_pairs(nullptr, tb, k32, e->g_keys2.as<uint32_t>(), dist_in, e->g_dist2.as<uint32_t>(), nocc, 0, end_bit, ctx->stream));
+            ENSURE(tmp, tb);
+            CK(rocprim::radix_sort_pairs(ctx->tmp.p, tb, k32, e->g_keys2.as<uint32_t>(), dist_in, e->g_dist2.as<uint32_t>(), nocc, 0, end_bit, ctx->stream));
+        } else if (weighted) {
             EENSURE(g_val2, (nocc + 1) * 8); EENSURE(g_wgt2, (nocc + 1) * 4);
             uint64_t *val_in = const_cast<uint64_t *>(d_val);
-            CK(rocprim::radix_sort_pairs(nullptr, tb, keys_in, e->g_keys2.as<uint64_t>(), val_in, e->g_val2.as<uint64_t>(), nocc, 0, 64, ctx->stream));
+            CK(rocprim::radix_sort_pairs(nullptr, tb, keys_in, e->g_keys2.as<uint64_t>(), val_in, e->g_val2.as<uint64_t>(), nocc, 0, end_bit, ctx->stream));
             ENSURE(tmp, tb);
-            CK(rocprim::radix_sort_pairs(ctx->tmp.p, tb, keys_in, e->g_keys2.as<uint64_t>(), val_in, e->g_val2.as<uint64_t>(), nocc, 0, 64, ctx->stream));
+            CK(rocprim::radix_sort_pairs(ctx->tmp.p, tb, keys_in, e->g_keys2.as<uint64_t>(), val_in, e->g_val2.as<uint64_t>(), nocc, 0, end_bit, ctx->stream));
             hipLaunchKernelGGL(egr_seg_split_kernel, blocks(nocc), dim3(256), 0, ctx->stream, nocc, e->g_val2.as<uint64_t>(), e->g_dist2.as<uint32_t>(), e->g_wgt2.as<uint32_t>());
         } else {
-            CK(rocprim::radix_sort_pairs(nullptr, tb, keys_in, e->g_keys2.as<uint64_t>(), dist_in, e->g_dist2.as<uint32_t>(), nocc, 0, 64, ctx->stream));
+            CK(rocprim::radix_sort_pairs(nullptr, tb, keys_in, e->g_keys2.as<uint64_t>(), dist_in, e->g_dist2.as<uint32_t>(), nocc, 0, end_bit, ctx->stream));
             ENSURE(tmp, tb);
-            CK(rocprim::radix_sort_pairs(ctx->tmp.p, tb, keys_in, e->g_keys2.as<uint64_t>(), dist_in, e->g_dist2.as<uint32_t>(), nocc, 0, 64, ctx->stream));
+            CK(rocprim::radix_sort_pairs(ctx->tmp.p, tb, keys_in, e->g_keys2.as<uint64_t>(), dist_in, e->g_dist2.as<uint32_t>(), nocc, 0, end_bit, ctx->stream));
         }
         tb = 0;
-        CK(rocprim::run_length_encode(nullptr, tb, e->g_keys2.as<uint64_t>(), (unsigned int) nocc, e->g_ukeys.as<uint64_t>(), e->g_counts.as<uint32_t>(),
-                                      e->g_nruns.as<uint32_t>(), ctx->stream));
-        ENSURE(tmp, tb);
-        CK(rocprim::run_length_encode(ctx->tmp.p, tb, e->g_keys2.as<uint64_t>(), (unsigned int) nocc, e->g_ukeys.as<uint64_t>(), e->g_counts.as<uint32_t>(),
-                                      e->g_nruns.as<uint32_t>(), ctx->stream));
+        if (form.kb && form.key32) {
+            CK(rocprim::run_length_encode(nullptr, tb, e->g_keys2.as<uint32_t>(), (unsigned int) nocc, e->g_pkeys.as<uint32_t>(), e->g_counts.as<uint32_t>(),
+                                          e->g_nruns.as<uint32_t>(), ctx->stream));
+            ENSURE(tmp, tb);
+            CK(rocprim::run_length_encode(ctx->tmp.p, tb, e->g_keys2.as<uint32_t>(), (unsigned int) nocc, e->g_pkeys.as<uint32_t>(), e->g_counts.as<uint32_t>(),
+                                          e->g_nruns.as<uint32_t>(), ctx->stream));
+        } else {
+            CK(rocprim::run_length_encode(nullptr, tb, e->g_keys2.as<uint64_t>(), (unsigned int) nocc, e->g_ukeys.as<uint64_t>(), e->g_counts.as<uint32_t>(),
+                                          e->g_nruns.as<uint32_t>(), ctx->stream));
+            ENSURE(tmp, tb);
+            CK(rocprim::run_length_encode(ctx->tmp.p, tb, e->g_keys2.as<uint64_t>(), (unsigned int) nocc, e->g_ukeys.as<uint64_t>(), e->g_counts.as<uint32_t>(),
+                                          e->g_nruns.as<uint32_t>(), ctx->stream));
+        }
         uint32_t n_runs = 0;
         CK(hipMemcpyAsync(&n_runs, e->g_nruns.p, 4, hipMemcpyDeviceToHost, ctx->stream));
         CK(hipStreamSynchronize(ctx->stream));
+        if (form.kb && n_runs) {
+            if (form.key32) hipLaunchKernelGGL(egr_unpack_keys_kernel<uint32_t>, blocks(n_runs), dim3(256), 0, ctx->stream, (uint64_t) n_runs, (const uint32_t *) e->g_pkeys.p,
+                                               form.kb, (const uint32_t *) e->g_cand.p, e->g_ukeys.as<uint64_t>());
+            else hipLaunchKernelGGL(egr_unpack_keys_kernel<uint64_t>, blocks(n_runs), dim3(256), 0, ctx->stream, (uint64_t) n_runs, (const uint64_t *) e->g_ukeys.p,
+                                    form.kb, (const uint32_t *) e->g_cand.p, e->g_ukeys.as<uint64_t>());
+        }
         EENSURE(g_nout, ((uint64_t) n_runs + 1) * 4);
         hipLaunchKernelGGL(egr_expand_count_kernel, blocks(n_runs), dim3(256), 0, ctx->stream, (uint64_t) n_runs, e->g_ukeys.as<uint64_t>(), e->g_nout.as<uint32_t>());
         { int rc = ec_exclusive_scan_u32(ctx, e, e->g_nout, e->g_nout64, e->g_outoff, n_runs, &na); if (rc) return rc; }
@@ -535,25 +569,34 @@
     return OATK_OK;
 }
 
-static int ec_light_pairs(oatk_hip_ctx *ctx, uint32_t c, const uint64_t **d_keys, const uint32_t **d_dist, uint64_t *n_keep)
+static int ec_light_keys_debug()
+{
+    const char *v = getenv("OATK_DEBUG_EC_LIGHT_KEYS");
+    return v && !strcmp(v, "0")? 0 : v && !strcmp(v, "64")? 64 : -1;
+}
+
+static int ec_light_pairs(oatk_hip_ctx *ctx, uint32_t c, bool packed, const void **d_keys, const uint32_t **d_dist, uint64_t *n_keep, EgrKeyForm *form)
 {
     using namespace oatk;
     if (!ctx->counted) { ctx->err = "the light EC graph needs a resident scan + count"; return OATK_E_STATE; }
     if (!ctx->ec) ctx->ec = new EcState();
     EcState *e = ctx->ec;
     const uint64_t nv = ec_n_vtx(ctx), nr = ctx->n_reads, n = ctx->n_occ;
-    int rc;
+    const int dbg = ec_light_keys_debug();
+    *form = EgrKeyForm();
+    if (nv >= 0x7FFFFFFFULL) { ctx->err = "too many syncmers for 32-bit oriented vertex ids"; return OATK_E_ARG; }
+    if (n >= 0xFFFFFFFFULL) { ctx->err = "more than 2^32 adjacent pairs"; return OATK_E_ARG; }
     EENSURE(g_keys, (n + 1) * 8); EENSURE(g_dist, (n + 1) * 4);
-    EENSURE(g_other, 2 * nv + 8); EENSURE(g_keep, n + 8); EENSURE(g_lkeys, (n + 1) * 8); EENSURE(g_ldist, (n + 1) * 4);
+    EENSURE(g_other, 2 * nv + 8); EENSURE(g_lkeys, (n + 1) * 8); EENSURE(g_ldist, (n + 1) * 4); EENSURE(g_nruns, 64);
+    const uint32_t *cov = e->global? e->g_gcov.as<uint32_t>() : ctx->scm_cov.as<uint32_t>();
     t_begin(ctx, OATK_T_EC_GRAPH);
     CK(hipMemsetAsync(e->g_other.p, 0, 2 * nv + 8, ctx->stream));
-    if (n) hipLaunchKernelGGL(egr_pair_light_wave_kernel, dim3((unsigned) ((nr + 3) / 4)), dim3(256), 0, ctx->stream, nr, ctx->scm_off.as<uint64_t>(), ec_chains(ctx),
-                              ctx->pos_mpos.as<uint32_t>(), e->global? e->g_gcov.as<uint32_t>() : ctx->scm_cov.as<uint32_t>(), c, e->g_keys.as<uint64_t>(), e->g_dist.as<uint32_t>(),
-                              e->g_keep.as<uint8_t>(), e->g_other.as<uint8_t>());
     uint64_t nk = 0;
-    if (n) {
-        if (n >= 0xFFFFFFFFULL) { ctx->err = "more than 2^32 adjacent pairs"; return OATK_E_ARG; }
-        EENSURE(g_keys2, (n + 1) * 8); EENSURE(g_nruns, 64);
+    if (n && dbg == 0) {
+        form->all_bits = true;
+        EENSURE(g_keep, n + 8); EENSURE(g_keys2, (n + 1) * 8);
+        hipLaunchKernelGGL(egr_pair_light_wave_kernel, dim3((unsigned) ((nr + 3) / 4)), dim3(256), 0, ctx->stream, nr, ctx->scm_off.as<uint64_t>(), ec_chains(ctx),
+                           ctx->pos_mpos.as<uint32_t>(), cov, c, e->g_keys.as<uint64_t>(), e->g_dist.as<uint32_t>(), e->g_keep.as<uint8_t>(), e->g_other.as<uint8_t>());
         uint32_t *pos = e->g_keys2.as<uint32_t>();
         uint64_t *d_cnt = e->g_nruns.as<uint64_t>() + 2;
         auto flags = rocprim::make_transform_iterator(e->g_keep.as<uint8_t>(), [] __device__(uint8_t f) -> uint32_t { return f; });
@@ -565,10 +608,51 @@
                            e->g_dist.as<uint32_t>(), e->g_lkeys.as<uint64_t>(), e->g_ldist.as<uint32_t>(), d_cnt);
         CK(hipMemcpyAsync(&nk, d_cnt, 8, hipMemcpyDeviceToHost, ctx->stream));
         CK(hipStreamSynchronize(ctx->stream));
-    }
-    (void) rc;
+    } else if (n) {
+        const uint64_t nb = (n + EGR_FLAT_WG - 1) / EGR_FLAT_WG;
+        EENSURE(g_first, n + 8); EENSURE(g_kmask, nb * (EGR_FLAT_WG / 64) * 8); EENSURE(g_bcnt, (nb + 1) * 4); EENSURE(g_boff, (nb + 1) * 4);
+        CK(hipMemsetAsync(e->g_first.p, 0, n, ctx->stream));
+        CK(hipMemsetAsync(e->g_bcnt.as<uint32_t>() + nb, 0, 4, ctx->stream));
+        hipLaunchKernelGGL(egr_first_mark_kernel, dim3((unsigned) ((nr + 255) / 256)), dim3(256), 0, ctx->stream, nr, ctx->scm_off.as<uint64_t>(), e->g_first.as<uint8_t>());
+        const uint32_t *tab = cov;
+        size_t tb = 0;
+        if (packed) {
+            EENSURE(g_rank, (nv + 1) * 4);
+            auto is_cand = rocprim::make_transform_iterator(rocprim::make_counting_iterator<uint64_t>(0),
+                                                            [cov, nv, c] __device__(uint64_t i) -> uint32_t { return i < nv && cov[i] >= c; });
+            CK(rocprim::exclusive_scan(nullptr, tb, is_cand, e->g_rank.as<uint32_t>(), 0u, nv + 1, rocprim::plus<uint32_t>(), ctx->stream));
+            ENSURE(tmp, tb);
+            CK(rocprim::exclusive_scan(ctx->tmp.p, tb, is_cand, e->g_rank.as<uint32_t>(), 0u, nv + 1, rocprim::plus<uint32_t>(), ctx->stream));
+            uint32_t nc = 0;
+            CK(hipMemcpyAsync(&nc, e->g_rank.as<uint32_t>() + nv, 4, hipMemcpyDeviceToHost, ctx->stream));
+            CK(hipStreamSynchronize(ctx->stream));
+            EENSURE(g_cand, ((uint64_t) nc + 1) * 4);
+            if (nv) hipLaunchKernelGGL(egr_rank_table_kernel, dim3((unsigned) ((nv + 255) / 256)), dim3(256), 0, ctx->stream, nv, cov, c, e->g_rank.as<uint32_t>(), e->g_cand.as<uint32_t>());
+            uint32_t kb = 1;
+            while (kb < 32 && (2 * (uint64_t) (nc? nc : 1) - 1) >> kb) ++kb;
+            form->kb = kb, form->key32 = 2 * kb <= 32 && dbg != 64;
+            tab = e->g_rank.as<uint32_t>();
+        }
+        const dim3 grid((unsigned) nb), wg(EGR_FLAT_WG);
+        if (form->key32) hipLaunchKernelGGL(egr_pair_light_flat_kernel<uint32_t>, grid, wg, 0, ctx->stream, n, e->g_first.as<uint8_t>(), ec_chains(ctx), ctx->pos_mpos.as<uint32_t>(), tab, c,
+                                            form->kb, e->g_keys.as<uint32_t>(), e->g_dist.as<uint32_t>(), e->g_kmask.as<uint64_t>(), e->g_bcnt.as<uint32_t>(), e->g_other.as<uint8_t>());
+        else hipLaunchKernelGGL(egr_pair_light_flat_kernel<uint64_t>, grid, wg, 0, ctx->stream, n, e->g_first.as<uint8_t>(), ec_chains(ctx), ctx->pos_mpos.as<uint32_t>(), tab, c,
+                                form->kb, e->g_keys.as<uint64_t>(), e->g_dist.as<uint32_t>(), e->g_kmask.as<uint64_t>(), e->g_bcnt.as<uint32_t>(), e->g_other.as<uint8_t>());
+        tb = 0;
+        CK(rocprim::exclusive_scan(nullptr, tb, e->g_bcnt.as<uint32_t>(), e->g_boff.as<uint32_t>(), 0u, nb + 1, rocprim::plus<uint32_t>(), ctx->stream));
+        ENSURE(tmp, tb);
+        CK(rocprim::exclusive_scan(ctx->tmp.p, tb, e->g_bcnt.as<uint32_t>(), e->g_boff.as<uint32_t>(), 0u, nb + 1, rocprim::plus<uint32_t>(), ctx->stream));
+        if (form->key32) hipLaunchKernelGGL(egr_compact_flat_kernel<uint32_t>, grid, wg, 0, ctx->stream, (const uint64_t *) e->g_kmask.p, (const uint32_t *) e->g_boff.p,
+                                            (const uint32_t *) e->g_keys.p, (const uint32_t *) e->g_dist.p, e->g_lkeys.as<uint32_t>(), e->g_ldist.as<uint32_t>());
+        else hipLaunchKernelGGL(egr_compact_flat_kernel<uint64_t>, grid, wg, 0, ctx->stream, (const uint64_t *) e->g_kmask.p, (const uint32_t *) e->g_boff.p,
+                                (const uint64_t *) e->g_keys.p, (const uint32_t *) e->g_dist.p, e->g_lkeys.as<uint64_t>(), e->g_ldist.as<uint32_t>());
+        uint32_t nk32 = 0;
+        CK(hipMemcpyAsync(&nk32, e->g_boff.as<uint32_t>() + nb, 4, hipMemcpyDeviceToHost, ctx->stream));
+        CK(hipStreamSynchronize(ctx->stream));
+        nk = nk32;
+    }
     CK(hipGetLastError());
-    *d_keys = e->g_lkeys.as<uint64_t>(), *d_dist = e->g_ldist.as<uint32_t>(), *n_keep = nk;
+    *d_keys = e->g_lkeys.p, *d_dist = e->g_ldist.as<uint32_t>(), *n_keep = nk;
     return OATK_OK;
 }
 
@@ -579,12 +663,13 @@
     CK(hipSetDevice(ctx->device));
     if (!ctx->ec) ctx->ec = new EcState();
     if (err_mer_c == 0) return oatk_hip_ec_graph(ctx);
-    const uint64_t *k = nullptr;
+    const void *k = nullptr;
     const uint32_t *d = nullptr;
     uint64_t n = 0;
-    int rc = ec_light_pairs(ctx, err_mer_c, &k, &d, &n);
+    EgrKeyForm form;
+    int rc = ec_light_pairs(ctx, err_mer_c, true, &k, &d, &n, &form);
     if (rc) return rc;
-    if ((rc = ec_graph_build(ctx, k, d, nullptr, n, true)) != OATK_OK) return rc;
+    if ((rc = ec_graph_build(ctx, k, d, nullptr, n, true, form)) != OATK_OK) return rc;
     ctx->ec->light_c = err_mer_c;
     return OATK_OK;
 }
diff --git a/oatk_amd/csrc/api_multi.inc b/oatk_amd/csrc/api_multi.inc
--- a/oatk_amd/csrc/api_multi.inc
+++ b/oatk_amd/csrc/api_multi.inc
@@ -912,10 +912,12 @@
     uint64_t np_all = 0;
     if (light) {
         EcState *e = ctx->ec;
-        const uint64_t *lk = nullptr;
+        const void *lkv = nullptr;
         const uint32_t *ld = nullptr;
         uint64_t nk = 0, n_seg = 0;
-        if ((rc = ec_light_pairs(ctx, err_mer_c, &lk, &ld, &nk)) != OATK_OK) return rc;
+        EgrKeyForm form;
+        if ((rc = ec_light_pairs(ctx, err_mer_c, false, &lkv, &ld, &nk, &form)) != OATK_OK) return rc;
+        const uint64_t *lk = (const uint64_t *) lkv;
         EENSURE(g_keys2, (nk + 1) * 8); EENSURE(g_dist2, (nk + 1) * 4); EENSURE(g_head, nk + 8); EENSURE(g_hpos, (nk + 1) * 4); EENSURE(g_iota, (nk + 1) * 4);
         if (nk) {
             size_t tb = 0;
diff --git a/oatk_amd/csrc/ecgraph.hpp b/oatk_amd/csrc/ecgraph.hpp
--- a/oatk_amd/csrc/ecgraph.hpp
+++ b/oatk_amd/csrc/ecgraph.hpp
@@ -63,6 +63,94 @@
     const uint32_t p0 = wave_prev(p1);
     if (in && lane == 0) keys[o] = EGR_INVALID, dist[o] = 0, keep[o] = 0;
     if (in && lane > 0) emit(o + lane, v0, p0, v1, p1);
+}
+
+#define EGR_FLAT_WG 256
+__global__ void egr_first_mark_kernel(uint64_t n_reads, const uint64_t *scm_off, uint8_t *first)
+{
+    const uint64_t r = (uint64_t) blockIdx.x * blockDim.x + threadIdx.x;
+    if (r >= n_reads) return;
+    const uint64_t o = scm_off[r];
+    if (scm_off[r + 1] > o) first[o] = 1;
+}
+
+#define EGR_NO_RANK 0xFFFFFFFFu
+__global__ void egr_rank_table_kernel(uint64_t nv, const uint32_t *cov, uint32_t c, uint32_t *rank, uint32_t *cand)
+{
+    const uint64_t i = (uint64_t) blockIdx.x * blockDim.x + threadIdx.x;
+    if (i >= nv) return;
+    if (cov[i] >= c) cand[rank[i]] = (uint32_t) i;
+    else rank[i] = EGR_NO_RANK;
+}
+
+template <class KeyT>
+__global__ __launch_bounds__(EGR_FLAT_WG) void egr_pair_light_flat_kernel(uint64_t n, const uint8_t *first, const uint64_t *k_mer, const uint32_t *m_pos, const uint32_t *tab,
+                                                                          uint32_t c, uint32_t kb, KeyT *keys, uint32_t *dist, uint64_t *kmask, uint32_t *bcnt, uint8_t *other)
+{
+    __shared__ uint32_t wave_cnt[EGR_FLAT_WG / 64];
+    const uint64_t i = (uint64_t) blockIdx.x * EGR_FLAT_WG + threadIdx.x;
+    const int lane = threadIdx.x & 63, wave = threadIdx.x >> 6;
+    const bool in = i < n, own_prev = lane == 0 && in && i > 0;
+    const uint64_t km = in? k_mer[i] : 0;
+    const uint32_t mp = in? m_pos[i] : 0;
+    const bool head = in? first[i] != 0 : true;
+    const uint64_t km_p = own_prev? k_mer[i - 1] : 0;
+    const uint32_t mp_p = own_prev? m_pos[i - 1] : 0;
+    const uint32_t v1 = (uint32_t) (km >> 1) << 1 | (mp & 1u), p1 = mp >> 1;
+    const uint32_t v_p = (uint32_t) (km_p >> 1) << 1 | (mp_p & 1u);
+    const uint32_t t1 = in? tab[v1 >> 1] : 0;
+    const uint32_t t_p = own_prev? tab[v_p >> 1] : 0;
+    uint32_t v0 = wave_prev(v1), p0 = wave_prev(p1), t0 = wave_prev(t1);
+    if (own_prev) v0 = v_p, p0 = mp_p >> 1, t0 = t_p;
+    const bool c0 = kb? t0 != EGR_NO_RANK : t0 >= c, c1 = kb? t1 != EGR_NO_RANK : t1 >= c;
+    const bool fw = v0 <= v1, keep = !head && c0 && c1;
+    const uint32_t a = fw? v0 : v1 ^ 1u, b = fw? v1 : v0 ^ 1u;
+    if (!head) {
+        const bool ca = fw? c0 : c1, cb = fw? c1 : c0;
+        if (ca && !cb) other[a] = 1;
+        if (cb && !ca) other[b ^ 1u] = 1;
+    }
+    if (keep) {
+        if (kb) {
+            const uint32_t r0 = t0 << 1 | (v0 & 1u), r1 = t1 << 1 | (v1 & 1u);
+            const uint32_t ra = fw? r0 : r1 ^ 1u, rb = fw? r1 : r0 ^ 1u;
+            keys[i] = (KeyT) ((KeyT) ra << kb | rb);
+        } else {
+            keys[i] = (KeyT) ((uint64_t) a << 32 | b);
+        }
+        dist[i] = p1 - p0;
+    }
+    const uint64_t m = __ballot(keep);
+    if (lane == 0) kmask[i >> 6] = m, wave_cnt[wave] = (uint32_t) __builtin_popcountll(m);
+    __syncthreads();
+    if (threadIdx.x == 0) {
+        uint32_t s = 0;
+        for (int w = 0; w < EGR_FLAT_WG / 64; ++w) s += wave_cnt[w];
+        bcnt[blockIdx.x] = s;
+    }
+}
+
+template <class KeyT>
+__global__ __launch_bounds__(EGR_FLAT_WG) void egr_compact_flat_kernel(const uint64_t *kmask, const uint32_t *boff, const KeyT *keys, const uint32_t *dist, KeyT *lkeys, uint32_t *ldist)
+{
+    const uint64_t i = (uint64_t) blockIdx.x * EGR_FLAT_WG + threadIdx.x;
+    const int lane = threadIdx.x & 63, wave = threadIdx.x >> 6;
+    const uint64_t *bm = kmask + (uint64_t) blockIdx.x * (EGR_FLAT_WG / 64);
+    const uint64_t m = bm[wave];
+    if (!((m >> lane) & 1ULL)) return;
+    uint32_t p = boff[blockIdx.x] + (uint32_t) __builtin_popcountll(m & ((1ULL << lane) - 1ULL));
+    for (int w = 0; w < wave; ++w) p += (uint32_t) __builtin_popcountll(bm[w]);
+    lkeys[p] = keys[i], ldist[p] = dist[i];
+}
+
+template <class KeyT>
+__global__ void egr_unpack_keys_kernel(uint64_t n_runs, const KeyT *pk, uint32_t kb, const uint32_t *cand, uint64_t *ukeys)
+{
+    const uint64_t i = (uint64_t) blockIdx.x * blockDim.x + threadIdx.x;
+    if (i >= n_runs) return;
+    const uint64_t k = pk[i], ra = k >> kb, rb = k & ((1ULL << kb) - 1ULL);
+    const uint64_t a = (uint64_t) cand[ra >> 1] << 1 | (ra & 1ULL), b = (uint64_t) cand[rb >> 1] << 1 | (rb & 1ULL);
+    ukeys[i] = a << 32 | b;
 }
 
 __global__ void egr_seg_head_kernel(uint64_t n, const uint64_t *skeys, const uint32_t *sdist, uint8_t *head)
diff --git a/oatk_amd/device.py b/oatk_amd/device.py
--- a/oatk_amd/device.py
+++ b/oatk_amd/device.py
@@ -17,7 +17,7 @@
     "INGEST_SEQ": np.uint8, "INGEST_OFF": np.uint64, "INGEST_LEN": np.uint32, "INGEST_HDR": np.uint64,
     "CONS_SEL": np.uint32, "CONS_SLOT": np.uint32, "CONS_RL": np.uint32, "CONS_MSEQ": np.uint32, "CONS_FIRST": np.uint64, "CONS_TOT": np.uint64,
     "EG_IDX_P": np.uint64, "EG_IDX_N": np.uint32, "EG_ARC_V": np.uint64, "EG_ARC_W": np.uint64, "EG_ARC_LS": np.uint32,
-    "EG_ARC_COV": np.uint32, "EG_ARC_COMP": np.uint8,
+    "EG_ARC_COV": np.uint32, "EG_ARC_COMP": np.uint8, "EG_OTHER": np.uint8,
     "RA_ALN_SID": np.uint32, "RA_ALN_OFF": np.uint64, "RA_ALN_S": np.float64, "RA_FRG_UID": np.uint64, "RA_FRG_UBEG": np.uint32,
     "RA_FRG_UEND": np.uint32, "RA_FRG_SBEG": np.uint32, "RA_FRG_SEND": np.uint32, "RA_SKIPPED": np.uint32,
     "OVL_KEY": np.uint64, "OVL_OFF": np.uint64, "OVL_DIST": np.int32, "OVL_CNT": np.uint32, "OVL_TAIL": np.uint8,
```

Result: no change. 380.0, median of 3 (+0.5%).
